# CMU-Quake/hercules

Hardware: AMD Instinct MI355X
Metric: element-updates/sec (whole node) + achieved HBM GB/s, 64M-elem box (higher is better)
Workload: dtype f64

## Files before the change

hercules_amd/capi.py:

```python
import ctypes
import os

import numpy as np

_HERE = os.path.dirname(os.path.abspath(__file__))
_LIBPATH = os.environ.get("HQ_SOLVER_LIB") or os.path.join(_HERE, "csrc", "libhq_solver.so")

HQ_VARIANT_AUTO, HQ_VARIANT_SCATTER, HQ_VARIANT_PATCH = 0, 1, 2
IPC_BLOB_BYTES = 4096

EXPORTS = ["hq_device_count", "hq_last_error", "hq_create", "hq_destroy", "hq_get_info", "hq_get_info_sized", "hq_abi_version", "hq_comm_init_ipc_n",
           "hq_options_init", "hq_create_opts", "hq_get_options", "hq_real_bytes",
           "hq_comm_unique_id", "hq_comm_init", "hq_comm_selftest", "hq_group_link", "hq_group_run", "hq_set_source", "hq_run", "hq_sync", "hq_gather", "hq_gather3",
           "hq_download", "hq_upload", "hq_phase_force", "hq_phase_update", "hq_download_force",
           "hq_run_timed", "hq_dominant_kernel", "hq_plan_check", "hq_stencil_plan_check", "hq_check_finite",
           "hq_stencil_coefficients", "hq_brick_plan_check", "hq_brick_plan_check_n", "hq_comm_init_host",
           "hq_comm_ipc_export", "hq_comm_init_ipc", "hq_comm_init_loopback",
           "hq_record_add", "hq_record_pending", "hq_record_fetch", "hq_record_clear",
           "hq_snapshot_add", "hq_snapshot_pending", "hq_snapshot_fetch", "hq_snapshot_clear"]
HQ_SNAP_TM1, HQ_SNAP_TM2, HQ_SNAP_VEL = 1, 2, 4


class HqError(RuntimeError):
    pass


HOST_EXCHANGE_FN = ctypes.CFUNCTYPE(ctypes.c_int, ctypes.c_void_p, ctypes.c_int32, ctypes.POINTER(ctypes.c_int32),
                                    ctypes.POINTER(ctypes.c_int64), ctypes.POINTER(ctypes.c_void_p), ctypes.c_int32,
                                    ctypes.POINTER(ctypes.c_int32), ctypes.POINTER(ctypes.c_int64),
                                    ctypes.POINTER(ctypes.c_void_p), ctypes.c_int32)


class _Messenger(ctypes.Structure):
    _fields_ = [("procid", ctypes.c_int32), ("nodecount", ctypes.c_int32),
                ("mapping", ctypes.c_void_p)]


class _Schedule(ctypes.Structure):
    _fields_ = [("c_count", ctypes.c_int32), ("first_c", ctypes.POINTER(_Messenger)),
                ("s_count", ctypes.c_int32), ("first_s", ctypes.POINTER(_Messenger))]


class _Desc(ctypes.Structure):
    _fields_ = [("lenum", ctypes.c_int32), ("nharbored", ctypes.c_int32), ("ldnnum", ctypes.c_int32),
                ("lnid", ctypes.c_void_p), ("node_xyz", ctypes.c_void_p),
                ("dn_ldnid", ctypes.c_void_p), ("dn_ptr", ctypes.c_void_p), ("dn_lanid", ctypes.c_void_p),
                ("eTable", ctypes.c_void_p), ("nTable", ctypes.c_void_p),
                ("tm1", ctypes.c_void_p), ("tm2", ctypes.c_void_p),
                ("an_sched", _Schedule), ("dn_sched", _Schedule),
                ("deltaT", ctypes.c_double), ("rank", ctypes.c_int32), ("nranks", ctypes.c_int32),
                ("variant", ctypes.c_int32), ("reserved", ctypes.c_int32), ("node_gnid", ctypes.c_void_p),
                ("edata", ctypes.c_void_p), ("mat_bbase", ctypes.c_double), ("mat_threshold_damping", ctypes.c_double),
                ("mat_threshold_vpvs", ctypes.c_double)]


class _RecorderDesc(ctypes.Structure):
    _fields_ = [("npoints", ctypes.c_int32), ("ids", ctypes.c_void_p), ("phi", ctypes.c_void_p),
                ("rate", ctypes.c_int32), ("derivs", ctypes.c_int32), ("capacity", ctypes.c_int32)]


class _SnapshotDesc(ctypes.Structure):
    _fields_ = [("first", ctypes.c_int32), ("count", ctypes.c_int32), ("rate", ctypes.c_int32),
                ("first_step", ctypes.c_int32), ("fields", ctypes.c_int32), ("slots", ctypes.c_int32)]


class _Info(ctypes.Structure):
    _fields_ = [("variant", ctypes.c_int32), ("npatches", ctypes.c_int32),
                ("patch_pairs", ctypes.c_int64), ("device_bytes", ctypes.c_int64),
                ("step", ctypes.c_int32), ("nranks", ctypes.c_int32),
                ("lattice_patches", ctypes.c_int32), ("stencil_patches", ctypes.c_int32),
                ("ragged_patches", ctypes.c_int32), ("brick_units", ctypes.c_int32),
                ("brick_nodes", ctypes.c_int64), ("brick_units_pernode", ctypes.c_int32),
                ("brick_units_het", ctypes.c_int32), ("pcie_h2d_bytes", ctypes.c_int64),
                ("pcie_d2h_bytes", ctypes.c_int64), ("transport", ctypes.c_int32), ("ipc_arena_coarse", ctypes.c_int32),
                ("ipc_arena_kind", ctypes.c_int32), ("debug_halo", ctypes.c_int32),
                ("brick_units_packed", ctypes.c_int32), ("brick_units_ragged", ctypes.c_int32),
                ("brick_stream", ctypes.c_int32), ("brick_units_ragged_het", ctypes.c_int32), ("timed_steps", ctypes.c_int64),
                ("t_step_us", ctypes.c_double), ("t_shell_us", ctypes.c_double), ("t_interior_us", ctypes.c_double),
                ("t_chain_us", ctypes.c_double), ("t_chain_exposed_us", ctypes.c_double)]


OPTION_FIELDS = ["no_bricks", "brick_cz", "brick_minz", "brick_minnodes", "brick_no_het", "brick_no_ntsame", "brick_by_component",
                 "brick_stream", "brick_no_faces", "brick_half_tiles", "brick_no_pack", "patch_pipe", "patch_threads", "patch_pmax", "patch_pmerge", "patch_psplit", "patch_nlmax",
                 "patch_vmax", "patch_ragged", "patch_no_lattice", "patch_no_stencil", "patch_no_uniform", "patch_no_iso",
                 "patch_no_ntsame", "patch_no_dedup", "patch_wform", "patch_merge_rounds", "overlap", "no_overlap", "reserve_cus",
                 "cu_mask", "no_fused_share", "group_copies", "debug_halo", "ipc_arena"]


class Options(ctypes.Structure):
    _fields_ = ([("size", ctypes.c_uint64)] + [(n, ctypes.c_int32) for n in OPTION_FIELDS] +
                [("ipc_timeout_ms", ctypes.c_double), ("loopback_delay_us", ctypes.c_double),
                 ("verbose", ctypes.c_int32), ("quiet", ctypes.c_int32),
                 ("brick_ragged", ctypes.c_int32), ("brick_ragged_minfill", ctypes.c_int32),
                 ("allow_env", ctypes.c_int32), ("brick_ragged_het", ctypes.c_int32), ("reserved0", ctypes.c_int32),
                 ("phase_timing", ctypes.c_int32)])

    def __init__(self, **kw):
        super().__init__()
        load_library().hq_options_init(ctypes.byref(self), ctypes.c_uint64(ctypes.sizeof(self)))
        for k, v in kw.items():
            if k not in dict(self._fields_):
                raise TypeError("hq_options has no field %r" % k)
            setattr(self, k, v)

    def as_dict(self):
        return {k: getattr(self, k) for k, _ in self._fields_ if k != "size"}


_lib = None
_lib_f32 = None
_LIBPATH_F32 = os.environ.get("HQ_SOLVER_LIB_F32") or os.path.join(_HERE, "csrc", "libhq_solver_f32.so")


def load_library(path=None, precision="f64"):
    global _lib, _lib_f32
    if precision == "f32" and path is None:
        if _lib_f32 is None:
            _lib_f32 = load_library(_LIBPATH_F32)
            if _lib_f32.hq_real_bytes() != 4:
                raise HqError("%s was not built with -DHQ_SINGLE_PRECISION_SOLVER" % _LIBPATH_F32)
        return _lib_f32
    if _lib is not None and path is None:
        return _lib
    p = path or _LIBPATH
    if not os.path.exists(p):
        raise HqError("native library %s is missing: run `python -m hercules_amd.build` "
                      "(there is no Python/CPU fallback)" % p)
    probe = ctypes.CDLL(p, mode=ctypes.RTLD_LOCAL)
    lib = probe if probe.hq_real_bytes() == 4 else ctypes.CDLL(p, mode=ctypes.RTLD_GLOBAL)
    lib.hq_last_error.restype = ctypes.c_char_p
    lib.hq_dominant_kernel.restype = ctypes.c_char_p
    lib.hq_dominant_kernel.argtypes = [ctypes.c_void_p]
    for name in EXPORTS:
        getattr(lib, name)
    if path is None:
        _lib = lib
    return lib


def device_count():
    return int(load_library().hq_device_count())


def _check(rc, lib=None):
    if rc != 0:
        raise HqError("hq error %d: %s" % (rc, (lib or load_library()).hq_last_error().decode()))


# ... 30 lines not shown
        if lib.hq_real_bytes() != np.dtype(self.real).itemsize:
            raise HqError("library and precision %r disagree about sizeof(hq_real)" % precision)
        if isinstance(options, dict):
            options = Options(**options)
        keep = []
        lnid = np.ascontiguousarray(lnid, np.int32)
        etable = np.ascontiguousarray(etable, np.float64)
        ntable = np.ascontiguousarray(ntable, self.real)
        d = _Desc()
        d.lenum, d.nharbored = lnid.shape[0], ntable.shape[0]
        d.lnid, d.eTable, d.nTable = _ptr(lnid), _ptr(etable), _ptr(ntable)
        keep += [lnid, etable, ntable]
        if node_xyz is not None:
            node_xyz = np.ascontiguousarray(node_xyz, np.int32)
            keep.append(node_xyz)
            d.node_xyz = _ptr(node_xyz)
        for name, a in (("tm1", tm1), ("tm2", tm2)):
            if a is not None:
                a = np.ascontiguousarray(a, self.real)
                keep.append(a)
                setattr(d, name, _ptr(a))
        if dangling is not None:
            ids, ptr, anchors = [np.ascontiguousarray(x, np.int32) for x in dangling]
            keep += [ids, ptr, anchors]
            d.ldnnum = len(ids)
            d.dn_ldnid, d.dn_ptr, d.dn_lanid = _ptr(ids), _ptr(ptr), _ptr(anchors)
        if edata is not None:
            edata = np.ascontiguousarray(edata, np.float32)
            assert edata.shape == (lnid.shape[0], 4) and material is not None
            keep.append(edata)
            d.edata = _ptr(edata)
            d.mat_bbase, d.mat_threshold_damping, d.mat_threshold_vpvs = [float(v) for v in material]
        d.an_sched = _schedule(an_sched, keep)
        d.dn_sched = _schedule(dn_sched, keep)
        d.deltaT, d.rank, d.nranks, d.variant = dt, rank, nranks, variant
        self._h = ctypes.c_void_p()
        self.N, self.E = d.nharbored, d.lenum
        self._lib = lib
        if options is None:
            _check(lib.hq_create(ctypes.byref(d), ctypes.c_int(device), ctypes.byref(self._h)), lib)
        else:
            _check(lib.hq_create_opts(ctypes.byref(d), ctypes.c_int(device), ctypes.byref(options), ctypes.byref(self._h)), lib)

    def close(self):
        if getattr(self, "_h", None) and self._h.value:
            self._lib.hq_destroy(self._h)
            self._h = ctypes.c_void_p()

    __del__ = close

    def info(self):
        i = _Info()
        _check(self._lib.hq_get_info_sized(self._h, ctypes.byref(i), ctypes.c_uint64(ctypes.sizeof(i))), self._lib)
        return {k: getattr(i, k) for k, _ in _Info._fields_}

    def options(self):
        o = Options()
        _check(self._lib.hq_get_options(self._h, ctypes.byref(o), ctypes.c_uint64(ctypes.sizeof(o))), self._lib)
        return o.as_dict()

    def set_source(self, loaded_lnid, forces, step0=0):
        ids = np.ascontiguousarray(loaded_lnid, np.int32)
        F = np.ascontiguousarray(forces, np.float64)
        nsteps = F.shape[0] if len(ids) else 0
        _check(self._lib.hq_set_source(self._h, ctypes.c_int32(len(ids)), _ptr(ids),
                                       ctypes.c_int32(step0), ctypes.c_int32(nsteps), _ptr(F)))

    def comm_init(self, id128):
        buf = (ctypes.c_char * 128).from_buffer_copy(bytes(id128))
        _check(self._lib.hq_comm_init(self._h, buf), self._lib)

    def comm_init_host(self, exchange):
        import numpy as np

        def view(ptr, n):
            return np.ctypeslib.as_array(ctypes.cast(ctypes.c_void_p(ptr), ctypes.POINTER(ctypes.c_double)), shape=(int(n),))

        def trampoline(user, nrecv, rpeer, rcount, rbuf, nsend, speer, scount, sbuf, tag):
            try:
                exchange([(rpeer[i], view(rbuf[i], rcount[i])) for i in range(nrecv)],
                         [(speer[i], view(sbuf[i], scount[i])) for i in range(nsend)], tag)
                return 0
            except Exception:
                import traceback
                traceback.print_exc()
                return 1
        self._host_exchange = HOST_EXCHANGE_FN(trampoline)
        _check(self._lib.hq_comm_init_host(self._h, self._host_exchange, None), self._lib)

    def comm_ipc_export(self):
        buf = (ctypes.c_char * IPC_BLOB_BYTES)()
        _check(self._lib.hq_comm_ipc_export(self._h, buf), self._lib)
        return bytes(buf)

    def comm_init_ipc(self, blobs):
        raw = blobs if isinstance(blobs, (bytes, bytearray)) else b"".join(blobs)
        if len(raw) % IPC_BLOB_BYTES:
            raise HqError("comm_init_ipc: %d bytes is not a whole number of %d-byte blobs" % (len(raw), IPC_BLOB_BYTES))
        buf = (ctypes.c_char * len(raw)).from_buffer_copy(bytes(raw))
        _check(self._lib.hq_comm_init_ipc_n(self._h, buf, ctypes.c_int32(len(raw) // IPC_BLOB_BYTES)), self._lib)

    def comm_init_loopback(self):
        _check(self._lib.hq_comm_init_loopback(self._h), self._lib)

    def comm_selftest(self, count=1024):
        _check(self._lib.hq_comm_selftest(self._h, ctypes.c_int32(count)), self._lib)

# ... 97 lines not shown
        vel = np.empty((count, 3), np.float64) if fields & HQ_SNAP_VEL else None
        step = ctypes.c_int32(-1)
        _check(self._lib.hq_snapshot_fetch(self._h, ctypes.c_int32(handle), _ptr(tm1), _ptr(tm2), _ptr(vel),
                                           ctypes.byref(step)), self._lib)
        if step.value < 0:
            return -1, None, None, None
        return step.value, tm1, tm2, vel

    def snapshot_clear(self):
        _check(self._lib.hq_snapshot_clear(self._h), self._lib)
        self._snapshots = {}

    def phase_force(self):
        _check(self._lib.hq_phase_force(self._h), self._lib)

    def phase_update(self):
        _check(self._lib.hq_phase_update(self._h), self._lib)

    def download_force(self):
        f = np.empty((self.N, 3))
        _check(self._lib.hq_download_force(self._h, _ptr(f)), self._lib)
        return f


PLAN_REPORT = ("patches", "lattice_patches", "pairs", "distinct_row_blocks", "gather_passes", "gather_instructions",
               "lattice_gather_passes", "faults")


def plan_check(desc):
    rep = (ctypes.c_int64 * 8)()
    _check(load_library().hq_plan_check(ctypes.byref(desc), rep))
    return dict(zip(PLAN_REPORT, [int(v) for v in rep]))


STENCIL_PLAN_REPORT = ("patches", "tables", "full_lattices", "boundary_nodes", "corners_checked", "faults")


def stencil_plan_check(desc):
    rep = (ctypes.c_int64 * 6)()
    _check(load_library().hq_stencil_plan_check(ctypes.byref(desc), rep))
    return dict(zip(STENCIL_PLAN_REPORT, [int(v) for v in rep]))


BRICK_PLAN_REPORT = ("brick_nodes", "columns", "units", "units_one_nt_row", "het_units", "neighbours_checked",
                     "patch_nodes", "faults", "ragged_units", "ragged_nodes", "ragged_het_units", "ragged_het_nodes", "packed_units")


def brick_plan_check(desc):
    rep = (ctypes.c_int64 * len(BRICK_PLAN_REPORT))()
    _check(load_library().hq_brick_plan_check_n(ctypes.byref(desc), rep, ctypes.c_int32(len(BRICK_PLAN_REPORT))))
    return dict(zip(BRICK_PLAN_REPORT, [int(v) for v in rep]))


def comm_unique_id():
    buf = (ctypes.c_char * 128)()
    _check(load_library().hq_comm_unique_id(buf))
    return bytes(buf)


def group_link(solvers):
    arr = (ctypes.c_void_p * len(solvers))(*[s._h for s in solvers])
    lib = solvers[0]._lib
    _check(lib.hq_group_link(arr, ctypes.c_int32(len(solvers))), lib)


def group_run(solvers, nsteps):
    arr = (ctypes.c_void_p * len(solvers))(*[s._h for s in solvers])
    lib = solvers[0]._lib
    _check(lib.hq_group_run(arr, ctypes.c_int32(len(solvers)), ctypes.c_int32(nsteps)), lib)
    for s in solvers:
        s.sync()
```

hercules_amd/csrc/hq_brick.h:

```cpp
#ifndef HQ_BRICK_H
#define HQ_BRICK_H

#include <chrono>
#include <map>

#include "hq_patch.h"

#define HQ_BK_TX 64
#ifndef HQ_BK_TY
#define HQ_BK_TY 8
#endif
#define HQ_BK_THREADS (HQ_BK_TX * HQ_BK_TY)
#define HQ_BK_PY (HQ_BK_TX + 2)
#define HQ_BK_PLANE ((HQ_BK_TX + 2) * (HQ_BK_TY + 2))
#ifndef HQ_BK_ATTR
#define HQ_BK_ATTR
#endif
#define HQ_BK_NTSAME 1
#define HQ_BK_HET 2
#define HQ_BK_TOPFACE 8
#define HQ_BK_BOTFACE 16
#define HQ_BK_RAGGED 32
#define HQ_BK_PACKED 4
#ifndef HQ_BH_WAVES
#define HQ_BH_WAVES 8
#endif
#define HQ_BH_THREADS (64 * HQ_BH_WAVES)
#define HQ_BH_NRT (64 + 2 * (HQ_BH_WAVES - 1))
#define HQ_BH_TX 62
#define HQ_BH_TY (HQ_BH_WAVES - 1)
#define HQ_BH_PY 65
#define HQ_BH_CS HQ_BH_THREADS
#define HQ_BH_ROWS (65 * (HQ_BH_WAVES + 1))

struct hq_brick_unit {
    int64_t base;
    int64_t tab;
    int32_t nx, ny, np, flags;
    double  c1, c2, beta;
    double  m0, m2, m1;
    double  ft[7], fb[7];
    int64_t coef;
};

struct hq_brick_cfg {
    int cz = 32;
    int minz = 4;
    int minnodes = 512;
    int ragged = 1;
    int minfill = 128;
    int ragged_het = 1;
};

static hq_brick_cfg hq_brick_cfg_of(const hq_options& o)
{
    hq_brick_cfg c;
    c.cz = std::max(2, hq_value_or(o.brick_cz, c.cz));
    c.minz = std::max(1, hq_value_or(o.brick_minz, c.minz));
    c.minnodes = std::max(1, hq_value_or(o.brick_minnodes, c.minnodes));
    c.ragged = hq_value_or(o.brick_ragged, c.ragged) != 0;
    c.minfill = std::min(HQ_BK_THREADS, std::max(1, hq_value_or(o.brick_ragged_minfill, c.minfill)));
    c.ragged_het = hq_value_or(o.brick_ragged_het, c.ragged_het) != 0;
    return c;
}

struct hq_brick_host {
    int64_t nb = 0;
    std::vector<int32_t> perm;
    std::vector<hq_brick_unit> units;
    int32_t nsame = 0;
    int32_t nrag = 0;
    std::vector<int32_t> tab;
    std::vector<double> coef;
    std::vector<float> coef32;
    std::vector<double> nt2;
    int32_t nhet = 0;
    int32_t npacked = 0;
    int32_t nrhet = 0, nrpacked = 0;
    int32_t ncolumns = 0, nlevels = 0;
};

struct hq_brick_plan {
    int64_t nb = 0;
    int32_t nunits = 0, nsame = 0, nrag = 0, nhet = 0, npacked = 0, nrhet = 0, nrpacked = 0;
    hq_brick_unit* d_units = nullptr;
    int32_t* d_tab = nullptr;
    double* d_coef = nullptr;
    float* d_coef32 = nullptr;
    double* d_nt2 = nullptr;
    hq_mat_const mat = { 0, 0, 0, 0, 0, 0 };
    int32_t* d_src_ptr = nullptr;
    int32_t* d_src_ent = nullptr;
    std::vector<int64_t> h_base;
    std::vector<int32_t> h_slot;
    std::vector<int64_t> h_size;
    std::vector<int64_t> h_first;
};

struct hq_mat_src {
    const float* edata = nullptr;
    double dt = 0, bbase = 0, thr_damp = 0, thr_vpvs = 0;
};

static int hq_brick_plan_host(const hq_options& o, int64_t E, int64_t N, const int32_t* lnid, const int32_t* xyz, const double* c1,
                              const double* c2, const double* beta, const double* ntab, const char* excl,
                              hq_brick_host* B, const hq_mat_src* MS = nullptr)
{
    *B = hq_brick_host();
    if (!xyz || E <= 0 || N <= 0) return 0;
    const hq_brick_cfg cfg = hq_brick_cfg_of(o);
    const bool verbose = o.verbose > 1;
    auto t_lap = std::chrono::steady_clock::now();
    auto lap = [&](const char* what) {
        if (!verbose) return;
        const auto now = std::chrono::steady_clock::now();
        fprintf(stderr, "  brick plan: %-36s %6.2f s\n", what, std::chrono::duration<double>(now - t_lap).count());
        t_lap = now;
    };
    const int TX = HQ_BK_TX, TY = HQ_BK_TY;
    const bool want_het = !hq_set(o.brick_no_het);
    const bool stencil_ok = hq_stencil().ok;

    std::vector<int32_t> hs((size_t)E);
    std::map<int32_t, int64_t> cnt;
    {
        bool bad_order = false;
#pragma omp parallel
        {
            std::map<int32_t, int64_t> mine;
#pragma omp for schedule(static) reduction(|| : bad_order)
            for (int64_t e = 0; e < E; e++) {
                const int32_t* id = lnid + 8 * e;
                const int64_t h = (int64_t)xyz[3 * (int64_t)id[1]] - xyz[3 * (int64_t)id[0]];
                if (h <= 0 || h > 0x7fffffff) { bad_order = true; hs[(size_t)e] = 0; continue; }
                hs[(size_t)e] = (int32_t)h;
                mine[(int32_t)h]++;
            }
#pragma omp critical
            for (auto& kv : mine) cnt[kv.first] += kv.second;
        }
        if (bad_order) return 0;
    }
    lap("edge lengths");

    const bool want_faces = stencil_ok && hq_stencil().face_ok && !hq_set(o.brick_no_faces) && !hq_set(o.brick_no_ntsame);
    std::vector<uint8_t> touch;
    if (want_faces) {
        touch.assign((size_t)N, 0);
#pragma omp parallel for schedule(static)
        for (int64_t i = 0; i < E * 8; i++) {
            uint8_t& t8 = touch[(size_t)lnid[i]];
#pragma omp atomic
            t8++;
        }
    }

    struct level_t {
        int32_t h;
        int64_t O[3];
        int64_t D[3];
        std::vector<int32_t> Ng;
        std::vector<int32_t> Eg;
    };
    struct column_t { int lvl; int32_t x0, y0, nx, ny, z0, nz, ti, tj; int64_t base; int het; int top, bot; int rag; };
    struct ragged_t { std::vector<uint8_t> own; std::vector<int32_t> pfx; double c[3], m[3]; };
    std::vector<level_t> levels;
    std::vector<column_t> cols;
    std::vector<ragged_t> rags;
    std::vector<int32_t> ntx_of_level;

    for (auto& kv : cnt) {
        const int32_t h = kv.first;
        if (kv.second < (int64_t)cfg.minnodes) continue;
        level_t L;
        L.h = h;
        int64_t mn[3] = { INT64_MAX, INT64_MAX, INT64_MAX }, mx[3] = { INT64_MIN, INT64_MIN, INT64_MIN };
        {
            int64_t mn0 = INT64_MAX, mn1 = INT64_MAX, mn2 = INT64_MAX, mx0 = INT64_MIN, mx1 = INT64_MIN, mx2 = INT64_MIN;
#pragma omp parallel for schedule(static) reduction(min : mn0, mn1, mn2) reduction(max : mx0, mx1, mx2)
            for (int64_t e = 0; e < E; e++) {
                if (hs[(size_t)e] != h) continue;
                const int32_t* p = xyz + 3 * (int64_t)lnid[8 * e];
                mn0 = std::min<int64_t>(mn0, p[0]); mn1 = std::min<int64_t>(mn1, p[1]); mn2 = std::min<int64_t>(mn2, p[2]);
                mx0 = std::max<int64_t>(mx0, p[0]); mx1 = std::max<int64_t>(mx1, p[1]); mx2 = std::max<int64_t>(mx2, p[2]);
            }
            mn[0] = mn0; mn[1] = mn1; mn[2] = mn2; mx[0] = mx0; mx[1] = mx1; mx[2] = mx2;
        }
        bool ok = true;
        for (int d = 0; d < 3; d++) {
            L.O[d] = mn[d];
            if ((mx[d] - mn[d]) % h) ok = false;
            L.D[d] = (mx[d] - mn[d]) / h + 1;
        }
        if (!ok) continue;
        const int64_t NX = L.D[0] + 1, NY = L.D[1] + 1, NZ = L.D[2] + 1;
        const double vol = (double)NX * (double)NY * (double)NZ;
        if (vol > 8.0 * (double)kv.second + 65536.0 || vol > 2.0e9) continue;
        std::vector<int32_t>& Eg = L.Eg;
        Eg.assign((size_t)(L.D[0] * L.D[1] * L.D[2]), -1);
        L.Ng.assign((size_t)(NX * NY * NZ), -1);
        for (int pass = 0; pass < 2 && ok; pass++) {
            bool bad = false;
#pragma omp parallel for schedule(static) reduction(|| : bad)
            for (int64_t e = 0; e < E; e++) {
                if (hs[(size_t)e] != h) continue;
                const int32_t* id = lnid + 8 * e;
                int64_t q[3];
                bool good = true;
                for (int d = 0; d < 3; d++) {
                    const int64_t v = (int64_t)xyz[3 * (int64_t)id[0] + d] - L.O[d];
                    if (v % h) good = false;
                    q[d] = v / h;
                }
                if (!good) { bad = true; continue; }
                int32_t& cell = Eg[(size_t)((q[2] * L.D[1] + q[1]) * L.D[0] + q[0])];
// ... 9 lines not shown
            if (bad) ok = false;
        }
        if (!ok) continue;
        lap("level grids");
        std::vector<char> S((size_t)(NX * NY * NZ), 0);
        int64_t sx0 = INT64_MAX, sx1 = -1, sy0 = INT64_MAX, sy1 = -1;
        int64_t nsimple = 0;
#pragma omp parallel for schedule(static) reduction(min : sx0, sy0) reduction(max : sx1, sy1) reduction(+ : nsimple)
        for (int64_t Z = 1; Z < L.D[2]; Z++)
            for (int64_t Y = 1; Y < L.D[1]; Y++)
                for (int64_t X = 1; X < L.D[0]; X++) {
                    const int32_t n = L.Ng[(size_t)((Z * NY + Y) * NX + X)];
                    if (n < 0 || (excl && excl[n])) continue;
                    const double* q = ntab + 7 * (int64_t)n;
                    if (!((q[1] == q[2]) && (q[1] == q[3]) && (q[4] == q[5]) && (q[4] == q[6]))) continue;
                    int32_t e0 = -1;
                    bool s = true, uni = true;
                    for (int o = 0; o < 8 && s; o++) {
                        const int64_t cx = X - (o & 1), cy = Y - ((o >> 1) & 1), cz = Z - ((o >> 2) & 1);
                        const int32_t e = Eg[(size_t)((cz * L.D[1] + cy) * L.D[0] + cx)];
                        if (e < 0) { s = false; break; }
                        if (e0 < 0) e0 = e;
                        else uni = uni && c1[e] == c1[e0] && c2[e] == c2[e0] && beta[e] == beta[e0];
                    }
                    if (!s) continue;
                    if (!stencil_ok) uni = false;
                    if (!uni && !want_het) continue;
                    S[(size_t)((Z * NY + Y) * NX + X)] = uni ? 2 : 1;
                    nsimple++;
                    sx0 = std::min(sx0, X); sx1 = std::max(sx1, X); sy0 = std::min(sy0, Y); sy1 = std::max(sy1, Y);
                }
        if (nsimple < cfg.minnodes) continue;
        if (want_faces && L.D[2] >= 2) {
#pragma omp parallel for schedule(static) collapse(2)
            for (int side = 0; side < 2; side++)
                for (int64_t Y = 1; Y < L.D[1]; Y++)
                    for (int64_t X = 1; X < L.D[0]; X++) {
                        const int64_t Z = side ? L.D[2] : 0, cz = side ? L.D[2] - 1 : 0;
                        const int32_t n = L.Ng[(size_t)((Z * NY + Y) * NX + X)];
                        if (n < 0 || (excl && excl[n]) || touch[(size_t)n] != 4) continue;
                        int32_t e0 = -1;
                        bool s4 = true;
                        for (int o = 0; o < 4 && s4; o++) {
                            const int32_t e = Eg[(size_t)((cz * L.D[1] + (Y - ((o >> 1) & 1))) * L.D[0] + (X - (o & 1)))];
                            if (e < 0) { s4 = false; break; }
                            if (e0 < 0) e0 = e;
                            else s4 = c1[e] == c1[e0] && c2[e] == c2[e0] && beta[e] == beta[e0];
                        }
                        if (s4 && c1[e0] + c2[e0] != 0.0) S[(size_t)((Z * NY + Y) * NX + X)] = side ? 4 : 3;
                    }
        }
        lap("simple nodes");
        const int lvl = (int)levels.size();
        std::vector<std::vector<column_t>> found;
        int32_t ntx_lvl = 1;
        const int rag = cfg.ragged && stencil_ok && !hq_set(o.brick_no_ntsame) ? 1 : 0;
        const int half = rag || hq_value_or(o.brick_half_tiles, 1) != 0 ? 1 : 0;
        const int rag_het = cfg.ragged && want_het && cfg.ragged_het ? 1 : 0;
        for (int round = 0; round < 2 + half + rag_het; round++) {
            const bool rh_round = rag_het && round == 2 + half;
            const int pass = (round == 1 + half || rh_round) ? 1 : 0;
            const bool rag_round = rag && round == 1;
            const int PTX = pass == 1 ? HQ_BH_TX : (round == 0 || rag_round ? TX : TX / 2), PTY = pass == 0 ? TY : HQ_BH_TY;
            auto in_run = [pass](char v) { return pass == 0 ? v == 2 : (v == 1 || v == 2); };
            if (round >= 1) {
                sx0 = INT64_MAX; sx1 = -1; sy0 = INT64_MAX; sy1 = -1;
                for (int64_t Z = 0; Z < NZ; Z++)
                    for (int64_t Y = 0; Y < NY; Y++)
                        for (int64_t X = 0; X < NX; X++)
                            if (in_run(S[(size_t)((Z * NY + Y) * NX + X)])) { sx0 = std::min(sx0, X); sx1 = std::max(sx1, X); sy0 = std::min(sy0, Y); sy1 = std::max(sy1, Y); }
                if (sx1 < 0) { if (pass == 1) break; else continue; }
            }
            const int32_t ntx = (int32_t)((sx1 - sx0) / PTX + 1), nty = (int32_t)((sy1 - sy0) / PTY + 1);
            if (round == 0) ntx_lvl = ntx;
            const size_t f0 = found.size();
            found.resize(f0 + (size_t)nty);
            std::vector<std::vector<ragged_t>> found_r(rag_round || rh_round ? (size_t)nty : 0);
            const int32_t minfill = rh_round ? std::max(1, cfg.minfill * (HQ_BH_TX * HQ_BH_TY) / HQ_BK_THREADS) : cfg.minfill;
#pragma omp parallel for schedule(dynamic, 1)
            for (int32_t tj = 0; tj < nty; tj++) {
                const int64_t y0 = sy0 + (int64_t)tj * PTY;
                const int32_t ny = (int32_t)std::min<int64_t>(PTY, sy1 - y0 + 1);
                std::vector<int32_t> cntz;
                for (int32_t ti = 0; ti < ntx; ti++) {
                    const int64_t x0 = sx0 + (int64_t)ti * PTX;
                    const int32_t nx = (int32_t)std::min<int64_t>(PTX, sx1 - x0 + 1);
                    if (rag_round || rh_round) {
                        cntz.assign((size_t)NZ, 0);
                        for (int iter = 0; iter < (rh_round ? 1 : 4); iter++) {
                            int32_t n0 = -1;
                            int64_t Z0 = 0, X0 = 0, Y0 = 0;
                            auto cand = [&](char v) { return rh_round ? (v == 1 || v == 2) : v == 2; };
                            for (int64_t Z = 1; Z < L.D[2] && n0 < 0; Z++)
                                for (int64_t y = y0; y < y0 + ny && n0 < 0; y++) {
                                    const char* row = &S[(size_t)((Z * NY + y) * NX + x0)];
                                    for (int32_t x = 0; x < nx; x++)
                                        if (cand(row[x])) { n0 = L.Ng[(size_t)((Z * NY + y) * NX + x0 + x)]; Z0 = Z; Y0 = y; X0 = x0 + x; break; }
                                }
                            if (n0 < 0) break;
                            const int32_t e0 = L.Eg[(size_t)(((Z0 - 1) * L.D[1] + (Y0 - 1)) * L.D[0] + (X0 - 1))];
                            const double rc[3] = { c1[e0], c2[e0], beta[e0] };
                            const double* q0 = ntab + 7 * (int64_t)n0;
                            auto match = [&](int64_t X, int64_t Y, int64_t Z) -> bool {
                                if (rh_round) return true;
                                const double* q = ntab + 7 * (int64_t)L.Ng[(size_t)((Z * NY + Y) * NX + X)];
                                if (q[0] != q0[0] || q[1] != q0[1] || q[4] != q0[4]) return false;
                                const int32_t e = L.Eg[(size_t)(((Z - 1) * L.D[1] + (Y - 1)) * L.D[0] + (X - 1))];
                                return c1[e] == rc[0] && c2[e] == rc[1] && beta[e] == rc[2];
                            };
                            for (int64_t Z = Z0; Z < L.D[2]; Z++) {
                                int32_t cnt = 0;
                                for (int64_t y = y0; y < y0 + ny; y++) {
                                    const char* row = &S[(size_t)((Z * NY + y) * NX + x0)];
                                    for (int32_t x = 0; x < nx; x++) cnt += cand(row[x]) && match(x0 + x, y, Z);
                                }
                                cntz[(size_t)Z] = cnt;
                            }
                            int64_t ra = -1;
                            for (int64_t Z = Z0; Z <= L.D[2]; Z++) {
                                const bool in = Z < L.D[2] && cntz[(size_t)Z] >= minfill;
                                if (in) { if (ra < 0) ra = Z; continue; }
                                if (ra < 0) continue;
                                const int64_t nz = Z - ra;
                                int64_t total = 0;
                                for (int64_t z = ra; z < Z; z++) total += cntz[(size_t)z];
                                if (nz >= cfg.minz && total >= cfg.minnodes) {
                                    ragged_t R;
                                    R.own.assign((size_t)(nz * nx * ny), 0);
                                    R.pfx.assign((size_t)nz + 1, 0);
                                    for (int d = 0; d < 3; d++) R.c[d] = rc[d];
                                    R.m[0] = q0[0]; R.m[1] = q0[1]; R.m[2] = q0[4];
                                    for (int64_t z = ra; z < Z; z++) {
                                        int32_t k = 0;
                                        for (int64_t y = y0; y < y0 + ny; y++) {
                                            char* row = &S[(size_t)((z * NY + y) * NX + x0)];
                                            for (int32_t x = 0; x < nx; x++)
                                                if (cand(row[x]) && match(x0 + x, y, z)) { R.own[(size_t)(((z - ra) * ny + (y - y0)) * nx + x)] = 1; row[x] = 0; k++; }
                                        }
                                        R.pfx[(size_t)(z - ra) + 1] = R.pfx[(size_t)(z - ra)] + k;
// ... 114 lines not shown
    }
    {
        int nth = 1;
#pragma omp parallel
        {
#pragma omp single
            nth = omp_get_num_threads();
        }
        std::vector<int64_t> first((size_t)nth + 1, 0);
#pragma omp parallel for schedule(static, 1)
        for (int t = 0; t < nth; t++) {
            const int64_t lo = N * t / nth, hi = N * (t + 1) / nth;
            int64_t cnt = 0;
            for (int64_t n = lo; n < hi; n++) cnt += B->perm[(size_t)n] < 0;
            first[(size_t)t + 1] = cnt;
        }
        for (int i = 0; i < nth; i++) first[(size_t)i + 1] += first[(size_t)i];
#pragma omp parallel for schedule(static, 1)
        for (int t = 0; t < nth; t++) {
            const int64_t lo = N * t / nth, hi = N * (t + 1) / nth;
            int64_t k = nb + first[(size_t)t];
            for (int64_t n = lo; n < hi; n++) if (B->perm[(size_t)n] < 0) B->perm[(size_t)n] = (int32_t)k++;
        }
        if (nb + first[(size_t)nth] != N) { g_patch_err = "brick plan: numbering is not a permutation"; return -1; }
    }
    lap("numbering");
    B->nb = nb;
    B->ncolumns = (int32_t)cols.size();
    B->nlevels = (int32_t)levels.size();

    struct unit_t { int col; int32_t za, np; int64_t key; };
    std::vector<unit_t> us;
    int cz = cfg.cz;
    if (!hq_given(o.brick_cz)) {
        for (cz = 32; cz > 8; cz /= 2) {
            int64_t n = 0;
            for (auto& c : cols) n += (c.nz + cz - 1) / cz;
            if (n >= 512) break;
        }
    }
    for (size_t ci = 0; ci < cols.size(); ci++) {
        const column_t& c = cols[ci];
        const int32_t nch = (c.nz + cz - 1) / cz;
        const int32_t G = std::max(1, 64 / std::max(1, ntx_of_level[(size_t)c.lvl]));
        for (int32_t k = 0; k < nch; k++) {
            const int32_t za = (int32_t)((int64_t)c.nz * k / nch), zb = (int32_t)((int64_t)c.nz * (k + 1) / nch);
            const int64_t key = ((int64_t)c.lvl << 56) | ((int64_t)(c.tj / G) << 42) | ((int64_t)((c.z0 + za) / cz) << 28) |
                                ((int64_t)(c.tj % G) << 20) | (int64_t)c.ti;
            us.push_back({ (int)ci, c.z0 + za, zb - za, key });
        }
    }
    std::stable_sort(us.begin(), us.end(), [](const unit_t& a, const unit_t& b) { return a.key < b.key; });
    B->units.resize(us.size());
    std::vector<int64_t> toff(us.size() + 1, 0);
    for (size_t u = 0; u < us.size(); u++) {
        const column_t& c = cols[(size_t)us[u].col];
        const int64_t nr = 2 * (c.nx + 2) + 2 * c.ny;
        toff[u + 1] = toff[u] + ((int64_t)(us[u].np + 2) * nr + (c.rag ? us[u].np + 2 : 2) * (int64_t)c.nx * c.ny + 3) / 4 * 4;
    }
    B->tab.assign((size_t)toff[us.size()] + 64, 0);
    std::vector<int64_t> coff(us.size() + 1, 0);
    for (size_t u = 0; u < us.size(); u++)
        coff[u + 1] = coff[u] + (cols[(size_t)us[u].col].het ? (int64_t)(us[u].np + 1) * HQ_BH_THREADS * 3 : 0);
    B->coef.assign((size_t)coff[us.size()] + 8, 0.0);
    const bool try_pack = MS && MS->edata && MS->dt > 0 && !hq_set(o.brick_no_pack);
    if (try_pack) { B->coef32.assign((size_t)coff[us.size()] + 8, 0.0f); B->nt2.assign(2 * (size_t)N, 0.0); }
    int fault = 0;
    auto set_fault = [&]() {
#pragma omp atomic write
        fault = 1;
    };
    std::vector<char> same(us.size(), 0);
#pragma omp parallel for schedule(dynamic, 16)
    for (int64_t u = 0; u < (int64_t)us.size(); u++) {
        const column_t& c = cols[(size_t)us[(size_t)u].col];
        const level_t& L = levels[(size_t)c.lvl];
        const int64_t NX = L.D[0] + 1, NY = L.D[1] + 1;
        const int32_t za = us[(size_t)u].za, np = us[(size_t)u].np, nx = c.nx, ny = c.ny, nr = 2 * (nx + 2) + 2 * ny;
        auto dev = [&](int64_t X, int64_t Y, int64_t Z) -> int32_t {
            if (X < 0 || Y < 0 || Z < 0 || X > L.D[0] || Y > L.D[1] || Z > L.D[2]) { set_fault(); return 0; }
            const int32_t n = L.Ng[(size_t)((Z * NY + Y) * NX + X)];
            if (n < 0) { set_fault(); return 0; }
            return B->perm[(size_t)n];
        };
        int32_t* t = B->tab.data() + toff[(size_t)u];
        hq_brick_unit& U = B->units[(size_t)u];
        if (c.rag) {
            const ragged_t& R = rags[(size_t)c.rag - 1];
            auto any = [&](int64_t X, int64_t Y, int64_t Z) -> int32_t {
                if (X < 0 || Y < 0 || Z < 0 || X > L.D[0] || Y > L.D[1] || Z > L.D[2]) return -1;
                const int32_t n = L.Ng[(size_t)((Z * NY + Y) * NX + X)];
                return n < 0 ? -1 : B->perm[(size_t)n];
            };
            auto owns = [&](int32_t i, int32_t j, int32_t k) -> bool {
                return i >= 0 && i < nx && j >= 0 && j < ny && k >= 1 && k <= np && R.own[(size_t)((((int64_t)za - 1 + k - c.z0) * ny + j) * nx + i)];
            };
            auto wanted = [&](int32_t i, int32_t j, int32_t k) -> bool {
                for (int32_t dk = -1; dk <= 1; dk++)
                    for (int32_t dj = -1; dj <= 1; dj++)
                        for (int32_t di = -1; di <= 1; di++)
                            if (owns(i + di, j + dj, k + dk)) return true;
                return false;
            };
            for (int32_t k = 0; k < np + 2; k++) {
                const int64_t Z = (int64_t)za - 1 + k;
                int32_t* r = t + (int64_t)k * nr;
                for (int32_t i = 0; i < nx + 2; i++) {
                    r[i] = wanted(i - 1, -1, k) ? any(c.x0 - 1 + i, c.y0 - 1, Z) : -1;
                    r[nx + 2 + i] = wanted(i - 1, ny, k) ? any(c.x0 - 1 + i, c.y0 + ny, Z) : -1;
                }
                for (int32_t j = 0; j < ny; j++) {
                    r[2 * (nx + 2) + j] = wanted(-1, j, k) ? any(c.x0 - 1, c.y0 + j, Z) : -1;
                    r[2 * (nx + 2) + ny + j] = wanted(nx, j, k) ? any(c.x0 + nx, c.y0 + j, Z) : -1;
                }
                int32_t* pl = t + (int64_t)(np + 2) * nr + (int64_t)k * nx * ny;
                for (int32_t j = 0; j < ny; j++)
                    for (int32_t i = 0; i < nx; i++) {
                        const bool own = owns(i, j, k);
                        const int32_t q = own || wanted(i, j, k) ? any(c.x0 + i, c.y0 + j, Z) : -1;
                        if (own && q < 0) set_fault();
                        pl[j * nx + i] = own ? q : (q < 0 ? -1 : -q - 2);
                    }
            }
            U.base = c.base + R.pfx[(size_t)(za - c.z0)];
            U.tab = toff[(size_t)u];
            U.nx = nx; U.ny = ny; U.np = np; U.flags = HQ_BK_NTSAME | HQ_BK_RAGGED;
            memset(U.ft, 0, sizeof U.ft); memset(U.fb, 0, sizeof U.fb);
            U.coef = 0;
            if (!c.het) {
                U.c1 = R.c[0]; U.c2 = R.c[1]; U.beta = R.c[2];
                U.m0 = R.m[0]; U.m2 = R.m[1]; U.m1 = R.m[2];
                same[(size_t)u] = 4;
                continue;
            }
            U.flags = HQ_BK_RAGGED;
            U.c1 = U.c2 = U.beta = 0.0; U.m0 = 1.0; U.m2 = U.m1 = 0.0;
        }
        if (!c.rag) {
        for (int32_t k = 0; k < np + 2; k++) {
            const int64_t Z = (int64_t)za - 1 + k;
            int32_t* r = t + (int64_t)k * nr;
            for (int32_t i = 0; i < nx + 2; i++) { r[i] = dev(c.x0 - 1 + i, c.y0 - 1, Z); r[nx + 2 + i] = dev(c.x0 - 1 + i, c.y0 + ny, Z); }
            for (int32_t j = 0; j < ny; j++) { r[2 * (nx + 2) + j] = dev(c.x0 - 1, c.y0 + j, Z); r[2 * (nx + 2) + ny + j] = dev(c.x0 + nx, c.y0 + j, Z); }
        }
        int32_t* cap = t + (int64_t)(np + 2) * nr;
        for (int32_t j = 0; j < ny; j++)
            for (int32_t i = 0; i < nx; i++) {
                cap[j * nx + i] = dev(c.x0 + i, c.y0 + j, (int64_t)za - 1);
                cap[nx * ny + j * nx + i] = dev(c.x0 + i, c.y0 + j, (int64_t)za + np);
            }
        U.base = c.base + (int64_t)(za - c.z0 + c.top) * nx * ny;
        U.tab = toff[(size_t)u];
        U.nx = nx; U.ny = ny; U.np = np; U.flags = 0;
        memset(U.ft, 0, sizeof U.ft); memset(U.fb, 0, sizeof U.fb);
        if (c.top && za == c.z0) {
            U.flags |= HQ_BK_TOPFACE;
            memcpy(U.ft, ntab + 7 * (int64_t)L.Ng[(size_t)((((int64_t)za - 1) * NY + c.y0) * NX + c.x0)], sizeof U.ft);
        }
        if (c.bot && za + np == c.z0 + c.nz) {
            U.flags |= HQ_BK_BOTFACE;
            memcpy(U.fb, ntab + 7 * (int64_t)L.Ng[(size_t)((((int64_t)za + np) * NY + c.y0) * NX + c.x0)], sizeof U.fb);
        }
        const int32_t n0 = L.Ng[(size_t)(((int64_t)za * NY + c.y0) * NX + c.x0)];
        {
            const int32_t e0 = L.Eg[(size_t)((((int64_t)za - 1) * L.D[1] + (c.y0 - 1)) * L.D[0] + (c.x0 - 1))];
            if (e0 < 0) { set_fault(); continue; }
            U.c1 = c1[e0]; U.c2 = c2[e0]; U.beta = beta[e0];
        }
        bool sm = true;
        const double* q0 = ntab + 7 * (int64_t)n0;
        for (int32_t z = 0; z < np && sm; z++)
            for (int32_t y = 0; y < ny && sm; y++)
                for (int32_t x = 0; x < nx; x++) {
                    const int32_t n = L.Ng[(size_t)((((int64_t)za + z) * NY + (c.y0 + y)) * NX + (c.x0 + x))];
                    const double* q = ntab + 7 * (int64_t)n;
                    if (q[0] != q0[0] || q[1] != q0[1] || q[4] != q0[4]) { sm = false; break; }
                }
        if (sm && !c.het && !hq_set(o.brick_no_ntsame)) { U.flags |= HQ_BK_NTSAME; same[(size_t)u] = 1; }
        U.m0 = q0[0]; U.m2 = q0[1]; U.m1 = q0[4];
        U.coef = 0;
        }
        if (c.het) {
            U.flags |= HQ_BK_HET;
            same[(size_t)u] = c.rag ? 5 : 2;
            U.coef = coff[(size_t)u];
            double* cf = B->coef.data() + coff[(size_t)u];
            for (int32_t l = 0; l <= np; l++)
                for (int32_t j = 0; j < HQ_BH_WAVES; j++)
                    for (int32_t i = 0; i < 64; i++) {
                        const int64_t cx = (int64_t)c.x0 - 1 + i, cy = (int64_t)c.y0 - 1 + j, cz = (int64_t)za - 1 + l;
                        double* o = cf + (int64_t)l * (3 * HQ_BH_THREADS) + (j * 64 + i);
                        int32_t e = -1;
                        if (cx >= 0 && cy >= 0 && cz >= 0 && cx < L.D[0] && cy < L.D[1] && cz < L.D[2])
                            e = L.Eg[(size_t)((cz * L.D[1] + cy) * L.D[0] + cx)];
                        if (e >= 0) { o[0] = c1[e]; o[HQ_BH_CS] = c2[e]; o[2 * HQ_BH_CS] = beta[e]; }
                        else if (!c.rag && i <= nx && j <= ny) set_fault();
                    }
            if (try_pack) {
                bool ok = true;
                int32_t e0 = L.Eg[(size_t)(((int64_t)za * L.D[1] + c.y0) * L.D[0] + c.x0)];
                if (c.rag) {
                    e0 = -1;
                    for (int32_t l = 0; l <= np && e0 < 0; l++)
                        for (int32_t j = 0; j < HQ_BH_WAVES && e0 < 0; j++)
                            for (int32_t i = 0; i < 64 && e0 < 0; i++) {
                                const int64_t cx = (int64_t)c.x0 - 1 + i, cy = (int64_t)c.y0 - 1 + j, cz = (int64_t)za - 1 + l;
                                if (cx >= 0 && cy >= 0 && cz >= 0 && cx < L.D[0] && cy < L.D[1] && cz < L.D[2]) e0 = L.Eg[(size_t)((cz * L.D[1] + cy) * L.D[0] + cx)];
                            }
                }
                const float hf = e0 >= 0 ? MS->edata[4 * (int64_t)e0] : 0.0f;
                hq_mat_const K = { (MS->dt * MS->dt) * (double)hf, (double)hf, MS->dt, MS->bbase, MS->thr_damp, MS->thr_vpvs };
                float* cq = B->coef32.data() + coff[(size_t)u];
                for (int32_t l = 0; l <= np && ok; l++)
                    for (int32_t j = 0; j < HQ_BH_WAVES && ok; j++)
                        for (int32_t i = 0; i < 64; i++) {
                            const int64_t cx = (int64_t)c.x0 - 1 + i, cy = (int64_t)c.y0 - 1 + j, cz = (int64_t)za - 1 + l;
                            int32_t e = -1;
                            if (cx >= 0 && cy >= 0 && cz >= 0 && cx < L.D[0] && cy < L.D[1] && cz < L.D[2])
                                e = L.Eg[(size_t)((cz * L.D[1] + cy) * L.D[0] + cx)];
                            float* o = cq + (int64_t)l * (3 * HQ_BH_THREADS) + (j * 64 + i);
                            o[0] = o[HQ_BH_CS] = o[2 * HQ_BH_CS] = 0.0f;
                            if (e < 0) continue;
                            const float* ed = MS->edata + 4 * (int64_t)e;
                            if (ed[0] != hf || !(ed[3] > 0.0f)) { ok = false; break; }
                            bool hit = false;
                            for (int fixed = 0; fixed < 2 && !hit; fixed++) {
                                double k1, k2, kb;
                                hq_material_coef(fixed ? -ed[3] : ed[3], ed[2], ed[1], K, &k1, &k2, &kb);
                                if (k1 == c1[e] && k2 == c2[e] && kb == beta[e]) { o[0] = fixed ? -ed[3] : ed[3]; o[HQ_BH_CS] = ed[2]; o[2 * HQ_BH_CS] = ed[1]; hit = true; }
                            }
                            if (!hit) { ok = false; break; }
                        }
                const int32_t* own_ids = c.rag ? t + (int64_t)(np + 2) * nr + (int64_t)nx * ny : nullptr;
                for (int32_t z = 0; z < np && ok; z++)
                    for (int32_t y = 0; y < ny && ok; y++)
                        for (int32_t x = 0; x < nx; x++) {
                            if (own_ids && own_ids[((int64_t)z * ny + y) * nx + x] < 0) continue;
                            const int32_t n = L.Ng[(size_t)((((int64_t)za + z) * NY + (c.y0 + y)) * NX + (c.x0 + x))];
                            const double* q = ntab + 7 * (int64_t)n;
                            const double sdiff = q[0] - q[4];
                            if (q[0] - sdiff != q[4] || fabs((2.0 * q[0] - sdiff) - q[1]) > 1e-15 * fabs(q[1])) { ok = false; break; }
                            double* o2 = B->nt2.data() + 2 * (own_ids ? (int64_t)own_ids[((int64_t)z * ny + y) * nx + x] : U.base + ((int64_t)z * ny + y) * nx + x);
                            o2[0] = q[0]; o2[1] = sdiff;
                        }
                if (ok) { U.flags |= HQ_BK_PACKED; same[(size_t)u] = c.rag ? 6 : 3; U.c1 = K.A; U.c2 = K.h; }
            }
        }
    }
    lap("unit tables");
    if (fault) { g_patch_err = "brick plan: a neighbour of a simple node is missing"; return -1; }
    {
        std::vector<hq_brick_unit> a, r, b, h, hp, rh, rhp;
        for (size_t u = 0; u < us.size(); u++)
            (same[u] == 1 ? a : (same[u] == 4 ? r : (same[u] == 2 ? h : (same[u] == 3 ? hp : (same[u] == 5 ? rh : (same[u] == 6 ? rhp : b)))))).push_back(B->units[u]);
        B->nsame = (int32_t)(a.size() + r.size());
        B->nrag = (int32_t)r.size();
        B->nhet = (int32_t)(h.size() + hp.size());
        B->npacked = (int32_t)hp.size();
        B->nrhet = (int32_t)(rh.size() + rhp.size());
        B->nrpacked = (int32_t)rhp.size();
        a.insert(a.end(), r.begin(), r.end());
        a.insert(a.end(), b.begin(), b.end());
        a.insert(a.end(), h.begin(), h.end());
        a.insert(a.end(), hp.begin(), hp.end());
        a.insert(a.end(), rh.begin(), rh.end());
        a.insert(a.end(), rhp.begin(), rhp.end());
        B->units.swap(a);
        if (B->npacked + B->nrpacked == 0) { std::vector<float>().swap(B->coef32); std::vector<double>().swap(B->nt2); }
        if (verbose) fprintf(stderr, "  brick plan: %d units: %d with one n_t row of which %d ragged, %d per-element coefficients of which %d packed, %d ragged per-element of which %d packed\n",
                             (int)B->units.size(), B->nsame, B->nrag, B->nhet, B->npacked, B->nrhet, B->nrpacked);
        if (verbose && B->nrag) {
            int64_t pos = 0, own = 0, other = 0;
            for (const hq_brick_unit& U : B->units) {
                if (!(U.flags & HQ_BK_RAGGED)) continue;
                const int32_t* pl = B->tab.data() + U.tab + (int64_t)(U.np + 2) * (2 * (U.nx + 2) + 2 * U.ny);
                for (int64_t i = 0; i < (int64_t)U.nx * U.ny * (U.np + 2); i++) { pos++; own += pl[i] >= 0; other += pl[i] <= -2; }
            }
            fprintf(stderr, "  brick plan: ragged units: %lld positions, %lld owned, %lld loaded for their neighbours' sake\n", (long long)pos, (long long)own, (long long)other);
        }
    }
    return 0;
}


static __device__ __forceinline__ double hq_uniform(double v)
{
    const int lo = __builtin_amdgcn_readfirstlane(__double2loint(v)), hi = __builtin_amdgcn_readfirstlane(__double2hiint(v));
    return __hiloint2double(hi, lo);
}

template <bool PERNODE, bool BYCOMP, bool RAGGED = false>
__global__ void HQ_BK_ATTR __launch_bounds__(HQ_BK_THREADS, 4)
hq_k_brick(int32_t count, int32_t per_xcd, const hq_brick_unit* __restrict__ units, const int32_t* __restrict__ tab,
           const hq_real* __restrict__ u1g, const hq_real* __restrict__ u2g, hq_real* __restrict__ ung,
           const double* __restrict__ nt3, const int32_t* __restrict__ src_ptr, const int32_t* __restrict__ src_ent,
           const double* __restrict__ F, double dt2, hq_stencil_coef sc)
{
    __shared__ __align__(16) double s_w[2 * 3 * HQ_BK_PLANE];
    const int slot = (int)(blockIdx.x & 7) * per_xcd + (int)(blockIdx.x >> 3);
    if (slot >= count) return;
    const hq_brick_unit U = units[slot];
    const int nx = U.nx, ny = U.ny, np = U.np, nxy = nx * ny, nr = 2 * (nx + 2) + 2 * ny;
    const int t = threadIdx.x, lx = t & (HQ_BK_TX - 1), ly = t >> 6;
    const bool active = lx < nx && ly < ny;
    const int sidx = active ? ly * nx + lx : 0;
    const int myrow = (ly + 1) * HQ_BK_PY + lx + 1;
    const bool ring = t < nr;
    int rrow;
    {
        int rx, ry;
        if (t < nx + 2) { rx = t - 1; ry = -1; }
        else if (t < 2 * (nx + 2)) { rx = t - (nx + 2) - 1; ry = ny; }
        else if (t < 2 * (nx + 2) + ny) { rx = -1; ry = t - 2 * (nx + 2); }
        else { rx = nx; ry = t - 2 * (nx + 2) - ny; }
        rrow = (ry + 1) * HQ_BK_PY + rx + 1;
    }
    const int32_t* __restrict__ utab = tab + U.tab;
    const int rofs = ring ? t : 0;
    const int32_t* __restrict__ cap = utab + (int64_t)(np + 2) * nr;
    int32_t vOut = -1, vMid = RAGGED ? cap[sidx] : 0, vCur = RAGGED ? cap[nxy + sidx] : 0, vNext = 0;
    const int32_t id_lo = RAGGED ? (vMid >= 0 ? vMid : -vMid - 2) : cap[sidx];
    const double beta = U.beta;
    double P[6], Q[2];
#pragma unroll
    for (int i = 0; i < 6; i++) P[i] = hq_uniform(U.c1 * sc.p1[i] + U.c2 * sc.p2[i]);
#pragma unroll
    for (int i = 0; i < 2; i++) Q[i] = hq_uniform(U.c1 * sc.q1[i] + U.c2 * sc.q2[i]);
    const bool has_src = F && src_ptr[slot + 1] > src_ptr[slot];

    hq_real x1[3] = { 0, 0, 0 }, x2[3] = { 0, 0, 0 }, y1[3] = { 0, 0, 0 }, y2[3] = { 0, 0, 0 };
    double mn[3] = { U.m0, U.m2, U.m1 };
    double m0A = hq_uniform(1.0 / U.m0), m0B = m0A;
    double fA[3] = { 0.0, 0.0, 0.0 }, fB[3] = { 0.0, 0.0, 0.0 };
    int32_t rid = utab[rofs];

#define HQ_BK_LOAD(node_)                                                                             \
    {                                                                                                 \
        const int64_t a_ = (node_);                                                                   \
        if (active && (!RAGGED || a_ >= 0)) {                                                         \
            _Pragma("unroll") for (int d = 0; d < 3; d++) { x1[d] = u1g[3 * a_ + d]; x2[d] = u2g[3 * a_ + d]; } \
            if (PERNODE) { _Pragma("unroll") for (int d = 0; d < 3; d++) mn[d] = nt3[3 * a_ + d]; }    \
        }                                                                                             \
        if (ring && (!RAGGED || rid >= 0)) {                                                          \
            const int64_t b_ = (int64_t)rid;                                                          \
            _Pragma("unroll") for (int d = 0; d < 3; d++) { y1[d] = u1g[3 * b_ + d]; y2[d] = u2g[3 * b_ + d]; } \
        }                                                                                             \
    }
#define HQ_BK_PUT(s_, acc_, M2_, M1_)                                                                 \
    {                                                                                                 \
        hq_lds_double* img_ = (hq_lds_double*)s_w + 3 * HQ_BK_PLANE * (s_);                            \
        if (active) {                                                                                 \
            _Pragma("unroll") for (int d = 0; d < 3; d++) {                                           \
                const double a1_ = x1[d], a2_ = x2[d];                                                \
// ... 77 lines not shown
            g[0] = fma(P[2], C[0], fma(P[3], sx[0], fma(P[4], sy[0], fma(P[5], dg[0], Q[1] * A_y))));
            g[1] = fma(P[2], C[1], fma(P[3], sy[1], fma(P[4], sx[1], fma(P[5], dg[1], Q[1] * A_x))));
            g[2] = fma(P[1], C[2], fma(P[3], sxy_z, P[5] * dg[2]));
            Uo[0] = fma(Q[0], Bx0_z, Q[1] * Bx1_z);
            Uo[1] = fma(Q[0], By0_z, Q[1] * By1_z);
            Uo[2] = fma(Q[0], Bx0_x, fma(Q[1], Bx1_x, fma(Q[0], By0_y, Q[1] * By1_y)));
        }
        if (k == 0 && topf) {
            m[0] = fma(rho, Uo[0], 0.5 * m[0]); m[1] = fma(rho, Uo[1], 0.5 * m[1]); m[2] = fma(-rho, Uo[2], 0.5 * m[2]);
        }
        if (k == np + 1 && botf && active) {
            double f[3];
            f[0] = fB[0] + fma(-rho, Uo[0], 0.5 * m[0]); f[1] = fB[1] + fma(-rho, Uo[1], 0.5 * m[1]); f[2] = fB[2] + fma(rho, Uo[2], 0.5 * m[2]);
            const int local = np * nxy + sidx;
            if (has_src) {
                for (int i = src_ptr[slot]; i < src_ptr[slot + 1]; i++)
                    if (src_ent[2 * i] == local) {
                        const int li = src_ent[2 * i + 1];
                        for (int d = 0; d < 3; d++) f[d] += F[3 * li + d] * dt2;
                    }
            }
            hq_real* out = ung + 3 * (int64_t)cap[nxy + sidx];
            const double rm = 1.0 / U.fb[0];
#pragma unroll
            for (int d = 0; d < 3; d++) out[d] = f[d] * rm;
        }
        const bool outface = k == 1 && topf;
        if ((k >= 2 || outface) && active && (!RAGGED || vOut >= 0)) {
            double f[3];
#pragma unroll
            for (int d = 0; d < 3; d++) f[d] = fA[d] + (g[d] + Uo[d]);
            const int local = RAGGED ? (int)(vOut - U.base) : (k - 2) * nxy + sidx;
            if (has_src) {
                for (int i = src_ptr[slot]; i < src_ptr[slot + 1]; i++)
                    if (src_ent[2 * i] == local) {
                        const int li = src_ent[2 * i + 1];
                        for (int d = 0; d < 3; d++) f[d] += F[3 * li + d] * dt2;
                    }
            }
            hq_real* out = ung + 3 * (RAGGED ? (int64_t)vOut : (outface ? (int64_t)cap[sidx] : U.base + (int64_t)local));
            const double rm = outface ? 1.0 / U.ft[0] : m0A;
#pragma unroll
            for (int d = 0; d < 3; d++) out[d] = f[d] * rm;
        }
#pragma unroll
        for (int d = 0; d < 3; d++) { fA[d] = fB[d] + m[d]; fB[d] = g[d] - Uo[d]; }
        if (RAGGED) { vOut = vMid; vMid = vCur; vCur = vNext; }
        if (PERNODE) { m0A = m0B; m0B = 1.0 / mn[0]; }
        if (k < np || (k == np && !botf)) HQ_BK_PUT((k + 1) & 1, fB, mn[1], mn[2])
        else if (k == np) HQ_BK_PUT((k + 1) & 1, fB, U.fb[1 + d], U.fb[4 + d])
    }
#undef HQ_BK_LOAD
#undef HQ_BK_PUT
}


#define HQ_BH_LDS (8 * (2 * 2 * 3 * HQ_BH_ROWS + 6 * HQ_BH_THREADS))
#ifndef HQ_BH_ABL
#define HQ_BH_ABL 0
#endif

static __device__ __forceinline__ double hq_dpp_from_next_lane(double v)
{
    int lo = __double2loint(v), hi = __double2hiint(v);
    lo = __builtin_amdgcn_update_dpp(0, lo, 0x130, 0xf, 0xf, true);
    hi = __builtin_amdgcn_update_dpp(0, hi, 0x130, 0xf, 0xf, true);
    return __hiloint2double(hi, lo);
}

static __device__ __forceinline__ int64_t hq_rag_node(int32_t v) { return v >= 0 ? (int64_t)v : (v <= -2 ? (int64_t)(-v - 2) : (int64_t)0); }

template <bool PACKED, bool RAGGED = false>
__global__ void __launch_bounds__(HQ_BH_THREADS, HQ_BH_WAVES == 12 ? 3 : 4)
hq_k_brick_het(int32_t count, int32_t per_xcd, const hq_brick_unit* __restrict__ units, const int32_t* __restrict__ tab,
               const void* __restrict__ coef_any, const hq_real* __restrict__ u1g, const hq_real* __restrict__ u2g,
               hq_real* __restrict__ ung, const double* __restrict__ nt3, const int32_t* __restrict__ src_ptr,
               const int32_t* __restrict__ src_ent, const double* __restrict__ F, double dt2, hq_mat_const mat)
{
    extern __shared__ __align__(16) double s_het[];
    hq_lds_double* const img = (hq_lds_double*)s_het;
    hq_lds_double* const xch = img + 2 * 2 * 3 * HQ_BH_ROWS;
    const int slot = (int)(blockIdx.x & 7) * per_xcd + (int)(blockIdx.x >> 3);
    if (slot >= count) return;
    const hq_brick_unit U = units[slot];
    const int nx = U.nx, ny = U.ny, np = U.np, nxy = nx * ny, nr = 2 * (nx + 2) + 2 * ny;
    const int t = threadIdx.x, lx = t & 63, ly = t >> 6;
    const bool owner = lx < nx && ly < ny;
    const int sidx = owner ? ly * nx + lx : 0;
    const int myrow = (ly + 1) * HQ_BH_PY + lx + 1;
    const int row0 = ly * HQ_BH_PY + lx;
    const int rq = ly == HQ_BH_WAVES - 1 ? lx : (lx >= 62 ? 64 + 2 * ly + (lx - 62) : -1);
    const bool ringA = rq >= 0 && rq < nr, ringB = rq >= 0 && rq + HQ_BH_NRT < nr;
    auto ring_row = [&](int r) {
        int rx, ry;
        if (r < nx + 2) { rx = r - 1; ry = -1; }
        else if (r < 2 * (nx + 2)) { rx = r - (nx + 2) - 1; ry = ny; }
        else if (r < 2 * (nx + 2) + ny) { rx = -1; ry = r - 2 * (nx + 2); }
        else { rx = nx; ry = r - 2 * (nx + 2) - ny; }
        return (ry + 1) * HQ_BH_PY + rx + 1;
    };
    const int rrowA = ringA ? ring_row(rq) : 0, rrowB = ringB ? ring_row(rq + HQ_BH_NRT) : 0;
    const int32_t* __restrict__ rtabA = tab + U.tab + (ringA ? rq : 0);
    const int32_t* __restrict__ rtabB = tab + U.tab + (ringB ? rq + HQ_BH_NRT : 0);
    const int32_t* __restrict__ cap = tab + U.tab + (int64_t)(np + 2) * nr;
    const int64_t id_lo = RAGGED ? 0 : cap[sidx], id_hi = RAGGED ? 0 : cap[nxy + sidx];
    int32_t vload = RAGGED ? cap[sidx] : 0, vnext = RAGGED ? cap[nxy + sidx] : 0, idA = -1, idB = -1;
// ... 87 lines not shown
                    G[yb][zb][2] = Z[m1] + hq_dpp_from_next_lane(Z[m0]);
                }
#pragma unroll
            for (int zb = 0; zb < 2; zb++)
#pragma unroll
                for (int d = 0; d < 3; d++) xch[(3 * zb + d) * HQ_BH_THREADS + t] = G[0][zb][d];
            __syncthreads();
            if (owner) {
                double H0[3], H1[3];
#pragma unroll
                for (int d = 0; d < 3; d++) {
                    H0[d] = G[1][0][d] + xch[d * HQ_BH_THREADS + t + 64];
                    H1[d] = G[1][1][d] + xch[(3 + d) * HQ_BH_THREADS + t + 64];
                }
                if (l >= 1 && (!RAGGED || idA >= 0)) {
                    double f[3];
#pragma unroll
                    for (int d = 0; d < 3; d++) f[d] = accA[d] + (H0[d] - H1[d]);
                    const int local = RAGGED ? (int)((int64_t)idA - U.base) : (l - 1) * nxy + sidx;
                    if (has_src) {
                        for (int i = src_ptr[slot]; i < src_ptr[slot + 1]; i++)
                            if (src_ent[2 * i] == local) {
                                const int li = src_ent[2 * i + 1];
                                for (int d = 0; d < 3; d++) f[d] += F[3 * li + d] * dt2;
                            }
                    }
                    hq_real* out = ung + 3 * (U.base + (int64_t)local);
#pragma unroll
                    for (int d = 0; d < 3; d++) out[d] = f[d] * m0A;
                }
#pragma unroll
                for (int d = 0; d < 3; d++) accA[d] = accB[d] + (H0[d] + H1[d]);
                m0A = m0B;
                if (RAGGED) idA = idB;
            }
        }
        if (l < np) HQ_BH_PUT(l & 1, accB, m0B)
        if (PACKED) hq_material_coef(nrho, nvs, nvp, K, &c1, &c2, &beta);
        else { c1 = nc1; c2 = nc2; beta = nbeta; }
        asm volatile("" : "+v"(c1), "+v"(c2), "+v"(beta), "+v"(ridA), "+v"(ridB));
        if (RAGGED) { asm volatile("" : "+v"(vnext)); ridA = ridA < 0 ? 0 : ridA; ridB = ridB < 0 ? 0 : ridB; }
        if (l + 1 < np) HQ_BH_REQUEST(l + 3)
        __syncthreads();
    }
#undef HQ_BH_REQUEST
#undef HQ_BH_LOAD
#undef HQ_BH_LOAD_B
#undef HQ_BH_PUT
}


static void hq_brick_free(hq_brick_plan* P)
{
    void* ptrs[] = { P->d_units, P->d_tab, P->d_coef, P->d_coef32, P->d_nt2, P->d_src_ptr, P->d_src_ent };
    for (void* p : ptrs) if (p) hipFree(p);
    *P = hq_brick_plan();
}

static int hq_brick_upload(hq_brick_plan* P, const hq_brick_host& B, int64_t* bytes)
{
    P->nb = B.nb;
    P->nunits = (int32_t)B.units.size();
    P->nsame = B.nsame;
    P->nrag = B.nrag;
    P->nhet = B.nhet;
    P->npacked = B.npacked;
    P->nrhet = B.nrhet;
    P->nrpacked = B.nrpacked;
    if (P->nunits == 0) return 0;
    if (P->nhet + P->nrhet > 0) {
        if (P->nhet > P->npacked || P->nrhet > P->nrpacked) {
            if (hipMalloc((void**)&P->d_coef, 8 * B.coef.size()) != hipSuccess) { g_patch_err = "hipMalloc failed"; return -2; }
            *bytes += (int64_t)(8 * B.coef.size());
            if (hipMemcpy(P->d_coef, B.coef.data(), 8 * B.coef.size(), hipMemcpyHostToDevice) != hipSuccess) { g_patch_err = "brick coefficient upload failed"; return -3; }
        }
        if (P->npacked + P->nrpacked > 0) {
            if (hipMalloc((void**)&P->d_coef32, 4 * B.coef32.size()) != hipSuccess || hipMalloc((void**)&P->d_nt2, 8 * B.nt2.size()) != hipSuccess) { g_patch_err = "hipMalloc failed"; return -2; }
            *bytes += (int64_t)(4 * B.coef32.size() + 8 * B.nt2.size());
            if (hipMemcpy(P->d_coef32, B.coef32.data(), 4 * B.coef32.size(), hipMemcpyHostToDevice) != hipSuccess ||
                hipMemcpy(P->d_nt2, B.nt2.data(), 8 * B.nt2.size(), hipMemcpyHostToDevice) != hipSuccess) { g_patch_err = "brick coefficient upload failed"; return -3; }
        }
        static bool attr_set = false;
        if (!attr_set) {
            if (hipFuncSetAttribute((const void*)hq_k_brick_het<false>, hipFuncAttributeMaxDynamicSharedMemorySize, HQ_BH_LDS) != hipSuccess ||
                hipFuncSetAttribute((const void*)hq_k_brick_het<true>, hipFuncAttributeMaxDynamicSharedMemorySize, HQ_BH_LDS) != hipSuccess ||
                hipFuncSetAttribute((const void*)hq_k_brick_het<false, true>, hipFuncAttributeMaxDynamicSharedMemorySize, HQ_BH_LDS) != hipSuccess ||
                hipFuncSetAttribute((const void*)hq_k_brick_het<true, true>, hipFuncAttributeMaxDynamicSharedMemorySize, HQ_BH_LDS) != hipSuccess) { g_patch_err = "hq_k_brick_het: LDS attribute"; return -3; }
            attr_set = true;
        }
    }
    if (hipMalloc((void**)&P->d_units, sizeof(hq_brick_unit) * B.units.size()) != hipSuccess ||
        hipMalloc((void**)&P->d_tab, 4 * B.tab.size()) != hipSuccess) { g_patch_err = "hipMalloc failed"; return -2; }
    *bytes += (int64_t)(sizeof(hq_brick_unit) * B.units.size() + 4 * B.tab.size());
    if (hipMemcpy(P->d_units, B.units.data(), sizeof(hq_brick_unit) * B.units.size(), hipMemcpyHostToDevice) != hipSuccess ||
        hipMemcpy(P->d_tab, B.tab.data(), 4 * B.tab.size(), hipMemcpyHostToDevice) != hipSuccess) { g_patch_err = "brick table upload failed"; return -3; }
    std::vector<std::pair<int64_t, int32_t>> by_base;
    for (int32_t u = 0; u < P->nunits; u++) by_base.push_back({ B.units[(size_t)u].base, u });
    std::sort(by_base.begin(), by_base.end());
    for (auto& pr : by_base) {
        const hq_brick_unit& U = B.units[(size_t)pr.second];
        const int64_t nxy = (int64_t)U.nx * U.ny;
        const int top = (U.flags & HQ_BK_TOPFACE) != 0, bot = (U.flags & HQ_BK_BOTFACE) != 0;
        int64_t size = nxy * (U.np + top + bot);
        if (U.flags & HQ_BK_RAGGED) {
            const int32_t* pl = B.tab.data() + U.tab + (int64_t)(U.np + 2) * (2 * (U.nx + 2) + 2 * U.ny);
            size = 0;
            for (int64_t i = nxy; i < nxy * (U.np + 1); i++) size += pl[i] >= 0;
        }
        P->h_base.push_back(pr.first - top * nxy); P->h_slot.push_back(pr.second); P->h_size.push_back(size);
        P->h_first.push_back(pr.first);
    }
    return 0;
}

static int hq_brick_set_source(hq_brick_plan* P, int32_t nloaded, const int32_t* loaded, int64_t* bytes)
{
    if (P->d_src_ptr) { hipFree(P->d_src_ptr); P->d_src_ptr = nullptr; }
    if (P->d_src_ent) { hipFree(P->d_src_ent); P->d_src_ent = nullptr; }
    if (nloaded <= 0 || P->nunits == 0) return 0;
    std::vector<std::array<int32_t, 3>> rec;
    for (int32_t i = 0; i < nloaded; i++) {
        if (loaded[i] >= P->nb) continue;
        const size_t k = (size_t)(std::upper_bound(P->h_base.begin(), P->h_base.end(), (int64_t)loaded[i]) - P->h_base.begin()) - 1;
        rec.push_back({ P->h_slot[k], (int32_t)(loaded[i] - P->h_first[k]), i });
    }
    if (rec.empty()) return 0;
    std::sort(rec.begin(), rec.end());
    std::vector<int32_t> ptr((size_t)P->nunits + 1, 0), ent(rec.size() * 2);
    for (auto& r : rec) ptr[(size_t)r[0] + 1]++;
    for (int32_t u = 0; u < P->nunits; u++) ptr[(size_t)u + 1] += ptr[(size_t)u];
    for (size_t k = 0; k < rec.size(); k++) { ent[2 * k] = rec[k][1]; ent[2 * k + 1] = rec[k][2]; }
    if (hipMalloc((void**)&P->d_src_ptr, 4 * ptr.size()) != hipSuccess) { P->d_src_ptr = nullptr; return -2; }
    if (hipMalloc((void**)&P->d_src_ent, 4 * ent.size()) != hipSuccess) {
        hipFree(P->d_src_ptr); P->d_src_ptr = nullptr; P->d_src_ent = nullptr;
        return -2;
    }
    if (hipMemcpy(P->d_src_ptr, ptr.data(), 4 * ptr.size(), hipMemcpyHostToDevice) != hipSuccess ||
        hipMemcpy(P->d_src_ent, ent.data(), 4 * ent.size(), hipMemcpyHostToDevice) != hipSuccess) {
        hipFree(P->d_src_ptr); hipFree(P->d_src_ent); P->d_src_ptr = nullptr; P->d_src_ent = nullptr;
        return -3;
    }
    *bytes += (int64_t)(4 * ptr.size() + 4 * ent.size());
    return 0;
}

static void hq_brick_launch(const hq_brick_plan* P, const hq_real* u1, const hq_real* u2, hq_real* un, const double* nt3,
                            const double* F, double dt2, hipStream_t stream, bool light = false)
{
    const int32_t cnt[7] = { P->nsame - P->nrag, P->nunits - P->nsame - P->nhet - P->nrhet, P->nhet - P->npacked, P->npacked, P->nrag,
                             P->nrhet - P->nrpacked, P->nrpacked };
    int32_t first = 0;
    for (int k4 = 0; k4 < 7; k4++) {
        const int k = k4 == 0 ? 0 : (k4 == 1 ? 4 : (k4 < 5 ? k4 - 1 : k4));
        const int32_t count = cnt[k];
        if (count <= 0) continue;
        const int per_xcd = (count + 7) / 8;
        const int32_t* sp = P->d_src_ptr ? P->d_src_ptr + first : nullptr;
#define HQ_BK_ARGS count, per_xcd, P->d_units + first, P->d_tab, u1, u2, un, nt3, sp, P->d_src_ent, (sp ? F : nullptr), dt2, hq_stencil().c
#ifdef HQ_EXPERIMENT
        const unsigned xpad = getenv("HQ_X_BRICK_LDS_PAD") ? (unsigned)atoi(getenv("HQ_X_BRICK_LDS_PAD")) : 0u;
        if (xpad && k == 0) {
            static bool once = false;
            if (!once) {
                once = true;
                hipFuncSetAttribute((const void*)hq_k_brick<false, true>, hipFuncAttributeMaxDynamicSharedMemorySize, (int)xpad);
                hipFuncSetAttribute((const void*)hq_k_brick<false, false>, hipFuncAttributeMaxDynamicSharedMemorySize, (int)xpad);
            }
            if (light) hq_k_brick<false, true><<<per_xcd * 8, HQ_BK_THREADS, xpad, stream>>>(HQ_BK_ARGS);
            else hq_k_brick<false, false><<<per_xcd * 8, HQ_BK_THREADS, xpad, stream>>>(HQ_BK_ARGS);
        } else
#endif
        if (k == 0 && light) hq_k_brick<false, true><<<per_xcd * 8, HQ_BK_THREADS, 0, stream>>>(HQ_BK_ARGS);
        else if (k == 0) hq_k_brick<false, false><<<per_xcd * 8, HQ_BK_THREADS, 0, stream>>>(HQ_BK_ARGS);
        else if (k == 1 && light) hq_k_brick<true, true><<<per_xcd * 8, HQ_BK_THREADS, 0, stream>>>(HQ_BK_ARGS);
        else if (k == 1) hq_k_brick<true, false><<<per_xcd * 8, HQ_BK_THREADS, 0, stream>>>(HQ_BK_ARGS);
        else if (k == 4 && light) hq_k_brick<false, true, true><<<per_xcd * 8, HQ_BK_THREADS, 0, stream>>>(HQ_BK_ARGS);
        else if (k == 4) hq_k_brick<false, false, true><<<per_xcd * 8, HQ_BK_THREADS, 0, stream>>>(HQ_BK_ARGS);
        else if (k == 2) hq_k_brick_het<false><<<per_xcd * 8, HQ_BH_THREADS, HQ_BH_LDS, stream>>>(count, per_xcd, P->d_units + first, P->d_tab, P->d_coef, u1, u2, un, nt3, sp,
                                                                                               P->d_src_ent, (sp ? F : nullptr), dt2, P->mat);
        else if (k == 3) hq_k_brick_het<true><<<per_xcd * 8, HQ_BH_THREADS, HQ_BH_LDS, stream>>>(count, per_xcd, P->d_units + first, P->d_tab, P->d_coef32, u1, u2, un, P->d_nt2, sp,
                                                                                   P->d_src_ent, (sp ? F : nullptr), dt2, P->mat);
        else if (k == 5) hq_k_brick_het<false, true><<<per_xcd * 8, HQ_BH_THREADS, HQ_BH_LDS, stream>>>(count, per_xcd, P->d_units + first, P->d_tab, P->d_coef, u1, u2, un, nt3, sp,
                                                                                                     P->d_src_ent, (sp ? F : nullptr), dt2, P->mat);
        else hq_k_brick_het<true, true><<<per_xcd * 8, HQ_BH_THREADS, HQ_BH_LDS, stream>>>(count, per_xcd, P->d_units + first, P->d_tab, P->d_coef32, u1, u2, un, P->d_nt2, sp,
                                                                                          P->d_src_ent, (sp ? F : nullptr), dt2, P->mat);
#undef HQ_BK_ARGS
        first += count;
    }
}

#endif
```

hercules_amd/csrc/hq_engine.hip:

```cpp
#include <hip/hip_runtime.h>
#include <dlfcn.h>
#include <stdint.h>
#include <stdio.h>
#include <stdlib.h>
#include <string.h>
#include <unistd.h>

#include <algorithm>
#include <chrono>
#include <vector>

#define HQ_SOLVER_IMPLEMENTATION 1
#include "../../include/hq_solver.h"
#include "hq_kernels.h"
#include "hq_opts.h"
#include "hq_patch.h"
#include "hq_brick.h"


static thread_local char g_err[512] = "";

static int hq_fail(int code, const char* fmt, const char* a = "", const char* b = "")
{
    snprintf(g_err, sizeof g_err, fmt, a, b);
// ... 62 lines not shown
    int32_t procid, nodecount;
    int32_t offset;
};

struct hq_dev_schedule {
    std::vector<hq_dev_messenger> c, s;
    int32_t* d_cmap = nullptr;
    int32_t* d_smap = nullptr;
    int32_t* d_cmap_f = nullptr;
    int32_t* d_smap_f = nullptr;
    double*  d_c_out = nullptr;
    double*  d_c_in = nullptr;
    double*  d_s_out = nullptr;
    double*  d_s_in = nullptr;
    int32_t  ctotal = 0, stotal = 0;
    int64_t* d_c_out_id = nullptr;
    int64_t* d_c_in_id = nullptr;
    int64_t* d_s_out_id = nullptr;
    int64_t* d_s_in_id = nullptr;
    double** d_c_dst = nullptr;
    double** d_s_dst = nullptr;
    double*  h_c_out = nullptr;
    double*  h_c_in = nullptr;
    double*  h_s_out = nullptr;
    double*  h_s_in = nullptr;
    int64_t* h_c_out_id = nullptr;
    int64_t* h_c_in_id = nullptr;
    int64_t* h_s_out_id = nullptr;
    int64_t* h_s_in_id = nullptr;
};

struct hq_ctx {
    hq_options opts;
    int device = 0;
    hipStream_t stream = nullptr;
    int32_t E = 0, N = 0, ldnnum = 0;
    int32_t variant = HQ_VARIANT_SCATTER;
    int32_t step = 0;
    int32_t rank = 0, nranks = 1;
    double dt = 0, dt2 = 0;
    int64_t bytes = 0;
    int64_t h2d_bytes = 0, d2h_bytes = 0;
    int32_t* d_gather_ids = nullptr;
    hq_real* d_gather_out = nullptr;
    int32_t gather_cap = 0;

    int32_t Epad = 0;
    int32_t* d_lnid = nullptr;
    double* d_c1 = nullptr;
    double* d_c2 = nullptr;
    double* d_beta = nullptr;
    double* d_nt = nullptr;
    double* d_nt_rows = nullptr;
    hq_real* d_u[3] = { nullptr, nullptr, nullptr };
    int now = 0, prev = 1, spare = 2;
    double* d_force = nullptr;
    int32_t nloaded = 0, src_step0 = 0, src_nsteps = 0;
    int32_t* d_loaded = nullptr;
    double* d_F = nullptr;
    std::vector<int32_t> h_loaded;
    size_t F_capacity = 0;
    int32_t* d_dn_id = nullptr;
    int32_t* d_dn_ptr = nullptr;
    int32_t* d_dn_anchor = nullptr;
    hq_dev_schedule an, dn;
    hq_nccl_comm comm = nullptr;
    hq_host_exchange_fn host_xchg = nullptr;
    void* host_user = nullptr;
    std::vector<hq_ctx*>* group = nullptr;
    bool group_owner = false;
    bool share_packed = false;
    struct hq_ipc_state* ipc = nullptr;
    hipEvent_t ev_sent = nullptr;
    hipStream_t cstream = nullptr;
    hipEvent_t ev_bnd = nullptr, ev_shared = nullptr, ev_an_shared = nullptr, ev_assigned = nullptr;
    hipStream_t bstream = nullptr;
    hipEvent_t ev_patches = nullptr, ev_bricks = nullptr;
    bool overlap = false;
    bool stream_masked = false;
    bool can_overlap = false;
    int reserve_cus = 8;
    int32_t nI = 0, nOI = 0;
    double* d_iforce = nullptr;
    int32_t* d_oi_node = nullptr;
    int32_t* d_oi_slot = nullptr;
    int32_t* d_oi_ptr = nullptr;
    int32_t* d_oi_pos = nullptr;
    int32_t* d_oi_fc = nullptr;
    int32_t  nSD = 0;
    int32_t* d_sd_dst = nullptr;
    int32_t* d_sd_ptr = nullptr;
    int32_t* d_sd_src = nullptr;
    int32_t* d_sd_deps = nullptr;
    hq_patch_plan plan;
    hq_brick_plan bricks;
    std::vector<int32_t> perm;
    bool debug_halo = false;
    unsigned long long dbg_send_epoch[4] = { 0, 0, 0, 0 }, dbg_recv_epoch[4] = { 0, 0, 0, 0 };
    int64_t* d_gkey = nullptr;
    int32_t* d_halo_err = nullptr;
    enum { HQ_CLK_STEP0 = 0, HQ_CLK_SHELL1, HQ_CLK_INT0, HQ_CLK_INT1, HQ_CLK_CHAIN0, HQ_CLK_CHAIN1, HQ_CLK_N, HQ_CLK_SLOTS = 64 };
    struct hq_clock_slot { hipEvent_t e[HQ_CLK_N] = {}; bool used[HQ_CLK_N] = {}; bool pending = false; };
    bool clock_skip = false;
    std::vector<hq_clock_slot> clock;
    size_t clock_at = 0;
    double clk_us[5] = { 0, 0, 0, 0, 0 };
    int64_t clk_steps = 0;
    struct hq_recorder {
// ... 978 lines not shown
    for (auto& sn : c->snaps) {
        if (!hq_snapshot_due(sn, c->step)) continue;
        if (sn.npending >= sn.slots) return hq_fail(HQ_ERR_STATE, "a snapshot's slots are all pending%s", "");
        const int32_t slot = (sn.head + sn.npending) % sn.slots;
        sn.steps[(size_t)slot] = c->step;
        sn.npending++;
        char* d = sn.d_stage + (size_t)slot * sn.slot_bytes;
        constexpr int32_t tile_rows = 256 * (16 / (int32_t)sizeof(hq_real));
        const int64_t ntiles = ((int64_t)sn.count + tile_rows - 1) / tile_rows;
        hq_k_snapshot<hq_real><<<(unsigned)std::min<int64_t>(ntiles, 8192), 256, 0, c->stream>>>(
            sn.first, sn.count, sn.d_map, c->d_u[c->now], c->d_u[c->prev], c->dt,
            (sn.fields & HQ_SNAP_TM1) ? (hq_real*)(d + sn.off[0]) : nullptr,
            (sn.fields & HQ_SNAP_TM2) ? (hq_real*)(d + sn.off[1]) : nullptr,
            (sn.fields & HQ_SNAP_VEL) ? (double*)(d + sn.off[2]) : nullptr);
        HQ_HIP(hipEventRecord(c->ev_snapped, c->stream));
        HQ_HIP(hipStreamWaitEvent(c->sstream, c->ev_snapped, 0));
        HQ_HIP(hipMemcpyAsync(sn.h_stage + (size_t)slot * sn.slot_bytes, d, sn.slot_bytes, hipMemcpyDeviceToHost, c->sstream));
        HQ_HIP(hipEventRecord(sn.done[(size_t)slot], c->sstream));
        c->d2h_bytes += (int64_t)sn.slot_bytes;
        any = true;
    }
    if (any && c->variant == HQ_VARIANT_PATCH) {
        if (brick_stream && c->bstream) HQ_HIP(hipStreamWaitEvent(c->bstream, c->ev_snapped, 0));
        if (c->overlap && c->cstream) HQ_HIP(hipStreamWaitEvent(c->cstream, c->ev_snapped, 0));
    }
    return HQ_OK;
}

static int hq_phase(hq_ctx* c, int ph)
{
    const bool patch = (c->variant == HQ_VARIANT_PATCH);
    double* ftab = patch ? c->d_iforce : c->d_force;
    hq_real* unew = patch ? c->d_u[c->spare] : c->d_u[c->prev];
    switch (ph) {
    case 0:
        if (patch) {
            int32_t k = c->step - c->src_step0;
            const double* F = (c->nloaded > 0 && k >= 0 && k < c->src_nsteps)
                                  ? c->d_F + (int64_t)k * c->nloaded * 3 : nullptr;
            int32_t nb = c->plan.nb, ne = c->plan.ne;
            if (c->overlap && !hq_patch_uses_pers(&c->plan) && nb > 0 && nb + ne <= 2 * hq_value_or(c->opts.patch_merge_rounds, 2) * c->plan.grid_cus) { nb += ne; ne = 0; }
            const bool bs = hq_use_brick_stream(c);
            if (c->overlap) HQ_HIP(hipStreamWaitEvent(c->stream, c->ev_shared, 0));
            if (bs) {
                HQ_HIP(hipStreamWaitEvent(c->stream, c->ev_bricks, 0));
                if (c->ev_shared) HQ_HIP(hipStreamWaitEvent(c->bstream, c->ev_shared, 0));
                HQ_HIP(hipStreamWaitEvent(c->bstream, c->ev_patches, 0));
            }
            if (!c->snaps.empty()) HQ_TRY(hq_snapshot_enqueue(c, bs));
            if (!c->recs.empty()) HQ_TRY(hq_record_enqueue(c, bs));
            auto launch_bricks = [&]() {
                if (c->bricks.nunits > 0)
                    hq_brick_launch(&c->bricks, c->d_u[c->now], c->d_u[c->prev], c->d_u[c->spare], c->plan.d_nt3, F, c->dt2,
                                    bs ? c->bstream : c->stream, hq_given(c->opts.brick_by_component) ? c->opts.brick_by_component != 0 : c->overlap);
                if (bs) hipEventRecord(c->ev_bricks, c->bstream);
            };
            hq_mark(c);
            hq_clock_begin(c);
            hq_clock(c, hq_ctx::HQ_CLK_STEP0, c->stream);
            if (bs) hq_clock(c, hq_ctx::HQ_CLK_INT0, c->bstream);
            bool chain_marked = false;
            auto chain_released = [&]() {
                if (!chain_marked && c->overlap) hq_clock(c, hq_ctx::HQ_CLK_CHAIN0, c->cstream);
                chain_marked = true;
            };
            if (c->plan.ns > 0 || c->plan.nr > 0) {
                const int32_t head = c->overlap ? nb : nb + ne;
                hq_patch_launch(&c->plan, 0, head, c->d_u[c->now], c->d_u[c->prev], c->d_u[c->spare], c->d_nt, F, c->dt2,
                                c->d_iforce, c->stream);
                hq_patch_launch_stencil(&c->plan, 0, c->d_u[c->now], c->d_u[c->prev], c->d_u[c->spare], c->d_nt, F, c->dt2,
                                        c->d_iforce, c->stream);
                if (c->overlap) {
                    HQ_HIP(hipEventRecord(c->ev_bnd, c->stream));
                    HQ_HIP(hipStreamWaitEvent(c->cstream, c->ev_bnd, 0));
                    chain_released();
                    hq_patch_launch(&c->plan, nb, ne, c->d_u[c->now], c->d_u[c->prev], c->d_u[c->spare], c->d_nt, F, c->dt2,
                                    c->d_iforce, c->stream, c->reserve_cus);
                }
                hq_patch_launch_stencil(&c->plan, 1, c->d_u[c->now], c->d_u[c->prev], c->d_u[c->spare], c->d_nt, F, c->dt2,
                                        c->d_iforce, c->stream);
            } else {
                if (c->overlap) {
                    hq_patch_launch(&c->plan, 0, nb, c->d_u[c->now], c->d_u[c->prev], c->d_u[c->spare], c->d_nt, F, c->dt2,
                                    c->d_iforce, c->stream);
                    HQ_HIP(hipEventRecord(c->ev_bnd, c->stream));
                    HQ_HIP(hipStreamWaitEvent(c->cstream, c->ev_bnd, 0));
                    chain_released();
                    hq_patch_launch(&c->plan, nb, ne, c->d_u[c->now], c->d_u[c->prev], c->d_u[c->spare], c->d_nt, F,
                                    c->dt2, c->d_iforce, c->stream, c->reserve_cus);
                } else {
                    hq_patch_launch(&c->plan, 0, nb + ne, c->d_u[c->now], c->d_u[c->prev], c->d_u[c->spare], c->d_nt, F,
                                    c->dt2, c->d_iforce, c->stream);
                }
            }
            if (bs) HQ_HIP(hipEventRecord(c->ev_patches, c->stream));
            hq_clock(c, hq_ctx::HQ_CLK_SHELL1, c->stream);
            if (!bs) hq_clock(c, hq_ctx::HQ_CLK_INT0, c->stream);
            launch_bricks();
            hq_clock(c, hq_ctx::HQ_CLK_INT1, bs ? c->bstream : c->stream);
            if (!c->overlap && hq_has_transport(c)) hq_clock(c, hq_ctx::HQ_CLK_CHAIN0, c->stream);
            hq_mark(c);
        } else {
            if (!c->snaps.empty()) HQ_TRY(hq_snapshot_enqueue(c, false));
            if (!c->recs.empty()) HQ_TRY(hq_record_enqueue(c, false));
            HQ_TRY(hq_launch_source(c));
            HQ_TRY(hq_launch_element_scatter(c));
        }
// ... 51 lines not shown
                }
                hq_k_interface_update<0><<<hq_blocks(c->nOI * 3, 256), 256, 0, xs>>>(
                    c->nOI, c->d_oi_node, c->d_oi_slot, c->d_oi_ptr, c->d_oi_pos, c->d_oi_fc, c->d_iforce, c->an.d_s_in,
                    c->d_nt, c->d_u[c->now], c->d_u[c->prev], unew, s_dst ? nullptr : s_out, s_dst, ia);
                c->share_packed = fuse;
            } else if (hq_ipc_ready(c) && !ipc_dbg) {
                hq_ipc_wait(c, &c->an, true, xs);
            }
        } else {
            HQ_TRY(hq_xchg_recv(c, &c->an, ftab, true, true));
            HQ_TRY(hq_launch_update(c));
        }
        return HQ_OK;
    case 5: return hq_xchg_send(c, &c->an, unew, false, false);
    case 6:
        HQ_TRY(hq_xchg_recv(c, &c->an, unew, false, false));
        if (c->ldnnum) {
            if (c->overlap) {
                HQ_HIP(hipEventRecord(c->ev_an_shared, c->cstream));
                HQ_HIP(hipStreamWaitEvent(c->stream, c->ev_an_shared, 0));
            }
            hq_k_adjust_assign<<<hq_blocks(c->ldnnum * 3, 256), 256, 0, c->stream>>>(
                c->ldnnum, c->d_dn_id, c->d_dn_ptr, c->d_dn_anchor, unew);
            if (c->overlap) {
                HQ_HIP(hipEventRecord(c->ev_assigned, c->stream));
                HQ_HIP(hipStreamWaitEvent(c->cstream, c->ev_assigned, 0));
            }
            if (c->bstream) HQ_HIP(hipEventRecord(c->ev_patches, c->stream));
        }
        return HQ_OK;
    case 7: return hq_xchg_send(c, &c->dn, unew, false, false);
    case 8:
        HQ_TRY(hq_xchg_recv(c, &c->dn, unew, false, false));
        if (patch) {
            if (c->overlap) HQ_HIP(hipEventRecord(c->ev_shared, c->cstream));
            if (hq_has_transport(c)) hq_clock(c, hq_ctx::HQ_CLK_CHAIN1, c->overlap ? c->cstream : c->stream);
            int n = c->now, p = c->prev, sp = c->spare;
            c->now = sp; c->prev = n; c->spare = p;
        } else {
            std::swap(c->now, c->prev);
        }
        c->step++;
        return HQ_OK;
    }
    return HQ_OK;
}

static int hq_step(hq_ctx* c)
{
    for (int ph = 0; ph < HQ_NPHASE; ph++) HQ_TRY(hq_phase(c, ph));
    return HQ_OK;
}


static int hq_build_distribution(hq_ctx* c, const std::vector<int32_t>& sd)
{
    const size_t n = sd.size() / 3;
    c->nSD = 0;
    if (!n) return HQ_OK;
    std::vector<int32_t> order(n);
    for (size_t i = 0; i < n; i++) order[i] = (int32_t)i;
    std::stable_sort(order.begin(), order.end(), [&](int32_t a, int32_t b) { return sd[3 * (size_t)a + 1] < sd[3 * (size_t)b + 1]; });
    std::vector<int32_t> dst, ptr(1, 0), src, deps;
    for (size_t k = 0; k < n; k++) {
        const size_t i = (size_t)order[k];
        if (dst.empty() || dst.back() != sd[3 * i + 1]) { if (!dst.empty()) ptr.push_back((int32_t)src.size()); dst.push_back(sd[3 * i + 1]); }
        src.push_back(sd[3 * i]); deps.push_back(sd[3 * i + 2]);
    }
    ptr.push_back((int32_t)src.size());
    auto up = [&](const std::vector<int32_t>& v, int32_t** p) -> int {
        HQ_TRY(hq_dev_alloc(c, p, v.size()));
        HQ_HIP(hipMemcpy(*p, v.data(), 4 * v.size(), hipMemcpyHostToDevice));
        return HQ_OK;
    };
    HQ_TRY(up(dst, &c->d_sd_dst)); HQ_TRY(up(ptr, &c->d_sd_ptr)); HQ_TRY(up(src, &c->d_sd_src)); HQ_TRY(up(deps, &c->d_sd_deps));
    c->nSD = (int32_t)dst.size();
    return HQ_OK;
}

static int hq_setup_interface(hq_ctx* c, const hq_desc* d)
{
    if (c->an.ctotal == 0 && c->an.stotal == 0 && c->dn.ctotal == 0 && c->dn.stotal == 0) return HQ_OK;
    std::vector<int32_t> slot((size_t)c->N, -1);
    std::vector<char> nonowned((size_t)c->N, 0), dn_shared((size_t)c->N, 0);
    int32_t nI = 0;
    auto slot_of = [&](int32_t n) { if (slot[n] < 0) slot[n] = nI++; return slot[n]; };
    auto translate = [&](int32_t count, const hq_messenger* list, std::vector<int32_t>& out, char* mark) {
        for (int32_t i = 0; i < count; i++)
            for (int32_t k = 0; k < list[i].nodecount; k++) {
                out.push_back(slot_of(list[i].mapping[k]));
                if (mark) mark[list[i].mapping[k]] = 1;
            }
    };
    std::vector<int32_t> an_ss, an_cs, dn_ss, dn_cs;
    translate(d->an_sched.s_count, d->an_sched.first_s, an_ss, nullptr);
    translate(d->an_sched.c_count, d->an_sched.first_c, an_cs, nonowned.data());
    translate(d->dn_sched.s_count, d->dn_sched.first_s, dn_ss, dn_shared.data());
    translate(d->dn_sched.c_count, d->dn_sched.first_c, dn_cs, nonowned.data());
    std::vector<int32_t> sd;
    for (int32_t k = 0; k < c->ldnnum; k++) {
        int32_t dnode = d->dn_ldnid[k];
        if (!dn_shared[dnode]) continue;
        int32_t deps = d->dn_ptr[k + 1] - d->dn_ptr[k];
        for (int32_t a = d->dn_ptr[k]; a < d->dn_ptr[k + 1]; a++) {
            sd.push_back(slot_of(dnode));
            sd.push_back(slot_of(d->dn_lanid[a]));
// ... 240 lines not shown
    if (hipMemset(c->d_halo_err, 0, 4 * sizeof(int32_t)) != hipSuccess) return bail(hq_fail(HQ_ERR_DEVICE, "memset%s", ""));
    if (hq_set(opts.debug_halo) && c->nranks > 1) {
        if (!d->node_gnid && !d->node_xyz)
            return bail(hq_fail(HQ_ERR_ARG, "HQ_DEBUG_HALO needs hq_desc.node_gnid or node_xyz%s", ""));
        std::vector<int64_t> key((size_t)c->N);
        for (int64_t n = 0; n < c->N; n++) {
            if (d->node_gnid) { key[(size_t)n] = d->node_gnid[n]; continue; }
            uint64_t h = 0x9E3779B97F4A7C15ull;
            for (int k = 0; k < 3; k++) {
                h ^= (uint64_t)(uint32_t)d->node_xyz[3 * n + k];
                h *= 0xBF58476D1CE4E5B9ull; h ^= h >> 29;
            }
            key[(size_t)n] = (int64_t)h;
        }
        if ((rc = hq_dev_alloc(c, &c->d_gkey, (size_t)c->N)) != HQ_OK) return bail(rc);
        if (hipMemcpy(c->d_gkey, key.data(), sizeof(int64_t) * (size_t)c->N, hipMemcpyHostToDevice) != hipSuccess)
            return bail(hq_fail(HQ_ERR_DEVICE, "node identity upload failed%s", ""));
        c->debug_halo = true;
    }

    if (variant == HQ_VARIANT_SCATTER) {
        if ((rc = hq_dev_alloc(c, &c->d_force, n3)) != HQ_OK) return bail(rc);
        if (hipMemset(c->d_force, 0, sizeof(double) * n3) != hipSuccess) return bail(hq_fail(HQ_ERR_DEVICE, "memset%s", ""));
        c->Epad = (c->E + 63) & ~63;
        std::vector<int32_t> soa((size_t)8 * c->Epad, 0);
        for (int64_t e = 0; e < c->E; e++)
            for (int n = 0; n < 8; n++) soa[(size_t)n * c->Epad + e] = d->lnid[8 * e + n];
        if ((rc = hq_dev_alloc(c, &c->d_lnid, soa.size())) != HQ_OK) return bail(rc);
        if ((rc = hq_dev_alloc(c, &c->d_c1, (size_t)c->E)) != HQ_OK) return bail(rc);
        if ((rc = hq_dev_alloc(c, &c->d_c2, (size_t)c->E)) != HQ_OK) return bail(rc);
        if ((rc = hq_dev_alloc(c, &c->d_beta, (size_t)c->E)) != HQ_OK) return bail(rc);
        if (hipMemcpy(c->d_lnid, soa.data(), sizeof(int32_t) * soa.size(), hipMemcpyHostToDevice) != hipSuccess ||
            hipMemcpy(c->d_c1, prep.c1.data(), sizeof(double) * c->E, hipMemcpyHostToDevice) != hipSuccess ||
            hipMemcpy(c->d_c2, prep.c2.data(), sizeof(double) * c->E, hipMemcpyHostToDevice) != hipSuccess ||
            hipMemcpy(c->d_beta, prep.beta.data(), sizeof(double) * c->E, hipMemcpyHostToDevice) != hipSuccess)
            return bail(hq_fail(HQ_ERR_DEVICE, "element table upload failed%s", ""));
        if ((rc = hq_build_schedule(c, &d->an_sched, &c->an)) != HQ_OK) return bail(rc);
        if ((rc = hq_build_schedule(c, &d->dn_sched, &c->dn)) != HQ_OK) return bail(rc);
        if (c->ldnnum) {
            std::vector<int32_t> sd;
            for (int32_t k = 0; k < c->ldnnum; k++)
                for (int32_t a = d->dn_ptr[k]; a < d->dn_ptr[k + 1]; a++) {
                    sd.push_back(d->dn_ldnid[k]); sd.push_back(d->dn_lanid[a]); sd.push_back(d->dn_ptr[k + 1] - d->dn_ptr[k]);
                }
            if ((rc = hq_build_distribution(c, sd)) != HQ_OK) return bail(rc);
        }
    } else {
        int64_t pb = 0;
        c->plan.ragged_default = true;
        rc = hq_patch_build(opts, &c->plan, c->E, c->N, d->lnid, d->node_xyz, prep.c1.data(), prep.c2.data(), prep.beta.data(), ntab,
                            prep.dn, prep.seed0.data(), &pb, BH.nb);
        lap("patch plan");
        if (rc == 0 && BH.nb > 0) rc = hq_brick_upload(&c->bricks, BH, &pb);
        c->bricks.mat = { 0.0, 0.0, d->deltaT, d->mat_bbase, d->mat_threshold_damping, d->mat_threshold_vpvs };
        lap("brick upload");
        if (rc != 0)
            return bail(hq_fail(rc == -1 ? HQ_ERR_ARG : (rc == -2 ? HQ_ERR_NOMEM : HQ_ERR_DEVICE), "patch plan: %s",
                                hq_patch_error()));
        c->bytes += pb;
        c->plan.grid_cus = std::max(8, prop.multiProcessorCount & ~7);
        if ((rc = hq_build_schedule(c, &d->an_sched, &c->an)) != HQ_OK) return bail(rc);
        if ((rc = hq_build_schedule(c, &d->dn_sched, &c->dn)) != HQ_OK) return bail(rc);
        if ((rc = hq_setup_interface(c, d)) != HQ_OK) return bail(rc);
        lap("schedules, interface");
    }
    if (hipDeviceSynchronize() != hipSuccess) return bail(hq_fail(HQ_ERR_DEVICE, "upload failed%s", ""));
    c->h2d_bytes = c->d2h_bytes = 0;
    *out = c;
    return HQ_OK;
}

#include "hq_plan_check.h"

extern "C" int hq_destroy(hq_ctx* c)
{
    if (!c) return HQ_OK;
    hipSetDevice(c->device);
    if (c->stream) hq_quiesce(c);
    if (c->sstream) hipStreamSynchronize(c->sstream);
    if (c->comm && g_rccl.handle) g_rccl.CommDestroy(c->comm);
    if (c->ipc) {
        hq_ipc_state* I = c->ipc;
        for (int x = 0; x < 4; x++) {
            hq_dev_schedule* sc = x < 2 ? &c->an : &c->dn;
            if (x & 1) sc->d_c_in = nullptr; else sc->d_s_in = nullptr;
            if (I->d_dst[x]) hipFree(I->d_dst[x]);
            if (I->d_sig[x]) hipFree(I->d_sig[x]);
            if (I->d_dst_id[x]) hipFree(I->d_dst_id[x]);
        }
        for (void* p : I->opened) hipIpcCloseMemHandle(p);
        if (I->d_done) hipFree(I->d_done);
        if (I->arena) hipFree(I->arena);
        delete I;
        c->ipc = nullptr;
    }
    void* ptrs[] = { c->d_gather_ids, c->d_gather_out, c->d_lnid, c->d_c1, c->d_c2, c->d_beta, c->d_nt_rows, c->d_u[0], c->d_u[1], c->d_u[2],
                     c->d_force, c->d_loaded, c->d_F, c->d_dn_id, c->d_dn_ptr, c->d_dn_anchor,
                     c->an.d_cmap, c->an.d_smap, c->an.d_c_out, c->an.d_c_in, c->an.d_s_out, c->an.d_s_in,
                     c->dn.d_cmap, c->dn.d_smap, c->dn.d_c_out, c->dn.d_c_in, c->dn.d_s_out, c->dn.d_s_in,
                     c->d_iforce, c->d_oi_node, c->d_oi_slot, c->d_oi_ptr, c->d_oi_pos, c->d_oi_fc, c->d_sd_dst, c->d_sd_ptr, c->d_sd_src, c->d_sd_deps,
                     c->d_gkey, c->d_halo_err, c->an.d_c_out_id, c->an.d_c_in_id, c->an.d_s_out_id, c->an.d_s_in_id,
                     c->dn.d_c_out_id, c->dn.d_c_in_id, c->dn.d_s_out_id, c->dn.d_s_in_id };
    for (void* p : ptrs) if (p) hipFree(p);
    hq_record_drop_all(c);
    hq_snapshot_drop_all(c);
    if (c->an.d_cmap_f && c->an.d_cmap_f != c->an.d_cmap) hipFree(c->an.d_cmap_f);
    if (c->an.d_smap_f && c->an.d_smap_f != c->an.d_smap) hipFree(c->an.d_smap_f);
    if (c->dn.d_cmap_f && c->dn.d_cmap_f != c->dn.d_cmap) hipFree(c->dn.d_cmap_f);
    if (c->dn.d_smap_f && c->dn.d_smap_f != c->dn.d_smap) hipFree(c->dn.d_smap_f);
    for (hq_dev_schedule* sc : { &c->an, &c->dn }) {
        for (double* hp : { sc->h_c_out, sc->h_c_in, sc->h_s_out, sc->h_s_in })
            if (hp) hipHostFree(hp);
        for (int64_t* hp : { sc->h_c_out_id, sc->h_c_in_id, sc->h_s_out_id, sc->h_s_in_id })
            if (hp) hipHostFree(hp);
        if (sc->d_c_dst) hipFree(sc->d_c_dst);
        if (sc->d_s_dst) hipFree(sc->d_s_dst);
    }
    if (c->ev_sent) hipEventDestroy(c->ev_sent);
    if (c->cstream) { hipStreamSynchronize(c->cstream); hipStreamDestroy(c->cstream); }
    if (c->bstream) { hipStreamSynchronize(c->bstream); hipStreamDestroy(c->bstream); }
    for (auto& sl : c->clock) for (hipEvent_t e : sl.e) if (e) hipEventDestroy(e);
    if (c->ev_patches) hipEventDestroy(c->ev_patches);
    if (c->ev_bricks) hipEventDestroy(c->ev_bricks);
    if (c->ev_bnd) hipEventDestroy(c->ev_bnd);
    if (c->ev_shared) hipEventDestroy(c->ev_shared);
    if (c->ev_an_shared) hipEventDestroy(c->ev_an_shared);
    if (c->ev_assigned) hipEventDestroy(c->ev_assigned);
    if (c->group) {
        std::vector<hq_ctx*>* g = c->group;
        bool any = false;
        for (auto& m : *g) { if (m == c) m = nullptr; any |= (m != nullptr); }
        if (!any) delete g;
    }
    hq_patch_free(&c->plan);
    hq_brick_free(&c->bricks);
    for (hipEvent_t e : c->ev) hipEventDestroy(e);
    for (int k = 0; k < 2; k++) if (c->ev_span[k]) hipEventDestroy(c->ev_span[k]);
    if (c->stream) hipStreamDestroy(c->stream);
    delete c;
    return HQ_OK;
}

extern "C" int hq_real_bytes(void) { return (int)sizeof(hq_real); }

extern "C" int hq_abi_version(void) { return HQ_ABI_VERSION; }

extern "C" int hq_get_info_sized(hq_ctx* c, hq_info* info, uint64_t size)
{
    if (!c || !info) return hq_fail(HQ_ERR_ARG, "null argument%s", "");
// ... 459 lines not shown
                             int32_t nsteps, const double* F)
{
    if (!c || nloaded < 0 || nsteps < 0 || (nloaded && nsteps && (!loaded || !F)))
        return hq_fail(HQ_ERR_ARG, "bad source description%s", "");
    HQ_HIP(hipSetDevice(c->device));
    HQ_HIP(hq_quiesce(c));
    for (int32_t i = 0; i < nloaded; i++)
        if (loaded[i] < 0 || loaded[i] >= c->N) return hq_fail(HQ_ERR_ARG, "loaded node id out of range%s", "");
    std::vector<int32_t> dev_ids;
    if (!c->perm.empty() && nloaded > 0) {
        dev_ids.resize((size_t)nloaded);
        for (int32_t i = 0; i < nloaded; i++) dev_ids[(size_t)i] = c->perm[(size_t)loaded[i]];
        loaded = dev_ids.data();
    }
    const bool same_nodes = nloaded > 0 && nsteps > 0 && c->d_loaded && (int32_t)c->h_loaded.size() == nloaded &&
                            memcmp(c->h_loaded.data(), loaded, sizeof(int32_t) * (size_t)nloaded) == 0 &&
                            (size_t)nloaded * 3 * (size_t)nsteps <= c->F_capacity;
    if (same_nodes) {
        c->src_step0 = step0; c->src_nsteps = nsteps;
        HQ_HIP(hipMemcpy(c->d_F, F, sizeof(double) * 3 * nloaded * (size_t)nsteps, hipMemcpyHostToDevice));
        HQ_HIP(hipStreamSynchronize(nullptr));
        c->h2d_bytes += 24 * (int64_t)nloaded * nsteps;
        return HQ_OK;
    }
    if (c->d_loaded) { hipFree(c->d_loaded); c->d_loaded = nullptr; }
    if (c->d_F) { hipFree(c->d_F); c->d_F = nullptr; }
    c->nloaded = nloaded; c->src_step0 = step0; c->src_nsteps = nsteps;
    c->h_loaded.clear(); c->F_capacity = 0;
    if (nloaded && nsteps) {
        HQ_TRY(hq_dev_alloc(c, &c->d_loaded, (size_t)nloaded));
        HQ_TRY(hq_dev_alloc(c, &c->d_F, (size_t)nloaded * 3 * nsteps));
        HQ_HIP(hipMemcpy(c->d_loaded, loaded, sizeof(int32_t) * nloaded, hipMemcpyHostToDevice));
        HQ_HIP(hipMemcpy(c->d_F, F, sizeof(double) * 3 * nloaded * (size_t)nsteps, hipMemcpyHostToDevice));
        c->h2d_bytes += 4 * (int64_t)nloaded + 24 * (int64_t)nloaded * nsteps;
        c->h_loaded.assign(loaded, loaded + nloaded);
        c->F_capacity = (size_t)nloaded * 3 * (size_t)nsteps;
    }
    if (c->variant == HQ_VARIANT_PATCH) {
        int r = hq_patch_set_source(&c->plan, (nloaded && nsteps) ? nloaded : 0, loaded, &c->bytes);
        if (r == 0) r = hq_brick_set_source(&c->bricks, (nloaded && nsteps) ? nloaded : 0, loaded, &c->bytes);
        if (r != 0) return hq_fail(HQ_ERR_NOMEM, "source table allocation failed%s", "");
    }
    HQ_HIP(hipStreamSynchronize(nullptr));
    return HQ_OK;
}

extern "C" int hq_run(hq_ctx* c, int32_t nsteps)
{
    if (!c || nsteps < 0) return hq_fail(HQ_ERR_ARG, "bad argument%s", "");
    if (c->group && c->group->size() > 1)
        return hq_fail(HQ_ERR_STATE, "linked contexts are stepped with hq_group_run%s", "");
    HQ_TRY(hq_output_check_room(c, nsteps));
    HQ_HIP(hipSetDevice(c->device));
    for (int32_t s = 0; s < nsteps; s++) HQ_TRY(hq_step(c));
    HQ_HIP(hipGetLastError());
    return HQ_OK;
}

extern "C" int hq_sync(hq_ctx* c)
{
    if (!c) return hq_fail(HQ_ERR_ARG, "null argument%s", "");
    HQ_HIP(hipSetDevice(c->device));
    HQ_HIP(hq_quiesce(c));
    if (c->sstream) HQ_HIP(hipStreamSynchronize(c->sstream));
    hq_clock_harvest_all(c, true);
    if (c->ipc) {
        int32_t late = 0;
        HQ_HIP(hipMemcpy(&late, c->d_halo_err + 2, sizeof late, hipMemcpyDeviceToHost));
        if (late) {
            char n[32];
            snprintf(n, sizeof n, "%d", late);
            HQ_HIP(hipMemsetAsync(c->d_halo_err + 2, 0, sizeof(int32_t), c->stream));
            HQ_HIP(hipStreamSynchronize(c->stream));
            return hq_fail(HQ_ERR_COMM, "IPC transport: %s waits for a neighbour's halo records timed out (HQ_IPC_TIMEOUT_MS)", n);
        }
    }
    if (c->debug_halo) {
        int32_t bad = 0;
        HQ_HIP(hipMemcpy(&bad, c->d_halo_err, sizeof bad, hipMemcpyDeviceToHost));
        if (bad) {
            char n[32];
            snprintf(n, sizeof n, "%d", bad);
            HQ_HIP(hipMemsetAsync(c->d_halo_err, 0, sizeof(int32_t), c->stream));
            HQ_HIP(hipStreamSynchronize(c->stream));
            return hq_fail(HQ_ERR_COMM, "HQ_DEBUG_HALO: %s halo records arrived for another node than the schedule names "
                                        "(global node ids do not match, psolve.c:5058-5069)", n);
        }
    }
    return HQ_OK;
}

extern "C" int hq_check_finite(hq_ctx* c, int64_t* nonfinite)
{
    if (!c || !nonfinite) return hq_fail(HQ_ERR_ARG, "null argument%s", "");
    HQ_HIP(hipSetDevice(c->device));
    HQ_HIP(hq_quiesce(c));
    HQ_HIP(hipMemsetAsync(c->d_halo_err + 1, 0, sizeof(int32_t), c->stream));
    const int64_t n3 = 3 * (int64_t)c->N;
    const hq_real* arr[2] = { c->d_u[c->now], c->d_u[c->prev] };
    for (const hq_real* a : arr)
        if (a) hq_k_count_nonfinite<<<2048, 256, 0, c->stream>>>(n3, a, c->d_halo_err + 1);
    if (c->d_force) hq_k_count_nonfinite<<<2048, 256, 0, c->stream>>>(n3, (const double*)c->d_force, c->d_halo_err + 1);
    int32_t bad = 0;
    HQ_HIP(hipMemcpyAsync(&bad, c->d_halo_err + 1, sizeof bad, hipMemcpyDeviceToHost, c->stream));
    HQ_HIP(hipStreamSynchronize(c->stream));
    *nonfinite = bad;
    return HQ_OK;
}

extern "C" int hq_run_timed(hq_ctx* c, int32_t nsteps, double* total_ms, double* kernel_ms_avg)
{
    if (!c || nsteps <= 0) return hq_fail(HQ_ERR_ARG, "bad argument%s", "");
    HQ_TRY(hq_output_check_room(c, nsteps));
    HQ_HIP(hipSetDevice(c->device));
    size_t need = 2 * (size_t)nsteps;
    while (c->ev.size() < need) {
        hipEvent_t e;
        HQ_HIP(hipEventCreate(&e));
        c->ev.push_back(e);
    }
    for (int k = 0; k < 2; k++)
        if (!c->ev_span[k]) HQ_HIP(hipEventCreate(&c->ev_span[k]));
    HQ_HIP(hq_quiesce(c));
    hq_clock_harvest_all(c, true);
    const double clk_us0 = c->clk_us[0];
    const int64_t clk_n0 = c->clk_steps;
    c->ev_used = 0;
    HQ_HIP(hipEventRecord(c->ev_span[0], c->stream));
    c->timing = true;
    int rc = HQ_OK;
    for (int32_t s = 0; s < nsteps && rc == HQ_OK; s++) rc = hq_step(c);
    c->timing = false;
    if (c->overlap) hipStreamWaitEvent(c->stream, c->ev_shared, 0);
    if (c->bstream) hipStreamWaitEvent(c->stream, c->ev_bricks, 0);
    hipEventRecord(c->ev_span[1], c->stream);
    hipError_t he = hq_quiesce(c);
    if (he == hipSuccess) hq_clock_harvest_all(c, true);
    double tot = 0, ker = 0;
    if (rc == HQ_OK && he == hipSuccess) {
        float ms = 0;
        hipEventElapsedTime(&ms, c->ev_span[0], c->ev_span[1]);
        tot = ms;
        for (size_t i = 0; i + 1 < c->ev_used; i += 2) {
            hipEventElapsedTime(&ms, c->ev[i], c->ev[i + 1]);
            ker += ms;
        }
        if (c->ev_used >= 2) ker /= (double)(c->ev_used / 2);
        if (c->bstream && c->clk_steps > clk_n0) ker = (c->clk_us[0] - clk_us0) / (double)(c->clk_steps - clk_n0) * 1e-3;
    }
    if (rc != HQ_OK) return rc;
    if (he != hipSuccess) return hq_fail(HQ_ERR_DEVICE, "timed run failed: %s", hipGetErrorString(he));
    if (total_ms) *total_ms = tot;
    if (kernel_ms_avg) *kernel_ms_avg = ker;
    return HQ_OK;
}

extern "C" const char* hq_dominant_kernel(hq_ctx* c)
{
    if (!c || c->variant != HQ_VARIANT_PATCH) return "hq_k_element_scatter";
    if (2 * c->bricks.nb > (int64_t)c->N) return "hq_k_brick";
    if (2 * c->plan.nstencil > c->plan.npatches) return "hq_k_patch_stencil";
    if (!hq_patch_uses_pers(&c->plan)) return "hq_k_patch_step";
    return c->plan.seeded ? "hq_k_patch_seed" : "hq_k_patch_pers";
}

static int hq_gather_impl(hq_ctx* c, int32_t n, const int32_t* lnid, hq_real* o1, hq_real* o2, hq_real* o3);

extern "C" int hq_gather(hq_ctx* c, int32_t n, const int32_t* lnid, hq_real* o1, hq_real* o2)
{
    return hq_gather_impl(c, n, lnid, o1, o2, nullptr);
}

extern "C" int hq_gather3(hq_ctx* c, int32_t n, const int32_t* lnid, hq_real* o1, hq_real* o2, hq_real* o3)
{
    if (c && o3 && c->variant != HQ_VARIANT_PATCH)
        return hq_fail(HQ_ERR_STATE, "u(t - 2 dt) is kept by the patch variant only%s", "");
    return hq_gather_impl(c, n, lnid, o1, o2, o3);
}

static int hq_gather_impl(hq_ctx* c, int32_t n, const int32_t* lnid, hq_real* o1, hq_real* o2, hq_real* o3)
{
    if (!c || n < 0 || (n && !lnid)) return hq_fail(HQ_ERR_ARG, "bad argument%s", "");
    if (n == 0) return HQ_OK;
    HQ_HIP(hipSetDevice(c->device));
    HQ_HIP(hq_quiesce(c));
    for (int32_t i = 0; i < n; i++)
        if (lnid[i] < 0 || lnid[i] >= c->N) return hq_fail(HQ_ERR_ARG, "node id out of range%s", "");
    if (n > c->gather_cap) {
        if (c->d_gather_ids) { hipFree(c->d_gather_ids); c->d_gather_ids = nullptr; }
        if (c->d_gather_out) { hipFree(c->d_gather_out); c->d_gather_out = nullptr; }
        c->gather_cap = 0;
        const int32_t cap = std::max(n, 1024);
        HQ_HIP(hipMalloc((void**)&c->d_gather_ids, sizeof(int32_t) * (size_t)cap));
        if (hipMalloc((void**)&c->d_gather_out, sizeof(hq_real) * 9 * (size_t)cap) != hipSuccess) {
            hipFree(c->d_gather_ids); c->d_gather_ids = nullptr;
            return hq_fail(HQ_ERR_NOMEM, "hipMalloc failed%s", "");
        }
        c->gather_cap = cap;
    }
    int32_t* d_ids = c->d_gather_ids;
    hq_real* d_o = c->d_gather_out;
    hipError_t e;
    c->h2d_bytes += 4 * (int64_t)n;
    c->d2h_bytes += 3 * (int64_t)sizeof(hq_real) * (int64_t)n * ((o1 ? 1 : 0) + (o2 ? 1 : 0) + (o3 ? 1 : 0));
    std::vector<int32_t> dev_ids;
    if (!c->perm.empty()) {
// ... 214 lines not shown

extern "C" int hq_snapshot_fetch(hq_ctx* c, int32_t handle, hq_real* tm1, hq_real* tm2, double* vel, int32_t* step)
{
    if (!c || !step) return hq_fail(HQ_ERR_ARG, "null argument%s", "");
    hq_ctx::hq_snapshot* sn = hq_snapshot_find(c, handle);
    if (!sn) return hq_fail(HQ_ERR_ARG, "unknown snapshot handle%s", "");
    if ((tm1 && !(sn->fields & HQ_SNAP_TM1)) || (tm2 && !(sn->fields & HQ_SNAP_TM2)) || (vel && !(sn->fields & HQ_SNAP_VEL)))
        return hq_fail(HQ_ERR_ARG, "the snapshot does not hold a field that an output pointer was given for%s", "");
    *step = -1;
    if (sn->npending == 0) return HQ_OK;
    HQ_HIP(hipSetDevice(c->device));
    HQ_HIP(hipEventSynchronize(sn->done[(size_t)sn->head]));
    const char* h = sn->h_stage + (size_t)sn->head * sn->slot_bytes;
    const size_t n3 = 3 * (size_t)sn->count;
    if (tm1) hq_host_copy(tm1, h + sn->off[0], sizeof(hq_real) * n3);
    if (tm2) hq_host_copy(tm2, h + sn->off[1], sizeof(hq_real) * n3);
    if (vel) hq_host_copy(vel, h + sn->off[2], sizeof(double) * n3);
    *step = sn->steps[(size_t)sn->head];
    sn->head = (sn->head + 1) % sn->slots;
    sn->npending--;
    return HQ_OK;
}

extern "C" int hq_snapshot_clear(hq_ctx* c)
{
    if (!c) return hq_fail(HQ_ERR_ARG, "null argument%s", "");
    if (c->snaps.empty()) return HQ_OK;
    HQ_HIP(hipSetDevice(c->device));
    HQ_HIP(hq_quiesce(c));
    if (c->sstream) HQ_HIP(hipStreamSynchronize(c->sstream));
    hq_snapshot_drop_all(c);
    return HQ_OK;
}

extern "C" int hq_download(hq_ctx* c, hq_real* tm1, hq_real* tm2)
{
    if (!c) return hq_fail(HQ_ERR_ARG, "null argument%s", "");
    HQ_HIP(hipSetDevice(c->device));
    HQ_HIP(hq_quiesce(c));
    if (tm1) HQ_TRY(hq_field_to_host(c, c->d_u[c->now], tm1));
    if (tm2) HQ_TRY(hq_field_to_host(c, c->d_u[c->prev], tm2));
    return HQ_OK;
}

extern "C" int hq_upload(hq_ctx* c, const hq_real* tm1, const hq_real* tm2, int32_t step)
{
    if (!c || !tm1 || !tm2) return hq_fail(HQ_ERR_ARG, "null argument%s", "");
    HQ_HIP(hipSetDevice(c->device));
    HQ_HIP(hq_quiesce(c));
    size_t bytes = sizeof(hq_real) * 3 * (size_t)c->N;
    HQ_TRY(hq_field_to_device(c, tm1, c->d_u[c->now]));
    HQ_TRY(hq_field_to_device(c, tm2, c->d_u[c->prev]));
    if (c->d_u[2]) {
        HQ_HIP(hipMemsetAsync(c->d_u[c->spare], 0, bytes, c->stream));
        HQ_HIP(hipStreamSynchronize(c->stream));
    }
    HQ_HIP(hipStreamSynchronize(nullptr));
    c->step = step;
    return HQ_OK;
}

extern "C" int hq_phase_force(hq_ctx* c)
{
    if (!c) return hq_fail(HQ_ERR_ARG, "null argument%s", "");
    if (c->variant != HQ_VARIANT_SCATTER) return hq_fail(HQ_ERR_STATE, "phases exist in the scatter variant only%s", "");
    HQ_HIP(hipSetDevice(c->device));
    HQ_TRY(hq_launch_source(c));
    HQ_TRY(hq_launch_element_scatter(c));
    HQ_HIP(hipGetLastError());
    return HQ_OK;
}

extern "C" int hq_phase_update(hq_ctx* c)
{
    if (!c) return hq_fail(HQ_ERR_ARG, "null argument%s", "");
    if (c->variant != HQ_VARIANT_SCATTER) return hq_fail(HQ_ERR_STATE, "phases exist in the scatter variant only%s", "");
    HQ_HIP(hipSetDevice(c->device));
    HQ_TRY(hq_launch_update(c));
    std::swap(c->now, c->prev);
    c->step++;
    HQ_HIP(hipGetLastError());
    return HQ_OK;
}

extern "C" int hq_download_force(hq_ctx* c, double* force)
{
    if (!c || !force) return hq_fail(HQ_ERR_ARG, "null argument%s", "");
    if (c->variant != HQ_VARIANT_SCATTER) return hq_fail(HQ_ERR_STATE, "no force array in the patch variant%s", "");
    HQ_HIP(hipSetDevice(c->device));
    HQ_HIP(hq_quiesce(c));
    HQ_HIP(hipMemcpy(force, c->d_force, sizeof(double) * 3 * (size_t)c->N, hipMemcpyDeviceToHost));
    return HQ_OK;
}
```

hercules_amd/csrc/hq_opts.h:

```cpp
#ifndef HQ_OPTS_H
#define HQ_OPTS_H

#include <cstddef>
#include <cstdlib>
#include <cstring>

struct hq_opt_entry { const char* env; size_t off; int kind; };

#define HQ_OPT_I(env_, field_) { env_, offsetof(hq_options, field_), 0 }
#define HQ_OPT_D(env_, field_) { env_, offsetof(hq_options, field_), 1 }
static const hq_opt_entry g_opt_table[] = {
    HQ_OPT_I("HQ_NO_BRICKS", no_bricks), HQ_OPT_I("HQ_BRICK_CZ", brick_cz), HQ_OPT_I("HQ_BRICK_MINZ", brick_minz),
    HQ_OPT_I("HQ_BRICK_MINNODES", brick_minnodes), HQ_OPT_I("HQ_BRICK_NO_HET", brick_no_het),
    HQ_OPT_I("HQ_BRICK_NO_NTSAME", brick_no_ntsame), HQ_OPT_I("HQ_BRICK_BY_COMPONENT", brick_by_component),
    HQ_OPT_I("HQ_BRICK_STREAM", brick_stream), HQ_OPT_I("HQ_BRICK_NO_FACES", brick_no_faces), HQ_OPT_I("HQ_BRICK_HALF_TILES", brick_half_tiles), HQ_OPT_I("HQ_BRICK_NO_PACK", brick_no_pack), HQ_OPT_I("HQ_PATCH_PIPE", patch_pipe), HQ_OPT_I("HQ_PATCH_THREADS", patch_threads),
    HQ_OPT_I("HQ_PATCH_PMAX", patch_pmax), HQ_OPT_I("HQ_PATCH_PMERGE", patch_pmerge), HQ_OPT_I("HQ_PATCH_PSPLIT", patch_psplit),
    HQ_OPT_I("HQ_PATCH_NLMAX", patch_nlmax), HQ_OPT_I("HQ_PATCH_VMAX", patch_vmax), HQ_OPT_I("HQ_PATCH_RAGGED", patch_ragged),
    HQ_OPT_I("HQ_PATCH_NO_LATTICE", patch_no_lattice), HQ_OPT_I("HQ_PATCH_NO_STENCIL", patch_no_stencil),
    HQ_OPT_I("HQ_PATCH_NO_UNIFORM", patch_no_uniform), HQ_OPT_I("HQ_PATCH_NO_ISO", patch_no_iso),
    HQ_OPT_I("HQ_PATCH_NO_NTSAME", patch_no_ntsame), HQ_OPT_I("HQ_PATCH_NO_DEDUP", patch_no_dedup),
    HQ_OPT_I("HQ_PATCH_WFORM", patch_wform), HQ_OPT_I("HQ_PATCH_MERGE_ROUNDS", patch_merge_rounds),
    HQ_OPT_I("HQ_OVERLAP", overlap), HQ_OPT_I("HQ_NO_OVERLAP", no_overlap), HQ_OPT_I("HQ_RESERVE_CUS", reserve_cus),
    HQ_OPT_I("HQ_CU_MASK", cu_mask), HQ_OPT_I("HQ_NO_FUSED_SHARE", no_fused_share), HQ_OPT_I("HQ_GROUP_COPIES", group_copies),
    HQ_OPT_I("HQ_DEBUG_HALO", debug_halo), HQ_OPT_I("HQ_IPC_ARENA", ipc_arena), HQ_OPT_D("HQ_IPC_TIMEOUT_MS", ipc_timeout_ms),
    HQ_OPT_D("HQ_LOOPBACK_DELAY_US", loopback_delay_us), HQ_OPT_I("HQ_PATCH_VERBOSE", verbose), HQ_OPT_I("HQ_QUIET", quiet),
    HQ_OPT_I("HQ_BRICK_RAGGED", brick_ragged), HQ_OPT_I("HQ_BRICK_RAGGED_MINFILL", brick_ragged_minfill),
    HQ_OPT_I("HQ_PHASE_TIMING", phase_timing), HQ_OPT_I("HQ_BRICK_RAGGED_HET", brick_ragged_het),
};
#undef HQ_OPT_I
#undef HQ_OPT_D

static void hq_options_defaults(hq_options* o)
{
    o->size = sizeof(hq_options);
    for (const hq_opt_entry& e : g_opt_table) {
        if (e.kind == 0) *(int32_t*)((char*)o + e.off) = -1;
        else *(double*)((char*)o + e.off) = -1.0;
    }
    o->allow_env = -1;
    o->reserved0 = -1;
}

static void hq_options_adopt(hq_options* dst, const hq_options* src)
{
    hq_options_defaults(dst);
    if (!src) return;
    const size_t n = (size_t)(src->size < sizeof(hq_options) ? src->size : sizeof(hq_options));
    if (n > sizeof(uint64_t)) memcpy((char*)dst + sizeof(uint64_t), (const char*)src + sizeof(uint64_t), n - sizeof(uint64_t));
    dst->size = sizeof(hq_options);
}

static int hq_opt_env_int(const char* env, const char* v)
{
    if (!strcmp(env, "HQ_IPC_ARENA")) return !strcmp(v, "fine") ? 0 : (!strcmp(v, "uncached") ? 1 : (!strcmp(v, "coarse") ? 2 : atoi(v)));
    if (!*v) return 1;
    return atoi(v);
}

static void hq_options_resolve(hq_options* out, const hq_options* caller)
{
    hq_options_adopt(out, caller);
    const char* master = getenv("HQ_ALLOW_ENV");
    const bool allow = out->allow_env >= 0 ? out->allow_env != 0 : (master && *master && strcmp(master, "0") != 0);
    out->allow_env = allow ? 1 : 0;
    if (!allow) return;
    for (const hq_opt_entry& e : g_opt_table) {
        const char* v = getenv(e.env);
        if (!v) continue;
        if (e.kind == 0) *(int32_t*)((char*)out + e.off) = hq_opt_env_int(e.env, v);
        else if (*v) *(double*)((char*)out + e.off) = atof(v);
    }
}

template <typename T> static inline bool hq_given(T f) { return f >= 0; }
template <typename T> static inline T hq_value_or(T f, T def) { return f >= 0 ? f : def; }
template <typename T> static inline bool hq_set(T f) { return f > 0; }

static inline const char* hq_opt_env_only(const hq_options& o, const char* env)
{
    return o.allow_env == 1 ? getenv(env) : nullptr;
}

#endif
```

hercules_amd/csrc/hq_plan_check.h:

```cpp
#ifndef HQ_PLAN_CHECK_H
#define HQ_PLAN_CHECK_H

extern "C" int hq_plan_check(const hq_desc* d, int64_t report[8])
{
    hq_options opts;
    hq_options_resolve(&opts, nullptr);
    if (!report) return hq_fail(HQ_ERR_ARG, "inconsistent mesh description%s", "");
    hq_prep prep;
    HQ_TRY(hq_prepare(d, opts, 0, &prep));
    const int64_t E = d->lenum, N = d->nharbored;
    const hq_dangling& dn = prep.dn;
    bool want_lattice = false;
    const hq_patch_cfg cfg = hq_patch_cfg_of(opts, dn.n > 0, d->node_xyz != nullptr, &want_lattice);
    hq_patch_host H;
    if (hq_patch_plan_host(opts, cfg, E, N, d->lnid, d->node_xyz, dn, want_lattice, &H) != 0)
        return hq_fail(HQ_ERR_ARG, "patch plan: %s", hq_patch_error());
    const hq_lattice_tab& T = hq_lattice();
    int64_t nlat = 0, passes = 0, lpasses = 0, instr = 0, bad = 0;
    std::vector<int32_t> covered((size_t)N, 0);
#pragma omp parallel for schedule(dynamic, 64) reduction(+ : nlat, passes, lpasses, instr, bad)
    for (int64_t p = 0; p < (int64_t)H.desc.size(); p++) {
        const hq_patch_desc& D = H.desc[(size_t)p];
        const bool lat = H.lattice[(size_t)p] != 0;
        nlat += lat;
// ... 336 lines not shown
        std::vector<int32_t> all((size_t)E);
        for (int64_t e = 0; e < E; e++) all[(size_t)e] = (int32_t)e;
        if (hq_patch_plan_host(opts, cfg, E, N, p_lnid, p_xyz, dn, false, &Ha, B.nb) != 0 ||
            hq_patch_plan_host(opts, cfg, E, N, p_lnid, p_xyz, dn, false, &Hb, B.nb, &all) != 0)
            return hq_fail(HQ_ERR_ARG, "patch plan: %s", hq_patch_error());
        if (Ha.pelem != Hb.pelem || Ha.halo != Hb.halo || Ha.pidx != Hb.pidx || Ha.desc.size() != Hb.desc.size() || Ha.ds_ent != Hb.ds_ent) bad++;
        for (size_t q = 0; q < Ha.desc.size() && q < Hb.desc.size(); q++)
            if (Ha.desc[q].base != Hb.desc[q].base || Ha.desc[q].nown != Hb.desc[q].nown || Ha.desc[q].npairs != Hb.desc[q].npairs ||
                Ha.desc[q].nhalo != Hb.desc[q].nhalo || Ha.desc[q].pair_off != Hb.desc[q].pair_off) bad++;
        std::vector<int32_t> patch_of((size_t)N, -1);
        for (size_t q = 0; q < Ha.desc.size(); q++)
            for (int32_t n = Ha.desc[q].base; n < Ha.desc[q].base + Ha.desc[q].nown; n++) patch_of[(size_t)n] = (int32_t)q;
        for (int64_t n = B.nb; n < N; n++) if (patch_of[(size_t)n] < 0) bad++;
        int64_t need = 0, have = 0;
        for (int64_t e = 0; e < E; e++) {
            int32_t seen[8]; int ns = 0;
            for (int c8 = 0; c8 < 8; c8++) {
                const int32_t q = patch_of[(size_t)p_lnid[8 * e + c8]];
                bool dup = q < 0;
                for (int t = 0; t < ns; t++) dup |= seen[t] == q;
                if (!dup) seen[ns++] = q;
            }
            for (int t = 0; t < ns; t++) {
                need++;
                const hq_patch_desc& D = Ha.desc[(size_t)seen[t]];
                have += std::binary_search(Ha.pelem.begin() + D.pair_off, Ha.pelem.begin() + D.pair_off + D.npairs, (int32_t)e);
            }
        }
        if (have != need) bad++;
    }
    report[0] = B.nb; report[1] = B.ncolumns; report[2] = (int64_t)B.units.size(); report[3] = nsame;
    report[4] = B.nhet + B.nrhet; report[5] = nchecked; report[6] = N - B.nb; report[7] = bad;
    report[8] = B.nrag; report[10] = B.nrhet; report[12] = B.npacked + B.nrpacked;
    for (const hq_brick_unit& U : B.units) {
        if (!(U.flags & HQ_BK_RAGGED)) continue;
        const int32_t* pl = B.tab.data() + U.tab + (int64_t)(U.np + 2) * (2 * (U.nx + 2) + 2 * U.ny);
        for (int64_t i = (int64_t)U.nx * U.ny; i < (int64_t)U.nx * U.ny * (U.np + 1); i++) report[(U.flags & HQ_BK_HET) ? 11 : 9] += pl[i] >= 0;
    }
    if (bad) return hq_fail(HQ_ERR_STATE, "brick plan self-check failed%s", "");
    return HQ_OK;
}

extern "C" int hq_brick_plan_check(const hq_desc* d, int64_t report[8]) { return hq_brick_plan_check_n(d, report, 8); }

extern "C" int hq_brick_plan_check_n(const hq_desc* d, int64_t* report, int32_t n)
{
    int64_t r13[13];
    if (!report || n < 8) return hq_fail(HQ_ERR_ARG, "hq_brick_plan_check_n: a report of at least 8 entries%s", "");
    const int rc = hq_brick_plan_check_impl(d, r13);
    for (int k = 0; k < n; k++) report[k] = k < 13 ? r13[k] : 0;
    return rc;
}

#endif
```

hercules_amd/csrc/hq_prepare.h:

```cpp
#ifndef HQ_PREPARE_H
#define HQ_PREPARE_H

template <typename F>
static void hq_for_each_sched_node(const hq_desc* d, F&& f)
{
    const hq_schedule* sched[2] = { &d->an_sched, &d->dn_sched };
    for (int s = 0; s < 2; s++)
        for (int side = 0; side < 2; side++) {
            const int32_t cnt = side ? sched[s]->s_count : sched[s]->c_count;
            const hq_messenger* list = side ? sched[s]->first_s : sched[s]->first_c;
            for (int32_t i = 0; i < cnt; i++)
                for (int32_t k = 0; k < list[i].nodecount; k++) f(s, side, list[i].mapping ? list[i].mapping[k] : -1);
        }
}

enum { HQ_PREP_COEF = 1, HQ_PREP_NT = 2, HQ_PREP_BRICKS = 4 };

struct hq_prep {
    std::vector<double> c1, c2, beta;
    const double* ntab = nullptr;
    std::vector<char> excl;
    hq_brick_host bricks;
    std::vector<int32_t> perm;
    hq_desc desc;
// ... 28 lines not shown
    const int64_t E = d->lenum, N = d->nharbored;
    const int32_t ndn = d->ldnnum;

    for (int64_t i = 0; i < E * 8; i++)
        if (d->lnid[i] < 0 || d->lnid[i] >= N) return hq_fail(HQ_ERR_ARG, "lnid out of range%s", "");
    if (ndn && (!d->dn_ldnid || !d->dn_ptr || !d->dn_lanid)) return hq_fail(HQ_ERR_ARG, "dangling-node tables missing%s", "");
    for (int32_t k = 0; k < ndn; k++) {
        if (d->dn_ldnid[k] < 0 || d->dn_ldnid[k] >= N || d->dn_ptr[k + 1] <= d->dn_ptr[k])
            return hq_fail(HQ_ERR_ARG, "bad dangling-node table%s", "");
        for (int32_t a = d->dn_ptr[k]; a < d->dn_ptr[k + 1]; a++)
            if (d->dn_lanid[a] < 0 || d->dn_lanid[a] >= N) return hq_fail(HQ_ERR_ARG, "bad anchor id%s", "");
    }
    if (ndn) {
        std::vector<char> is_dn((size_t)N, 0);
        for (int32_t k = 0; k < ndn; k++) is_dn[d->dn_ldnid[k]] = 1;
        for (int32_t a = 0; a < d->dn_ptr[ndn]; a++)
            if (is_dn[d->dn_lanid[a]]) return hq_fail(HQ_ERR_ARG, "an anchor is itself a hanging node%s", "");
    }
    bool ids_ok = true;
    hq_for_each_sched_node(d, [&](int, int, int32_t n) { ids_ok = ids_ok && n >= 0 && n < N; });
    if (!ids_ok) return hq_fail(HQ_ERR_ARG, "messenger node id out of range%s", "");

    if (what & HQ_PREP_COEF) {
        out->c1.resize((size_t)E); out->c2.resize((size_t)E); out->beta.resize((size_t)E);
        for (int64_t e = 0; e < E; e++) {
            const double* ep = d->eTable + 4 * e;
            out->c1[(size_t)e] = ep[0]; out->c2[(size_t)e] = ep[1];
            out->beta[(size_t)e] = (ep[0] != 0.0) ? ep[2] / ep[0] : ((ep[1] != 0.0) ? ep[3] / ep[1] : 0.0);
            const double lhs = ep[2] * ep[1], rhs = ep[3] * ep[0];
            if (fabs(lhs - rhs) > 1e-12 * std::max(fabs(lhs), fabs(rhs)))
                return hq_fail(HQ_ERR_ARG, "eTable is not Rayleigh-proportional (c3/c1 != c4/c2): not the table solver_init builds%s", "");
        }
    }
    auto t_last = std::chrono::steady_clock::now();
    auto lap = [&](double* s) {
        *s = std::chrono::duration<double>(std::chrono::steady_clock::now() - t_last).count();
        t_last = std::chrono::steady_clock::now();
    };
    if (what & HQ_PREP_NT) out->ntab = hq_ntable64(d, out->nt64);

    out->excl.assign((size_t)N, 0);
    for (int32_t k = 0; k < ndn; k++) {
        out->excl[d->dn_ldnid[k]] = 1;
        for (int32_t a = d->dn_ptr[k]; a < d->dn_ptr[k + 1]; a++) out->excl[d->dn_lanid[a]] = 1;
    }
    hq_for_each_sched_node(d, [&](int, int, int32_t n) { out->excl[n] = 1; });

    hq_desc& dd = out->desc;
    dd = *d;
    hq_brick_host& BH = out->bricks;
    if ((what & HQ_PREP_BRICKS) && d->node_xyz && !hq_set(o.no_bricks)) {
        hq_mat_src ms;
        ms.edata = d->edata; ms.dt = d->deltaT; ms.bbase = d->mat_bbase; ms.thr_damp = d->mat_threshold_damping; ms.thr_vpvs = d->mat_threshold_vpvs;
        if (hq_brick_plan_host(o, E, N, d->lnid, d->node_xyz, out->c1.data(), out->c2.data(), out->beta.data(), out->ntab,
                               out->excl.data(), &BH, &ms) != 0)
            return hq_fail(HQ_ERR_ARG, "brick plan: %s", hq_patch_error());
        lap(&out->brick_plan_s);
    }
    if (BH.nb > 0) {
        const std::vector<int32_t>& pm = BH.perm;
        bool in_range = (int64_t)pm.size() == N;
#pragma omp parallel for schedule(static) reduction(&& : in_range)
        for (int64_t n = 0; n < (int64_t)pm.size(); n++) in_range = in_range && pm[(size_t)n] >= 0 && pm[(size_t)n] < N;
        if (!in_range) return hq_fail(HQ_ERR_STATE, "brick plan: the numbering leaves the mesh%s", "");
        out->p_lnid.resize((size_t)E * 8);
#pragma omp parallel for schedule(static)
        for (int64_t i = 0; i < E * 8; i++) out->p_lnid[(size_t)i] = pm[(size_t)d->lnid[i]];
        out->p_xyz.resize((size_t)N * 3);
        out->p_nt.resize((size_t)N * 7);
        int32_t* p_xyz = out->p_xyz.data();
        double* p_nt = out->p_nt.data();
        const double* ntab = out->ntab;
#pragma omp parallel for schedule(static)
        for (int64_t n = 0; n < N; n++) {
            const int64_t q = pm[(size_t)n];
            for (int k = 0; k < 3; k++) p_xyz[3 * q + k] = d->node_xyz[3 * n + k];
            for (int k = 0; k < 7; k++) p_nt[7 * q + k] = ntab[7 * n + k];
        }
        dd.lnid = out->p_lnid.data(); dd.node_xyz = p_xyz; dd.nTable = nullptr; out->ntab = p_nt;
        std::vector<double>().swap(out->nt64);
        if (d->node_gnid) {
            out->p_gnid.resize((size_t)N);
            for (int64_t n = 0; n < N; n++) out->p_gnid[(size_t)pm[(size_t)n]] = d->node_gnid[n];
            dd.node_gnid = out->p_gnid.data();
        }
        if (ndn) {
            const int32_t na = d->dn_ptr[ndn];
            out->p_dn_id.resize((size_t)ndn); out->p_dn_anchor.resize((size_t)na);
            for (int32_t k = 0; k < ndn; k++) out->p_dn_id[(size_t)k] = pm[(size_t)d->dn_ldnid[k]];
            for (int32_t a = 0; a < na; a++) out->p_dn_anchor[(size_t)a] = pm[(size_t)d->dn_lanid[a]];
            dd.dn_ldnid = out->p_dn_id.data(); dd.dn_lanid = out->p_dn_anchor.data();
        }
        {
            const hq_schedule* in[2] = { &d->an_sched, &d->dn_sched };
            hq_schedule* to[2] = { &dd.an_sched, &dd.dn_sched };
            size_t nm = 0;
            for (int s2 = 0; s2 < 2; s2++) nm += (size_t)in[s2]->c_count + (size_t)in[s2]->s_count;
            out->p_maps.reserve(nm);
            for (int s2 = 0; s2 < 2; s2++)
                for (int side = 0; side < 2; side++) {
                    const int32_t cnt = side ? in[s2]->s_count : in[s2]->c_count;
                    const hq_messenger* list = side ? in[s2]->first_s : in[s2]->first_c;
                    std::vector<hq_messenger>& v = out->p_msg[2 * s2 + side];
                    for (int32_t i = 0; i < cnt; i++) {
                        out->p_maps.emplace_back((size_t)list[i].nodecount);
                        for (int32_t k = 0; k < list[i].nodecount; k++) out->p_maps.back()[(size_t)k] = pm[(size_t)list[i].mapping[k]];
                        v.push_back({ list[i].procid, list[i].nodecount, out->p_maps.back().data() });
                    }
// ... 31 lines not shown
```

include/hq_solver.h:

```cpp
#ifndef HQ_SOLVER_H
#define HQ_SOLVER_H

#include <stdint.h>

#ifdef __cplusplus
extern "C" {
#endif

#define HQ_API __attribute__((visibility("default")))

typedef struct hq_ctx hq_ctx;

typedef enum {
    HQ_OK            =  0,
    HQ_ERR_ARG       = -1,
    HQ_ERR_NOMEM     = -2,
    HQ_ERR_DEVICE    = -3,
    HQ_ERR_NODEVICE  = -4,
    HQ_ERR_COMM      = -5,
    HQ_ERR_STATE     = -6
} hq_status;

enum {
    HQ_VARIANT_AUTO    = 0,
// ... 81 lines not shown
HQ_API int hq_device_count(void);

HQ_API const char* hq_last_error(void);

HQ_API int hq_create(const hq_desc* desc, int device, hq_ctx** out);

typedef struct {
    uint64_t size;
    int32_t no_bricks;
    int32_t brick_cz;
    int32_t brick_minz;
    int32_t brick_minnodes;
    int32_t brick_no_het;
    int32_t brick_no_ntsame;
    int32_t brick_by_component;
    int32_t brick_stream;
    int32_t brick_no_faces;
    int32_t brick_half_tiles;
    int32_t brick_no_pack;
    int32_t patch_pipe;
    int32_t patch_threads;
    int32_t patch_pmax;
    int32_t patch_pmerge;
    int32_t patch_psplit;
    int32_t patch_nlmax;
    int32_t patch_vmax;
    int32_t patch_ragged;
    int32_t patch_no_lattice;
    int32_t patch_no_stencil;
    int32_t patch_no_uniform;
    int32_t patch_no_iso;
    int32_t patch_no_ntsame;
    int32_t patch_no_dedup;
    int32_t patch_wform;
    int32_t patch_merge_rounds;
    int32_t overlap;
    int32_t no_overlap;
    int32_t reserve_cus;
    int32_t cu_mask;
    int32_t no_fused_share;
    int32_t group_copies;
    int32_t debug_halo;
    int32_t ipc_arena;
    double  ipc_timeout_ms;
    double  loopback_delay_us;
    int32_t verbose;
    int32_t quiet;
    int32_t brick_ragged;
    int32_t brick_ragged_minfill;
    int32_t allow_env;
    int32_t brick_ragged_het;
    int32_t reserved0;
    int32_t phase_timing;
} hq_options;

HQ_API void hq_options_init(hq_options* opts, uint64_t size);
HQ_API int  hq_create_opts(const hq_desc* desc, int device, const hq_options* opts, hq_ctx** out);
HQ_API int  hq_get_options(hq_ctx* ctx, hq_options* out, uint64_t size);

HQ_API int hq_destroy(hq_ctx* ctx);

#define HQ_ABI_VERSION 6
HQ_API int hq_abi_version(void);
HQ_API int hq_real_bytes(void);
HQ_API int hq_get_info_sized(hq_ctx* ctx, hq_info* info, uint64_t size);
HQ_API int hq_get_info(hq_ctx* ctx, hq_info* info);
#ifndef HQ_SOLVER_IMPLEMENTATION
#define hq_get_info(ctx, info) hq_get_info_sized((ctx), (info), (uint64_t)sizeof(hq_info))
#endif

HQ_API int hq_comm_unique_id(void* id128);
HQ_API int hq_comm_init(hq_ctx* ctx, const void* id128);
HQ_API int hq_comm_selftest(hq_ctx* ctx, int32_t count);

typedef int (*hq_host_exchange_fn)(void* user, int32_t nrecv, const int32_t* recv_peer, const int64_t* recv_count,
                                   double* const* recv_buf, int32_t nsend, const int32_t* send_peer,
                                   const int64_t* send_count, const double* const* send_buf, int32_t tag);
HQ_API int hq_comm_init_host(hq_ctx* ctx, hq_host_exchange_fn fn, void* user);

#define HQ_IPC_BLOB_BYTES 4096
HQ_API int hq_comm_ipc_export(hq_ctx* ctx, void* blob);
HQ_API int hq_comm_init_ipc(hq_ctx* ctx, const void* all_blobs);
HQ_API int hq_comm_init_ipc_n(hq_ctx* ctx, const void* all_blobs, int32_t nblobs);
HQ_API int hq_comm_init_loopback(hq_ctx* ctx);

HQ_API int hq_group_link(hq_ctx** ctxs, int32_t n);
HQ_API int hq_group_run(hq_ctx** ctxs, int32_t n, int32_t nsteps);

HQ_API int hq_set_source(hq_ctx* ctx, int32_t nloaded, const int32_t* loaded_lnid,
                         int32_t step0, int32_t nsteps, const double* F);

HQ_API int hq_run(hq_ctx* ctx, int32_t nsteps);

HQ_API int hq_sync(hq_ctx* ctx);

HQ_API int hq_check_finite(hq_ctx* ctx, int64_t* nonfinite);

HQ_API int hq_gather(hq_ctx* ctx, int32_t n, const int32_t* lnid, hq_real* tm1_out, hq_real* tm2_out);
HQ_API int hq_gather3(hq_ctx* ctx, int32_t n, const int32_t* lnid, hq_real* tm1_out, hq_real* tm2_out,
                      hq_real* tm3_out);
HQ_API int hq_download(hq_ctx* ctx, hq_real* tm1, hq_real* tm2);
HQ_API int hq_upload(hq_ctx* ctx, const hq_real* tm1, const hq_real* tm2, int32_t step);

typedef struct {
    int32_t        npoints;
    const int32_t* ids;
    const double*  phi;
    int32_t        rate;
    int32_t        derivs;
    int32_t        capacity;
} hq_recorder_desc;
HQ_API int hq_record_add(hq_ctx* ctx, const hq_recorder_desc* desc, int32_t* handle);
HQ_API int hq_record_pending(hq_ctx* ctx, int32_t handle, int32_t* nsamples, int32_t* first_step);
HQ_API int hq_record_fetch(hq_ctx* ctx, int32_t handle, int32_t max_samples, double* out, int32_t* steps,
                           int32_t* nfetched);
HQ_API int hq_record_clear(hq_ctx* ctx);

enum { HQ_SNAP_TM1 = 1, HQ_SNAP_TM2 = 2, HQ_SNAP_VEL = 4 };
typedef struct {
    int32_t first, count;
    int32_t rate;
    int32_t first_step;
    int32_t fields;
    int32_t slots;
} hq_snapshot_desc;
HQ_API int hq_snapshot_add(hq_ctx* ctx, const hq_snapshot_desc* desc, int32_t* handle);
HQ_API int hq_snapshot_pending(hq_ctx* ctx, int32_t handle, int32_t* npending, int32_t* nready, int32_t* first_step);
HQ_API int hq_snapshot_fetch(hq_ctx* ctx, int32_t handle, hq_real* tm1, hq_real* tm2, double* vel, int32_t* step);
HQ_API int hq_snapshot_clear(hq_ctx* ctx);

HQ_API int hq_phase_force(hq_ctx* ctx);
HQ_API int hq_phase_update(hq_ctx* ctx);
HQ_API int hq_download_force(hq_ctx* ctx, double* force);

HQ_API int hq_run_timed(hq_ctx* ctx, int32_t nsteps, double* total_ms, double* kernel_ms_avg);

HQ_API int hq_plan_check(const hq_desc* desc, int64_t report[8]);

HQ_API int hq_stencil_plan_check(const hq_desc* desc, int64_t report[6]);

HQ_API int hq_brick_plan_check(const hq_desc* desc, int64_t report[8]);
HQ_API int hq_brick_plan_check_n(const hq_desc* desc, int64_t* report, int32_t n);

HQ_API int hq_stencil_coefficients(double out[16]);

HQ_API const char* hq_dominant_kernel(hq_ctx* ctx);

#ifdef __cplusplus
}
#endif
#endif
```

Before: 61.74 billion.

## Add two-step temporal blocking for uniform brick units on single-rank runs

Adds a two-step brick mode in which uniform interior units (same material, single n_t row, not ragged or heterogeneous) advance two time steps per pass. Each unit keeps a widened halo of two cells, with extra index tables, and the tiles are cut to a smaller 62x6 footprint so the overlapping halo fits the block. Units near loaded source nodes are demoted back to single-step. The goal is to roughly halve HBM traffic per element update for the bulk of a box mesh, at the cost of redundant halo computation, larger tables and more planning complexity. It is enabled by default only for f64 single-rank runs with no scheduled communication.

```diff
diff --git a/hercules_amd/capi.py b/hercules_amd/capi.py
--- a/hercules_amd/capi.py
+++ b/hercules_amd/capi.py
@@ -9,7 +9,7 @@
 HQ_VARIANT_AUTO, HQ_VARIANT_SCATTER, HQ_VARIANT_PATCH = 0, 1, 2
 IPC_BLOB_BYTES = 4096
 
-EXPORTS = ["hq_device_count", "hq_last_error", "hq_create", "hq_destroy", "hq_get_info", "hq_get_info_sized", "hq_abi_version", "hq_comm_init_ipc_n",
+EXPORTS = ["hq_brick_twostep_check", "hq_get_pair_info", "hq_device_count", "hq_last_error", "hq_create", "hq_destroy", "hq_get_info", "hq_get_info_sized", "hq_abi_version", "hq_comm_init_ipc_n",
            "hq_options_init", "hq_create_opts", "hq_get_options", "hq_real_bytes",
            "hq_comm_unique_id", "hq_comm_init", "hq_comm_selftest", "hq_group_link", "hq_group_run", "hq_set_source", "hq_run", "hq_sync", "hq_gather", "hq_gather3",
            "hq_download", "hq_upload", "hq_phase_force", "hq_phase_update", "hq_download_force",
@@ -93,7 +93,7 @@
                  ("verbose", ctypes.c_int32), ("quiet", ctypes.c_int32),
                  ("brick_ragged", ctypes.c_int32), ("brick_ragged_minfill", ctypes.c_int32),
                  ("allow_env", ctypes.c_int32), ("brick_ragged_het", ctypes.c_int32), ("reserved0", ctypes.c_int32),
-                 ("phase_timing", ctypes.c_int32)])
+                 ("phase_timing", ctypes.c_int32), ("brick_twostep", ctypes.c_int32), ("reserved1", ctypes.c_int32)])
 
     def __init__(self, **kw):
         super().__init__()
@@ -230,7 +230,11 @@
     def info(self):
         i = _Info()
         _check(self._lib.hq_get_info_sized(self._h, ctypes.byref(i), ctypes.c_uint64(ctypes.sizeof(i))), self._lib)
-        return {k: getattr(i, k) for k, _ in _Info._fields_}
+        out = {k: getattr(i, k) for k, _ in _Info._fields_}
+        pair = (ctypes.c_int64 * 4)()
+        _check(self._lib.hq_get_pair_info(self._h, pair), self._lib)
+        out.update(brick_units_twostep=int(pair[0]), brick_units_demoted=int(pair[1]), steps_paired=int(pair[2]))
+        return out
 
     def options(self):
         o = Options()
@@ -434,6 +438,17 @@
     return dict(zip(BRICK_PLAN_REPORT, [int(v) for v in rep]))
 
 
+TWOSTEP_REPORT = ("twostep_units", "twostep_nodes", "region_nodes_checked", "neighbours_checked", "demoted_units", "units",
+                  "reserved", "faults")
+
+
+def brick_twostep_check(desc, loaded=()):
+    ids = np.ascontiguousarray(loaded, np.int32)
+    rep = (ctypes.c_int64 * 8)()
+    _check(load_library().hq_brick_twostep_check(ctypes.byref(desc), ctypes.c_int32(len(ids)), _ptr(ids) if len(ids) else None, rep))
+    return dict(zip(TWOSTEP_REPORT, [int(v) for v in rep]))
+
+
 def comm_unique_id():
     buf = (ctypes.c_char * 128)()
     _check(load_library().hq_comm_unique_id(buf))
diff --git a/hercules_amd/csrc/hq_brick.h b/hercules_amd/csrc/hq_brick.h
--- a/hercules_amd/csrc/hq_brick.h
+++ b/hercules_amd/csrc/hq_brick.h
@@ -22,6 +22,10 @@
 #define HQ_BK_BOTFACE 16
 #define HQ_BK_RAGGED 32
 #define HQ_BK_PACKED 4
+#define HQ_BK_TWOSTEP 64
+#define HQ_B2_TX (HQ_BK_TX - 2)
+#define HQ_B2_TY (HQ_BK_TY - 2)
+#define HQ_B2_THREADS (HQ_BK_THREADS + HQ_BK_TX * HQ_B2_TY)
 #ifndef HQ_BH_WAVES
 #define HQ_BH_WAVES 8
 #endif
@@ -41,6 +45,7 @@
     double  m0, m2, m1;
     double  ft[7], fb[7];
     int64_t coef;
+    int64_t tab2;
 };
 
 struct hq_brick_cfg {
@@ -50,6 +55,7 @@
     int ragged = 1;
     int minfill = 128;
     int ragged_het = 1;
+    int twostep = 1;
 };
 
 static hq_brick_cfg hq_brick_cfg_of(const hq_options& o)
@@ -61,6 +67,7 @@
     c.ragged = hq_value_or(o.brick_ragged, c.ragged) != 0;
     c.minfill = std::min(HQ_BK_THREADS, std::max(1, hq_value_or(o.brick_ragged_minfill, c.minfill)));
     c.ragged_het = hq_value_or(o.brick_ragged_het, c.ragged_het) != 0;
+    c.twostep = hq_value_or(o.brick_twostep, c.twostep) != 0 && sizeof(hq_real) == sizeof(double);
     return c;
 }
 
@@ -70,6 +77,7 @@
     std::vector<hq_brick_unit> units;
     int32_t nsame = 0;
     int32_t nrag = 0;
+    int32_t ntwo = 0;
     std::vector<int32_t> tab;
     std::vector<double> coef;
     std::vector<float> coef32;
@@ -82,6 +90,8 @@
 
 struct hq_brick_plan {
     int64_t nb = 0;
+    int32_t ntwo = 0, ndemoted = 0;
+    uint8_t* d_demoted = nullptr;
     int32_t nunits = 0, nsame = 0, nrag = 0, nhet = 0, npacked = 0, nrhet = 0, nrpacked = 0;
     hq_brick_unit* d_units = nullptr;
     int32_t* d_tab = nullptr;
@@ -104,7 +114,7 @@
 
 static int hq_brick_plan_host(const hq_options& o, int64_t E, int64_t N, const int32_t* lnid, const int32_t* xyz, const double* c1,
                               const double* c2, const double* beta, const double* ntab, const char* excl,
-                              hq_brick_host* B, const hq_mat_src* MS = nullptr)
+                              hq_brick_host* B, const hq_mat_src* MS = nullptr, bool alone = false)
 {
     *B = hq_brick_host();
     if (!xyz || E <= 0 || N <= 0) return 0;
@@ -161,6 +171,7 @@
         int64_t D[3];
         std::vector<int32_t> Ng;
         std::vector<int32_t> Eg;
+        std::vector<char> S0;
     };
     struct column_t { int lvl; int32_t x0, y0, nx, ny, z0, nz, ti, tj; int64_t base; int het; int top, bot; int rag; };
     struct ragged_t { std::vector<uint8_t> own; std::vector<int32_t> pfx; double c[3], m[3]; };
@@ -276,6 +287,25 @@
         }
         lap("simple nodes");
         const int lvl = (int)levels.size();
+        std::vector<int64_t> cutx, cuty;
+        if (cfg.twostep && alone && stencil_ok && !hq_set(o.brick_no_ntsame)) {
+            const int64_t W = sx1 - sx0 + 1, H = sy1 - sy0 + 1;
+            int64_t kx = (W - 2) / HQ_B2_TX, ky = (H - 2) / HQ_B2_TY;
+            if (ky >= 1 && H - ky * HQ_B2_TY < 8) ky--;
+            int64_t n2 = 0;
+#pragma omp parallel for schedule(static) reduction(+ : n2)
+            for (int64_t i = 0; i < (int64_t)S.size(); i++) n2 += S[(size_t)i] == 2;
+            if (kx >= 2 && ky >= 2 && H - ky * HQ_B2_TY <= 2 * TY && n2 == W * H * (L.D[2] - 1)) {
+                const int64_t lx0 = (W - kx * HQ_B2_TX) / 2, ly0 = (H - ky * HQ_B2_TY) / 2;
+                cutx.push_back(sx0);
+                for (int64_t i = 0; i <= kx; i++) cutx.push_back(sx0 + lx0 + i * HQ_B2_TX);
+                cutx.push_back(sx1 + 1);
+                cuty.push_back(sy0);
+                for (int64_t j = 0; j <= ky; j++) cuty.push_back(sy0 + ly0 + j * HQ_B2_TY);
+                cuty.push_back(sy1 + 1);
+                L.S0 = S;
+            }
+        }
         std::vector<std::vector<column_t>> found;
         int32_t ntx_lvl = 1;
         const int rag = cfg.ragged && stencil_ok && !hq_set(o.brick_no_ntsame) ? 1 : 0;
@@ -295,7 +325,9 @@
                             if (in_run(S[(size_t)((Z * NY + Y) * NX + X)])) { sx0 = std::min(sx0, X); sx1 = std::max(sx1, X); sy0 = std::min(sy0, Y); sy1 = std::max(sy1, Y); }
                 if (sx1 < 0) { if (pass == 1) break; else continue; }
             }
-            const int32_t ntx = (int32_t)((sx1 - sx0) / PTX + 1), nty = (int32_t)((sy1 - sy0) / PTY + 1);
+            const bool cut = round == 0 && !cutx.empty();
+            const int32_t ntx = cut ? (int32_t)cutx.size() - 1 : (int32_t)((sx1 - sx0) / PTX + 1);
+            const int32_t nty = cut ? (int32_t)cuty.size() - 1 : (int32_t)((sy1 - sy0) / PTY + 1);
             if (round == 0) ntx_lvl = ntx;
             const size_t f0 = found.size();
             found.resize(f0 + (size_t)nty);
@@ -303,12 +335,12 @@
             const int32_t minfill = rh_round ? std::max(1, cfg.minfill * (HQ_BH_TX * HQ_BH_TY) / HQ_BK_THREADS) : cfg.minfill;
 #pragma omp parallel for schedule(dynamic, 1)
             for (int32_t tj = 0; tj < nty; tj++) {
-                const int64_t y0 = sy0 + (int64_t)tj * PTY;
-                const int32_t ny = (int32_t)std::min<int64_t>(PTY, sy1 - y0 + 1);
+                const int64_t y0 = cut ? cuty[(size_t)tj] : sy0 + (int64_t)tj * PTY;
+                const int32_t ny = cut ? (int32_t)(cuty[(size_t)tj + 1] - y0) : (int32_t)std::min<int64_t>(PTY, sy1 - y0 + 1);
                 std::vector<int32_t> cntz;
                 for (int32_t ti = 0; ti < ntx; ti++) {
-                    const int64_t x0 = sx0 + (int64_t)ti * PTX;
-                    const int32_t nx = (int32_t)std::min<int64_t>(PTX, sx1 - x0 + 1);
+                    const int64_t x0 = cut ? cutx[(size_t)ti] : sx0 + (int64_t)ti * PTX;
+                    const int32_t nx = cut ? (int32_t)(cutx[(size_t)ti + 1] - x0) : (int32_t)std::min<int64_t>(PTX, sx1 - x0 + 1);
                     if (rag_round || rh_round) {
                         cntz.assign((size_t)NZ, 0);
                         for (int iter = 0; iter < (rh_round ? 1 : 4); iter++) {
@@ -529,11 +561,36 @@
     }
     std::stable_sort(us.begin(), us.end(), [](const unit_t& a, const unit_t& b) { return a.key < b.key; });
     B->units.resize(us.size());
-    std::vector<int64_t> toff(us.size() + 1, 0);
+    std::vector<char> two(us.size(), 0);
+#pragma omp parallel for schedule(dynamic, 16)
+    for (int64_t u = 0; u < (int64_t)us.size(); u++) {
+        const column_t& c = cols[(size_t)us[(size_t)u].col];
+        const level_t& L = levels[(size_t)c.lvl];
+        const int32_t za = us[(size_t)u].za, np = us[(size_t)u].np;
+        if (L.S0.empty() || c.rag || c.het || c.nx > HQ_B2_TX || c.ny > HQ_B2_TY) continue;
+        if ((c.top && za == c.z0) || (c.bot && za + np == c.z0 + c.nz)) continue;
+        const int64_t NX = L.D[0] + 1, NY = L.D[1] + 1;
+        if (c.x0 < 2 || c.y0 < 2 || za < 2 || c.x0 + c.nx + 1 > L.D[0] || c.y0 + c.ny + 1 > L.D[1] || za + np + 1 > L.D[2]) continue;
+        const double* q0 = ntab + 7 * (int64_t)L.Ng[(size_t)(((int64_t)za * NY + c.y0) * NX + c.x0)];
+        const int32_t e0 = L.Eg[(size_t)((((int64_t)za - 1) * L.D[1] + (c.y0 - 1)) * L.D[0] + (c.x0 - 1))];
+        bool ok = e0 >= 0;
+        for (int64_t Z = (int64_t)za - 1; Z <= (int64_t)za + np && ok; Z++)
+            for (int64_t Y = (int64_t)c.y0 - 1; Y <= (int64_t)c.y0 + c.ny && ok; Y++)
+                for (int64_t X = (int64_t)c.x0 - 1; X <= (int64_t)c.x0 + c.nx; X++) {
+                    const size_t at = (size_t)((Z * NY + Y) * NX + X);
+                    if (L.S0[at] != 2) { ok = false; break; }
+                    const double* q = ntab + 7 * (int64_t)L.Ng[at];
+                    const int32_t e = L.Eg[(size_t)(((Z - 1) * L.D[1] + (Y - 1)) * L.D[0] + (X - 1))];
+                    if (q[0] != q0[0] || q[1] != q0[1] || q[4] != q0[4] || e < 0 || c1[e] != c1[e0] || c2[e] != c2[e0] || beta[e] != beta[e0]) { ok = false; break; }
+                }
+        two[(size_t)u] = ok;
+    }
+    std::vector<int64_t> toff(us.size() + 1, 0), toff2(us.size(), 0);
     for (size_t u = 0; u < us.size(); u++) {
         const column_t& c = cols[(size_t)us[u].col];
         const int64_t nr = 2 * (c.nx + 2) + 2 * c.ny;
-        toff[u + 1] = toff[u] + ((int64_t)(us[u].np + 2) * nr + (c.rag ? us[u].np + 2 : 2) * (int64_t)c.nx * c.ny + 3) / 4 * 4;
+        toff2[u] = toff[u] + ((int64_t)(us[u].np + 2) * nr + (c.rag ? us[u].np + 2 : 2) * (int64_t)c.nx * c.ny + 3) / 4 * 4;
+        toff[u + 1] = toff2[u] + (two[u] ? ((int64_t)(us[u].np + 4) * (nr + 2 * (c.nx + 4) + 2 * (c.ny + 2)) + 4 * (int64_t)c.nx * c.ny + 3) / 4 * 4 : 0);
     }
     B->tab.assign((size_t)toff[us.size()] + 64, 0);
     std::vector<int64_t> coff(us.size() + 1, 0);
@@ -601,7 +658,7 @@
             }
             U.base = c.base + R.pfx[(size_t)(za - c.z0)];
             U.tab = toff[(size_t)u];
-            U.nx = nx; U.ny = ny; U.np = np; U.flags = HQ_BK_NTSAME | HQ_BK_RAGGED;
+            U.nx = nx; U.ny = ny; U.np = np; U.flags = HQ_BK_NTSAME | HQ_BK_RAGGED; U.tab2 = 0;
             memset(U.ft, 0, sizeof U.ft); memset(U.fb, 0, sizeof U.fb);
             U.coef = 0;
             if (!c.het) {
@@ -628,7 +685,7 @@
             }
         U.base = c.base + (int64_t)(za - c.z0 + c.top) * nx * ny;
         U.tab = toff[(size_t)u];
-        U.nx = nx; U.ny = ny; U.np = np; U.flags = 0;
+        U.nx = nx; U.ny = ny; U.np = np; U.flags = 0; U.tab2 = 0;
         memset(U.ft, 0, sizeof U.ft); memset(U.fb, 0, sizeof U.fb);
         if (c.top && za == c.z0) {
             U.flags |= HQ_BK_TOPFACE;
@@ -656,6 +713,26 @@
         if (sm && !c.het && !hq_set(o.brick_no_ntsame)) { U.flags |= HQ_BK_NTSAME; same[(size_t)u] = 1; }
         U.m0 = q0[0]; U.m2 = q0[1]; U.m1 = q0[4];
         U.coef = 0;
+        if (two[(size_t)u] && same[(size_t)u] == 1) {
+            U.flags |= HQ_BK_TWOSTEP; same[(size_t)u] = 7;
+            U.tab2 = toff2[(size_t)u];
+            const int32_t nr2 = 2 * (nx + 4) + 2 * (ny + 2), rl = nr + nr2;
+            int32_t* t2 = B->tab.data() + toff2[(size_t)u];
+            for (int32_t k = 0; k < np + 4; k++) {
+                const int64_t Z = (int64_t)za - 2 + k;
+                int32_t* r = t2 + (int64_t)k * rl;
+                for (int32_t i = 0; i < nx + 2; i++) { r[i] = dev(c.x0 - 1 + i, c.y0 - 1, Z); r[nx + 2 + i] = dev(c.x0 - 1 + i, c.y0 + ny, Z); }
+                for (int32_t j = 0; j < ny; j++) { r[2 * (nx + 2) + j] = dev(c.x0 - 1, c.y0 + j, Z); r[2 * (nx + 2) + ny + j] = dev(c.x0 + nx, c.y0 + j, Z); }
+                r += nr;
+                for (int32_t i = 0; i < nx + 4; i++) { r[i] = dev(c.x0 - 2 + i, c.y0 - 2, Z); r[nx + 4 + i] = dev(c.x0 - 2 + i, c.y0 + ny + 1, Z); }
+                for (int32_t j = 0; j < ny + 2; j++) { r[2 * (nx + 4) + j] = dev(c.x0 - 2, c.y0 - 1 + j, Z); r[2 * (nx + 4) + ny + 2 + j] = dev(c.x0 + nx + 1, c.y0 - 1 + j, Z); }
+            }
+            int32_t* cap2 = t2 + (int64_t)(np + 4) * rl;
+            const int64_t Zc[4] = { (int64_t)za - 2, (int64_t)za - 1, (int64_t)za + np, (int64_t)za + np + 1 };
+            for (int q4 = 0; q4 < 4; q4++)
+                for (int32_t j = 0; j < ny; j++)
+                    for (int32_t i = 0; i < nx; i++) cap2[((int64_t)q4 * ny + j) * nx + i] = dev(c.x0 + i, c.y0 + j, Zc[q4]);
+        }
         }
         if (c.het) {
             U.flags |= HQ_BK_HET;
@@ -727,9 +804,11 @@
     lap("unit tables");
     if (fault) { g_patch_err = "brick plan: a neighbour of a simple node is missing"; return -1; }
     {
-        std::vector<hq_brick_unit> a, r, b, h, hp, rh, rhp;
+        std::vector<hq_brick_unit> a, a1, r, b, h, hp, rh, rhp;
         for (size_t u = 0; u < us.size(); u++)
-            (same[u] == 1 ? a : (same[u] == 4 ? r : (same[u] == 2 ? h : (same[u] == 3 ? hp : (same[u] == 5 ? rh : (same[u] == 6 ? rhp : b)))))).push_back(B->units[u]);
+            (same[u] == 7 ? a : same[u] == 1 ? a1 : (same[u] == 4 ? r : (same[u] == 2 ? h : (same[u] == 3 ? hp : (same[u] == 5 ? rh : (same[u] == 6 ? rhp : b)))))).push_back(B->units[u]);
+        B->ntwo = (int32_t)a.size();
+        a.insert(a.end(), a1.begin(), a1.end());
         B->nsame = (int32_t)(a.size() + r.size());
         B->nrag = (int32_t)r.size();
         B->nhet = (int32_t)(h.size() + hp.size());
@@ -744,6 +823,7 @@
         a.insert(a.end(), rhp.begin(), rhp.end());
         B->units.swap(a);
         if (B->npacked + B->nrpacked == 0) { std::vector<float>().swap(B->coef32); std::vector<double>().swap(B->nt2); }
+        if (verbose) fprintf(stderr, "  brick plan: %d units may take two steps per pass\n", B->ntwo);
         if (verbose) fprintf(stderr, "  brick plan: %d units: %d with one n_t row of which %d ragged, %d per-element coefficients of which %d packed, %d ragged per-element of which %d packed\n",
                              (int)B->units.size(), B->nsame, B->nrag, B->nhet, B->npacked, B->nrhet, B->nrpacked);
         if (verbose && B->nrag) {
@@ -771,11 +851,12 @@
 hq_k_brick(int32_t count, int32_t per_xcd, const hq_brick_unit* __restrict__ units, const int32_t* __restrict__ tab,
            const hq_real* __restrict__ u1g, const hq_real* __restrict__ u2g, hq_real* __restrict__ ung,
            const double* __restrict__ nt3, const int32_t* __restrict__ src_ptr, const int32_t* __restrict__ src_ent,
-           const double* __restrict__ F, double dt2, hq_stencil_coef sc)
+           const double* __restrict__ F, double dt2, hq_stencil_coef sc, const uint8_t* __restrict__ only = nullptr)
 {
     __shared__ __align__(16) double s_w[2 * 3 * HQ_BK_PLANE];
     const int slot = (int)(blockIdx.x & 7) * per_xcd + (int)(blockIdx.x >> 3);
     if (slot >= count) return;
+    if (only && !only[slot]) return;
     const hq_brick_unit U = units[slot];
     const int nx = U.nx, ny = U.ny, np = U.np, nxy = nx * ny, nr = 2 * (nx + 2) + 2 * ny;
     const int t = threadIdx.x, lx = t & (HQ_BK_TX - 1), ly = t >> 6;
@@ -959,6 +1040,225 @@
     }
 #undef HQ_BK_LOAD
 #undef HQ_BK_PUT
+}
+
+
+
+template <int PY>
+static __device__ __forceinline__ void hq_bk_plane_sums(const hq_lds_double* __restrict__ q, const double* P, const double* Q,
+                                                       double m[3], double g[3], double Uo[3])
+{
+    double C[3], XM[3], XP[3], YM[3], YP[3], MM[3], PM[3], MP[3], PP[3];
+#pragma unroll
+    for (int d = 0; d < 3; d++) {
+        C[d] = q[d]; XM[d] = q[d - 3]; XP[d] = q[d + 3]; YM[d] = q[d - 3 * PY]; YP[d] = q[d + 3 * PY];
+        MM[d] = q[d - 3 * PY - 3]; PM[d] = q[d - 3 * PY + 3];
+        MP[d] = q[d + 3 * PY - 3]; PP[d] = q[d + 3 * PY + 3];
+    }
+    double sx[3], sy[3], dg[3];
+#pragma unroll
+    for (int d = 0; d < 3; d++) { sx[d] = XM[d] + XP[d]; sy[d] = YM[d] + YP[d]; dg[d] = (MM[d] + PP[d]) + (PM[d] + MP[d]); }
+    const double A_x = (PP[0] + MM[0]) - (PM[0] + MP[0]), A_y = (PP[1] + MM[1]) - (PM[1] + MP[1]);
+    const double Bx0_z = XP[2] - XM[2], Bx0_x = XP[0] - XM[0], By0_z = YP[2] - YM[2], By0_y = YP[1] - YM[1];
+    const double Bx1_z = (PP[2] - MP[2]) + (PM[2] - MM[2]), Bx1_x = (PP[0] - MP[0]) + (PM[0] - MM[0]);
+    const double By1_z = (PP[2] - PM[2]) + (MP[2] - MM[2]), By1_y = (PP[1] - PM[1]) + (MP[1] - MM[1]);
+    const double sxy_z = sx[2] + sy[2];
+    m[0] = fma(P[0], C[0], fma(P[1], sx[0], fma(P[2], sy[0], fma(P[3], dg[0], Q[0] * A_y))));
+    m[1] = fma(P[0], C[1], fma(P[1], sy[1], fma(P[2], sx[1], fma(P[3], dg[1], Q[0] * A_x))));
+    m[2] = fma(P[0], C[2], fma(P[2], sxy_z, P[4] * dg[2]));
+    g[0] = fma(P[2], C[0], fma(P[3], sx[0], fma(P[4], sy[0], fma(P[5], dg[0], Q[1] * A_y))));
+    g[1] = fma(P[2], C[1], fma(P[3], sy[1], fma(P[4], sx[1], fma(P[5], dg[1], Q[1] * A_x))));
+    g[2] = fma(P[1], C[2], fma(P[3], sxy_z, P[5] * dg[2]));
+    Uo[0] = fma(Q[0], Bx0_z, Q[1] * Bx1_z);
+    Uo[1] = fma(Q[0], By0_z, Q[1] * By1_z);
+    Uo[2] = fma(Q[0], Bx0_x, fma(Q[1], Bx1_x, fma(Q[0], By0_y, Q[1] * By1_y)));
+}
+
+#define HQ_B2_P1Y (HQ_BK_TX + 2)
+#define HQ_B2_PLANE1 ((HQ_BK_TX + 2) * (HQ_BK_TY + 2))
+#define HQ_B2_P2Y HQ_BK_TX
+#define HQ_B2_PLANE2 (HQ_BK_TX * HQ_BK_TY)
+#define HQ_B2_LDS (8 * (2 * 3 * HQ_B2_PLANE1 + 2 * 9 * HQ_B2_PLANE2 + 2 * 3 * HQ_B2_PLANE2))
+
+__global__ void __launch_bounds__(HQ_B2_THREADS, 4)
+hq_k_brick2(int32_t count, int32_t per_xcd, const hq_brick_unit* __restrict__ units, const int32_t* __restrict__ tab,
+            const uint8_t* __restrict__ demoted, const hq_real* __restrict__ u1g, const hq_real* __restrict__ u2g,
+            hq_real* __restrict__ ung, hq_real* __restrict__ u4g, hq_stencil_coef sc)
+{
+    extern __shared__ __align__(16) double s_b2[];
+    double* const s_w1 = s_b2;
+    double* const s_w2 = s_b2 + 2 * 3 * HQ_B2_PLANE1;
+    double* const s_u = s_w2 + 2 * 9 * HQ_B2_PLANE2;
+    const int slot = (int)(blockIdx.x & 7) * per_xcd + (int)(blockIdx.x >> 3);
+    if (slot >= count) return;
+    if (demoted && demoted[slot]) return;
+    const hq_brick_unit U = units[slot];
+    const int nx = U.nx, ny = U.ny, np = U.np, nxy = nx * ny;
+    const int nr = 2 * (nx + 2) + 2 * ny, nr2 = 2 * (nx + 4) + 2 * (ny + 2), rl = nr + nr2;
+    const int32_t* __restrict__ t2 = tab + U.tab2;
+    const int32_t* __restrict__ cap2 = t2 + (int64_t)(np + 4) * rl;
+    double P[6], Q[2];
+#pragma unroll
+    for (int i = 0; i < 6; i++) P[i] = hq_uniform(U.c1 * sc.p1[i] + U.c2 * sc.p2[i]);
+#pragma unroll
+    for (int i = 0; i < 2; i++) Q[i] = hq_uniform(U.c1 * sc.q1[i] + U.c2 * sc.q2[i]);
+    const double beta = U.beta, m2 = U.m2, m1 = U.m1, m0i = hq_uniform(1.0 / U.m0);
+    const int t = threadIdx.x;
+    const bool s1 = t < HQ_BK_THREADS;
+    const int tt = s1 ? t : t - HQ_BK_THREADS;
+    const int lx = tt & (HQ_BK_TX - 1), ly = s1 ? tt >> 6 : 1 + (tt >> 6);
+    const bool inner = lx >= 1 && lx <= nx && ly >= 1 && ly <= ny;
+    const int sidx = inner ? (ly - 1) * nx + (lx - 1) : 0;
+    const int row1 = (ly + 1) * HQ_B2_P1Y + lx + 1, row2 = ly * HQ_B2_P2Y + lx;
+    if (s1) {
+        const bool inreg = lx < nx + 2 && ly < ny + 2, border = inreg && !inner;
+        const int bofs = !border ? 0 : (ly == 0 ? lx : (ly == ny + 1 ? nx + 2 + lx : (lx == 0 ? 2 * (nx + 2) + ly - 1 : 2 * (nx + 2) + ny + ly - 1)));
+        const bool ring = t < nr2;
+        int rrow;
+        {
+            const int rx = nx + 2, ry = ny + 2;
+            int px, py;
+            if (t < rx + 2) { px = t - 1; py = -1; }
+            else if (t < 2 * (rx + 2)) { px = t - (rx + 2) - 1; py = ry; }
+            else if (t < 2 * (rx + 2) + ry) { px = -1; py = t - 2 * (rx + 2); }
+            else { px = rx; py = t - 2 * (rx + 2) - ry; }
+            rrow = (py + 1) * HQ_B2_P1Y + px + 1;
+        }
+        const int oofs = nr + (ring ? t : 0);
+        hq_real x1[3] = { 0, 0, 0 }, x2[3] = { 0, 0, 0 }, y1[3] = { 0, 0, 0 }, y2[3] = { 0, 0, 0 };
+        double fA[3] = { 0.0, 0.0, 0.0 }, fB[3] = { 0.0, 0.0, 0.0 };
+        int32_t bid = inner ? cap2[sidx] : t2[bofs], oid = t2[oofs];
+#define HQ_B2_LOAD(k_)                                                                                \
+        {                                                                                             \
+            const int kk_ = (k_);                                                                     \
+            if (inreg) {                                                                              \
+                const int64_t a_ = inner && kk_ >= 2 && kk_ < np + 2 ? U.base + (int64_t)(kk_ - 2) * nxy + sidx : (int64_t)bid; \
+                _Pragma("unroll") for (int d = 0; d < 3; d++) { x1[d] = u1g[3 * a_ + d]; x2[d] = u2g[3 * a_ + d]; } \
+            }                                                                                         \
+            if (ring) {                                                                               \
+                const int64_t b_ = (int64_t)oid;                                                      \
+                _Pragma("unroll") for (int d = 0; d < 3; d++) { y1[d] = u1g[3 * b_ + d]; y2[d] = u2g[3 * b_ + d]; } \
+            }                                                                                         \
+            if (kk_ < np + 3) {                                              \
+                const int kn_ = kk_ + 1;                                                              \
+                bid = inner ? cap2[(kn_ < 2 ? kn_ : (kn_ >= np + 2 ? kn_ - np : 0)) * nxy + sidx] : t2[(int64_t)kn_ * rl + bofs]; \
+                oid = t2[(int64_t)kn_ * rl + oofs];                                                   \
+            }                                                                                         \
+        }
+#define HQ_B2_PUT(k_, acc_)                                                                           \
+        {                                                                                             \
+            hq_lds_double* img_ = (hq_lds_double*)s_w1 + 3 * HQ_B2_PLANE1 * ((k_) & 1);                \
+            _Pragma("unroll") for (int d = 0; d < 3; d++) {                                           \
+                const double a1_ = x1[d], a2_ = x2[d];                                                \
+                img_[3 * row1 + d] = a1_ + beta * (a1_ - a2_);                                        \
+                acc_[d] += m2 * a1_ - m1 * a2_;                                                       \
+                ((hq_lds_double*)s_u)[3 * (HQ_B2_PLANE2 * ((k_) & 1) + row2) + d] = a1_;               \
+            }                                                                                         \
+            if (ring) { _Pragma("unroll") for (int d = 0; d < 3; d++) { const double b1_ = y1[d], b2_ = y2[d]; img_[3 * rrow + d] = b1_ + beta * (b1_ - b2_); } } \
+        }
+        HQ_B2_LOAD(0)
+        { double dummy[3] = { 0.0, 0.0, 0.0 }; HQ_B2_PUT(0, dummy) }
+        for (int k = 0; k <= np + 4; k++) {
+            if (k <= np + 2) HQ_B2_LOAD(k + 1)
+            __syncthreads();
+            if (k <= np + 3) {
+                double m[3], g[3], Uo[3];
+                hq_bk_plane_sums<HQ_B2_P1Y>((const hq_lds_double*)s_w1 + 3 * (HQ_B2_PLANE1 * (k & 1) + row1), P, Q, m, g, Uo);
+                __builtin_amdgcn_sched_barrier(0);
+                double un1[3];
+#pragma unroll
+                for (int d = 0; d < 3; d++) {
+                    const double f = fA[d] + (g[d] + Uo[d]);
+                    const hq_real r = (hq_real)(f * m0i);
+                    un1[d] = (double)r;
+                }
+                if (inner && k >= 3 && k < np + 3) {
+                    hq_real* out = ung + 3 * (U.base + (int64_t)(k - 3) * nxy + sidx);
+#pragma unroll
+                    for (int d = 0; d < 3; d++) out[d] = (hq_real)un1[d];
+                }
+                hq_lds_double* img2 = (hq_lds_double*)s_w2 + 9 * HQ_B2_PLANE2 * ((k + 1) & 1);
+#pragma unroll
+                for (int d = 0; d < 3; d++) {
+                    const double a1_ = un1[d], a2_ = ((const hq_lds_double*)s_u)[3 * (HQ_B2_PLANE2 * ((k + 1) & 1) + row2) + d];
+                    img2[3 * row2 + d] = a1_ + beta * (a1_ - a2_);
+                    img2[3 * HQ_B2_PLANE2 + 3 * row2 + d] = a1_;
+                    img2[6 * HQ_B2_PLANE2 + 3 * row2 + d] = a2_;
+                }
+#pragma unroll
+                for (int d = 0; d < 3; d++) { fA[d] = fB[d] + m[d]; fB[d] = g[d] - Uo[d]; }
+                if (k <= np + 2) HQ_B2_PUT(k + 1, fB)
+            }
+        }
+#undef HQ_B2_LOAD
+#undef HQ_B2_PUT
+    } else {
+        double gA[3] = { 0.0, 0.0, 0.0 }, gB[3] = { 0.0, 0.0, 0.0 };
+        for (int k = 0; k <= np + 4; k++) {
+            __syncthreads();
+            const int r = k - 2;
+            if (inner && r >= 1) {
+                const hq_lds_double* img2 = (const hq_lds_double*)s_w2 + 9 * HQ_B2_PLANE2 * (r & 1);
+                double m[3], g[3], Uo[3];
+#pragma unroll
+                for (int d = 0; d < 3; d++) {
+                    const double a1_ = img2[3 * HQ_B2_PLANE2 + 3 * row2 + d], a2_ = img2[6 * HQ_B2_PLANE2 + 3 * row2 + d];
+                    gB[d] += m2 * a1_ - m1 * a2_;
+                }
+                hq_bk_plane_sums<HQ_B2_P2Y>(img2 + 3 * row2, P, Q, m, g, Uo);
+                if (r >= 3 && r < np + 3) {
+                    hq_real* out = u4g + 3 * (U.base + (int64_t)(r - 3) * nxy + sidx);
+#pragma unroll
+                    for (int d = 0; d < 3; d++) { const double f = gA[d] + (g[d] + Uo[d]); out[d] = (hq_real)(f * m0i); }
+                }
+#pragma unroll
+                for (int d = 0; d < 3; d++) { gA[d] = gB[d] + m[d]; gB[d] = g[d] - Uo[d]; }
+            }
+        }
+    }
+}
+
+static __host__ __device__ inline bool hq_b2_is_loaded(const int32_t* __restrict__ sorted, int32_t n, int32_t id)
+{
+    int32_t lo = 0, hi = n;
+    while (lo < hi) { const int32_t mid = (lo + hi) >> 1; if (sorted[mid] < id) lo = mid + 1; else hi = mid; }
+    return lo < n && sorted[lo] == id;
+}
+
+__global__ void hq_k_brick2_demote(int32_t ntwo, const hq_brick_unit* __restrict__ units, const int32_t* __restrict__ tab,
+                                   int32_t nloaded, const int32_t* __restrict__ sorted, uint8_t* __restrict__ demoted)
+{
+    const int u = blockIdx.x;
+    if (u >= ntwo) return;
+    const hq_brick_unit U = units[u];
+    const int nxy = U.nx * U.ny;
+    const int64_t total = (int64_t)(U.np + 4) * (2 * (U.nx + 2) + 2 * U.ny + 2 * (U.nx + 4) + 2 * (U.ny + 2)) + 4 * (int64_t)nxy;
+    const int32_t* __restrict__ t2 = tab + U.tab2;
+    bool hit = false;
+    for (int64_t i = threadIdx.x; i < total; i += blockDim.x) hit = hit || hq_b2_is_loaded(sorted, nloaded, t2[i]);
+    if (threadIdx.x == 0) {
+        int32_t lo = 0, hi = nloaded;
+        while (lo < hi) { const int32_t mid = (lo + hi) >> 1; if ((int64_t)sorted[mid] < U.base) lo = mid + 1; else hi = mid; }
+        hit = hit || (lo < nloaded && (int64_t)sorted[lo] < U.base + (int64_t)nxy * U.np);
+    }
+    if (hit) demoted[u] = 1;
+}
+
+static void hq_brick2_demote_host(const hq_brick_host& B, const std::vector<int32_t>& sorted, std::vector<uint8_t>* flags)
+{
+    flags->assign((size_t)B.ntwo, 0);
+    const int32_t n = (int32_t)sorted.size();
+    for (int32_t u = 0; u < B.ntwo; u++) {
+        const hq_brick_unit& U = B.units[(size_t)u];
+        const int64_t nxy = (int64_t)U.nx * U.ny;
+        const int64_t total = (int64_t)(U.np + 4) * (2 * (U.nx + 2) + 2 * U.ny + 2 * (U.nx + 4) + 2 * (U.ny + 2)) + 4 * nxy;
+        const int32_t* t2 = B.tab.data() + U.tab2;
+        bool hit = false;
+        for (int64_t i = 0; i < total && !hit; i++) hit = hq_b2_is_loaded(sorted.data(), n, t2[i]);
+        auto it = std::lower_bound(sorted.begin(), sorted.end(), (int32_t)U.base);
+        hit = hit || (it != sorted.end() && (int64_t)*it < U.base + nxy * U.np);
+        (*flags)[(size_t)u] = hit;
+    }
 }
 
 
@@ -1152,7 +1452,7 @@
 
 static void hq_brick_free(hq_brick_plan* P)
 {
-    void* ptrs[] = { P->d_units, P->d_tab, P->d_coef, P->d_coef32, P->d_nt2, P->d_src_ptr, P->d_src_ent };
+    void* ptrs[] = { P->d_units, P->d_tab, P->d_coef, P->d_coef32, P->d_nt2, P->d_src_ptr, P->d_src_ent, P->d_demoted };
     for (void* p : ptrs) if (p) hipFree(p);
     *P = hq_brick_plan();
 }
@@ -1167,7 +1467,18 @@
     P->npacked = B.npacked;
     P->nrhet = B.nrhet;
     P->nrpacked = B.nrpacked;
+    P->ntwo = B.ntwo;
     if (P->nunits == 0) return 0;
+    if (P->ntwo > 0) {
+        static bool attr2_set = false;
+        if (!attr2_set) {
+            if (hipFuncSetAttribute((const void*)hq_k_brick2, hipFuncAttributeMaxDynamicSharedMemorySize, HQ_B2_LDS) != hipSuccess) { g_patch_err = "hq_k_brick2: LDS attribute"; return -3; }
+            attr2_set = true;
+        }
+        if (hipMalloc((void**)&P->d_demoted, (size_t)P->ntwo) != hipSuccess) { g_patch_err = "hipMalloc failed"; return -2; }
+        if (hipMemset(P->d_demoted, 0, (size_t)P->ntwo) != hipSuccess) { g_patch_err = "memset failed"; return -3; }
+        *bytes += P->ntwo;
+    }
     if (P->nhet + P->nrhet > 0) {
         if (P->nhet > P->npacked || P->nrhet > P->nrpacked) {
             if (hipMalloc((void**)&P->d_coef, 8 * B.coef.size()) != hipSuccess) { g_patch_err = "hipMalloc failed"; return -2; }
@@ -1217,6 +1528,25 @@
 {
     if (P->d_src_ptr) { hipFree(P->d_src_ptr); P->d_src_ptr = nullptr; }
     if (P->d_src_ent) { hipFree(P->d_src_ent); P->d_src_ent = nullptr; }
+    P->ndemoted = 0;
+    if (P->ntwo > 0) {
+        if (hipMemset(P->d_demoted, 0, (size_t)P->ntwo) != hipSuccess) return -3;
+        if (nloaded > 0) {
+            std::vector<int32_t> sorted(loaded, loaded + nloaded);
+            std::sort(sorted.begin(), sorted.end());
+            int32_t* d_sorted = nullptr;
+            if (hipMalloc((void**)&d_sorted, 4 * sorted.size()) != hipSuccess) return -2;
+            std::vector<uint8_t> flags((size_t)P->ntwo, 0);
+            bool ok = hipMemcpy(d_sorted, sorted.data(), 4 * sorted.size(), hipMemcpyHostToDevice) == hipSuccess;
+            if (ok) {
+                hq_k_brick2_demote<<<P->ntwo, 256, 0, nullptr>>>(P->ntwo, P->d_units, P->d_tab, nloaded, d_sorted, P->d_demoted);
+                ok = hipMemcpy(flags.data(), P->d_demoted, (size_t)P->ntwo, hipMemcpyDeviceToHost) == hipSuccess;
+            }
+            hipFree(d_sorted);
+            if (!ok) return -3;
+            for (uint8_t f : flags) P->ndemoted += f != 0;
+        }
+    }
     if (nloaded <= 0 || P->nunits == 0) return 0;
     std::vector<std::array<int32_t, 3>> rec;
     for (int32_t i = 0; i < nloaded; i++) {
@@ -1245,14 +1575,26 @@
 }
 
 static void hq_brick_launch(const hq_brick_plan* P, const hq_real* u1, const hq_real* u2, hq_real* un, const double* nt3,
-                            const double* F, double dt2, hipStream_t stream, bool light = false)
+                            const double* F, double dt2, hipStream_t stream, bool light = false, int pair = 0, hq_real* u4 = nullptr)
 {
+    if (pair == 1 && P->ntwo > 0) {
+        const int per_xcd = (P->ntwo + 7) / 8;
+        hq_k_brick2<<<per_xcd * 8, HQ_B2_THREADS, HQ_B2_LDS, stream>>>(P->ntwo, per_xcd, P->d_units, P->d_tab, P->d_demoted, u1, u2, un, u4, hq_stencil().c);
+    }
+    if (pair && P->ndemoted > 0) {
+        const int per_xcd = (P->ntwo + 7) / 8;
+        const int32_t* sp = P->d_src_ptr;
+        hq_k_brick<false, false><<<per_xcd * 8, HQ_BK_THREADS, 0, stream>>>(P->ntwo, per_xcd, P->d_units, P->d_tab, u1, u2, un, nt3, sp, P->d_src_ent,
+                                                                            (sp ? F : nullptr), dt2, hq_stencil().c, P->d_demoted);
+    }
     const int32_t cnt[7] = { P->nsame - P->nrag, P->nunits - P->nsame - P->nhet - P->nrhet, P->nhet - P->npacked, P->npacked, P->nrag,
                              P->nrhet - P->nrpacked, P->nrpacked };
     int32_t first = 0;
+    const int32_t skip = pair ? P->ntwo : 0;
     for (int k4 = 0; k4 < 7; k4++) {
         const int k = k4 == 0 ? 0 : (k4 == 1 ? 4 : (k4 < 5 ? k4 - 1 : k4));
-        const int32_t count = cnt[k];
+        int32_t count = cnt[k];
+        if (k == 0 && skip) { first += skip; count -= skip; }
         if (count <= 0) continue;
         const int per_xcd = (count + 7) / 8;
         const int32_t* sp = P->d_src_ptr ? P->d_src_ptr + first : nullptr;
diff --git a/hercules_amd/csrc/hq_engine.hip b/hercules_amd/csrc/hq_engine.hip
--- a/hercules_amd/csrc/hq_engine.hip
+++ b/hercules_amd/csrc/hq_engine.hip
@@ -138,8 +138,11 @@
     double* d_beta = nullptr;
     double* d_nt = nullptr;
     double* d_nt_rows = nullptr;
-    hq_real* d_u[3] = { nullptr, nullptr, nullptr };
+    hq_real* d_u[4] = { nullptr, nullptr, nullptr, nullptr };
     int now = 0, prev = 1, spare = 2;
+    int extra = 3;
+    int pair = 0;
+    int64_t steps_paired = 0;
     double* d_force = nullptr;
     int32_t nloaded = 0, src_step0 = 0, src_nsteps = 0;
     int32_t* d_loaded = nullptr;
@@ -1224,7 +1227,8 @@
             auto launch_bricks = [&]() {
                 if (c->bricks.nunits > 0)
                     hq_brick_launch(&c->bricks, c->d_u[c->now], c->d_u[c->prev], c->d_u[c->spare], c->plan.d_nt3, F, c->dt2,
-                                    bs ? c->bstream : c->stream, hq_given(c->opts.brick_by_component) ? c->opts.brick_by_component != 0 : c->overlap);
+                                    bs ? c->bstream : c->stream, hq_given(c->opts.brick_by_component) ? c->opts.brick_by_component != 0 : c->overlap,
+                                    c->pair, c->pair == 1 ? c->d_u[c->extra] : nullptr);
                 if (bs) hipEventRecord(c->ev_bricks, c->bstream);
             };
             hq_mark(c);
@@ -1382,6 +1386,41 @@
     return HQ_OK;
 }
 
+static bool hq_can_pair(const hq_ctx* c, int32_t remaining)
+{
+    if (remaining < 2 || c->variant != HQ_VARIANT_PATCH || c->bricks.ntwo <= 0 || !c->d_u[3]) return false;
+    if (hq_has_transport(c) || c->nranks != 1) return false;
+    const int64_t mid = (int64_t)c->step + 1;
+    for (const auto& r : c->recs) if (mid % r.rate == 0) return false;
+    for (const auto& sn : c->snaps) if (hq_snapshot_due(sn, mid)) return false;
+    if (c->nloaded > 0 && c->src_nsteps > 0 && (mid == c->src_step0 || mid == (int64_t)c->src_step0 + c->src_nsteps)) return false;
+    if (hq_clock_on(c) && (hq_set(c->opts.phase_timing) || (mid & 3) == 0)) return false;
+    return true;
+}
+
+static int hq_step_pair(hq_ctx* c)
+{
+    c->pair = 1;
+    int rc = hq_step(c);
+    if (rc == HQ_OK) {
+        std::swap(c->spare, c->extra);
+        c->pair = 2;
+        rc = hq_step(c);
+    }
+    c->pair = 0;
+    if (rc == HQ_OK) c->steps_paired++;
+    return rc;
+}
+
+static int hq_steps(hq_ctx* c, int32_t nsteps)
+{
+    for (int32_t s = 0; s < nsteps;) {
+        if (hq_can_pair(c, nsteps - s)) { HQ_TRY(hq_step_pair(c)); s += 2; }
+        else { HQ_TRY(hq_step(c)); s++; }
+    }
+    return HQ_OK;
+}
+
 
 static int hq_build_distribution(hq_ctx* c, const std::vector<int32_t>& sd)
 {
@@ -1728,6 +1767,10 @@
                             prep.dn, prep.seed0.data(), &pb, BH.nb);
         lap("patch plan");
         if (rc == 0 && BH.nb > 0) rc = hq_brick_upload(&c->bricks, BH, &pb);
+        if (rc == 0 && c->bricks.ntwo > 0) {
+            if (hq_dev_alloc(c, &c->d_u[3], n3) != HQ_OK) rc = -2;
+            else if (hipMemset(c->d_u[3], 0, sizeof(hq_real) * n3) != hipSuccess) rc = -3;
+        }
         c->bricks.mat = { 0.0, 0.0, d->deltaT, d->mat_bbase, d->mat_threshold_damping, d->mat_threshold_vpvs };
         lap("brick upload");
         if (rc != 0)
@@ -1770,7 +1813,7 @@
         delete I;
         c->ipc = nullptr;
     }
-    void* ptrs[] = { c->d_gather_ids, c->d_gather_out, c->d_lnid, c->d_c1, c->d_c2, c->d_beta, c->d_nt_rows, c->d_u[0], c->d_u[1], c->d_u[2],
+    void* ptrs[] = { c->d_gather_ids, c->d_gather_out, c->d_lnid, c->d_c1, c->d_c2, c->d_beta, c->d_nt_rows, c->d_u[0], c->d_u[1], c->d_u[2], c->d_u[3],
                      c->d_force, c->d_loaded, c->d_F, c->d_dn_id, c->d_dn_ptr, c->d_dn_anchor,
                      c->an.d_cmap, c->an.d_smap, c->an.d_c_out, c->an.d_c_in, c->an.d_s_out, c->an.d_s_in,
                      c->dn.d_cmap, c->dn.d_smap, c->dn.d_c_out, c->dn.d_c_in, c->dn.d_s_out, c->dn.d_s_in,
@@ -2336,7 +2379,7 @@
         return hq_fail(HQ_ERR_STATE, "linked contexts are stepped with hq_group_run%s", "");
     HQ_TRY(hq_output_check_room(c, nsteps));
     HQ_HIP(hipSetDevice(c->device));
-    for (int32_t s = 0; s < nsteps; s++) HQ_TRY(hq_step(c));
+    HQ_TRY(hq_steps(c, nsteps));
     HQ_HIP(hipGetLastError());
     return HQ_OK;
 }
@@ -2413,7 +2456,7 @@
     HQ_HIP(hipEventRecord(c->ev_span[0], c->stream));
     c->timing = true;
     int rc = HQ_OK;
-    for (int32_t s = 0; s < nsteps && rc == HQ_OK; s++) rc = hq_step(c);
+    rc = hq_steps(c, nsteps);
     c->timing = false;
     if (c->overlap) hipStreamWaitEvent(c->stream, c->ev_shared, 0);
     if (c->bstream) hipStreamWaitEvent(c->stream, c->ev_bricks, 0);
@@ -2436,6 +2479,13 @@
     if (he != hipSuccess) return hq_fail(HQ_ERR_DEVICE, "timed run failed: %s", hipGetErrorString(he));
     if (total_ms) *total_ms = tot;
     if (kernel_ms_avg) *kernel_ms_avg = ker;
+    return HQ_OK;
+}
+
+extern "C" int hq_get_pair_info(hq_ctx* c, int64_t out[4])
+{
+    if (!c || !out) return hq_fail(HQ_ERR_ARG, "null argument%s", "");
+    out[0] = c->bricks.ntwo; out[1] = c->bricks.ndemoted; out[2] = c->steps_paired; out[3] = 0;
     return HQ_OK;
 }
 
@@ -2756,6 +2806,7 @@
     HQ_TRY(hq_field_to_device(c, tm1, c->d_u[c->now]));
     HQ_TRY(hq_field_to_device(c, tm2, c->d_u[c->prev]));
     if (c->d_u[2]) {
+        if (c->d_u[3]) HQ_HIP(hipMemsetAsync(c->d_u[c->extra], 0, bytes, c->stream));
         HQ_HIP(hipMemsetAsync(c->d_u[c->spare], 0, bytes, c->stream));
         HQ_HIP(hipStreamSynchronize(c->stream));
     }
diff --git a/hercules_amd/csrc/hq_opts.h b/hercules_amd/csrc/hq_opts.h
--- a/hercules_amd/csrc/hq_opts.h
+++ b/hercules_amd/csrc/hq_opts.h
@@ -26,6 +26,7 @@
     HQ_OPT_D("HQ_LOOPBACK_DELAY_US", loopback_delay_us), HQ_OPT_I("HQ_PATCH_VERBOSE", verbose), HQ_OPT_I("HQ_QUIET", quiet),
     HQ_OPT_I("HQ_BRICK_RAGGED", brick_ragged), HQ_OPT_I("HQ_BRICK_RAGGED_MINFILL", brick_ragged_minfill),
     HQ_OPT_I("HQ_PHASE_TIMING", phase_timing), HQ_OPT_I("HQ_BRICK_RAGGED_HET", brick_ragged_het),
+    HQ_OPT_I("HQ_BRICK_TWOSTEP", brick_twostep),
 };
 #undef HQ_OPT_I
 #undef HQ_OPT_D
@@ -39,6 +40,7 @@
     }
     o->allow_env = -1;
     o->reserved0 = -1;
+    o->reserved1 = -1;
 }
 
 static void hq_options_adopt(hq_options* dst, const hq_options* src)
diff --git a/hercules_amd/csrc/hq_plan_check.h b/hercules_amd/csrc/hq_plan_check.h
--- a/hercules_amd/csrc/hq_plan_check.h
+++ b/hercules_amd/csrc/hq_plan_check.h
@@ -412,4 +412,131 @@
     return rc;
 }
 
+extern "C" int hq_brick_twostep_check(const hq_desc* d, int32_t nloaded, const int32_t* loaded, int64_t report[8])
+{
+    hq_options opts;
+    hq_options_resolve(&opts, nullptr);
+    if (!report) return hq_fail(HQ_ERR_ARG, "null argument%s", "");
+    for (int k = 0; k < 8; k++) report[k] = 0;
+    if (!d || !d->node_xyz || !d->eTable || !d->nTable || nloaded < 0 || (nloaded && !loaded))
+        return hq_fail(HQ_ERR_ARG, "inconsistent mesh description (node_xyz is needed)%s", "");
+    hq_prep prep;
+    HQ_TRY(hq_prepare(d, opts, HQ_PREP_BRICKS, &prep));
+    const int64_t E = d->lenum, N = d->nharbored;
+    const hq_brick_host& B = prep.bricks;
+    report[5] = (int64_t)B.units.size();
+    if (B.nb == 0 || B.ntwo == 0) return HQ_OK;
+    const std::vector<int32_t>& perm = prep.perm;
+    const std::vector<double>&c1 = prep.c1, &c2 = prep.c2, &beta = prep.beta;
+    int64_t bad = 0, nreg = 0, nnb = 0, nown = 0;
+    std::vector<int32_t> inv((size_t)N, -1);
+    for (int64_t n = 0; n < N; n++) inv[(size_t)perm[(size_t)n]] = (int32_t)n;
+    std::vector<int64_t> aptr((size_t)N + 1, 0);
+    for (int64_t i = 0; i < E * 8; i++) aptr[(size_t)d->lnid[i] + 1]++;
+    for (int64_t n = 0; n < N; n++) aptr[(size_t)n + 1] += aptr[(size_t)n];
+    std::vector<int64_t> adj((size_t)(E * 8));
+    {
+        std::vector<int64_t> fill(aptr.begin(), aptr.end() - 1);
+        for (int64_t i = 0; i < E * 8; i++) adj[(size_t)fill[(size_t)d->lnid[i]]++] = i;
+    }
+    auto at2 = [&](const hq_brick_unit& U, int x, int y, int k) -> int64_t {
+        const int nx = U.nx, ny = U.ny, np = U.np, nr = 2 * (nx + 2) + 2 * ny, rl = nr + 2 * (nx + 4) + 2 * (ny + 2);
+        const int32_t* t2 = B.tab.data() + U.tab2;
+        const int32_t* row = t2 + (int64_t)k * rl;
+        if (x >= 0 && x < nx && y >= 0 && y < ny) {
+            if (k >= 2 && k < np + 2) return U.base + ((int64_t)(k - 2) * ny + y) * nx + x;
+            return t2[(int64_t)(np + 4) * rl + ((int64_t)(k < 2 ? k : k - np) * ny + y) * nx + x];
+        }
+        if (x >= -1 && x <= nx && y >= -1 && y <= ny) {
+            if (y == -1) return row[x + 1];
+            if (y == ny) return row[nx + 2 + x + 1];
+            if (x == -1) return row[2 * (nx + 2) + y];
+            return row[2 * (nx + 2) + ny + y];
+        }
+        row += nr;
+        if (y == -2) return row[x + 2];
+        if (y == ny + 1) return row[nx + 4 + x + 2];
+        if (x == -2) return row[2 * (nx + 4) + y + 1];
+        return row[2 * (nx + 4) + ny + 2 + y + 1];
+    };
+    for (size_t u = 0; u < B.units.size(); u++)
+        if (((B.units[u].flags & HQ_BK_TWOSTEP) != 0) != ((int64_t)u < B.ntwo)) bad++;
+#pragma omp parallel for schedule(dynamic, 4) reduction(+ : bad, nreg, nnb, nown)
+    for (int64_t u = 0; u < (int64_t)B.ntwo; u++) {
+        const hq_brick_unit& U = B.units[(size_t)u];
+        const int nx = U.nx, ny = U.ny, np = U.np;
+        if (!(U.flags & HQ_BK_NTSAME) || (U.flags & (HQ_BK_HET | HQ_BK_RAGGED | HQ_BK_TOPFACE | HQ_BK_BOTFACE)) || nx < 1 || nx > HQ_B2_TX ||
+            ny < 1 || ny > HQ_B2_TY || np < 1 || U.tab2 < 0) { bad++; continue; }
+        nown += (int64_t)nx * ny * np;
+        for (int k = 1; k <= np + 2; k++)
+            for (int y = -1; y <= ny; y++)
+                for (int x = -1; x <= nx; x++) {
+                    const int64_t q = at2(U, x, y, k);
+                    if (q < 0 || q >= N) { bad++; continue; }
+                    const int32_t n = inv[(size_t)q];
+                    nreg++;
+                    if (prep.excl[(size_t)n]) bad++;
+                    const double* t7 = prep.ntab + 7 * q;
+                    if (!((t7[1] == t7[2]) && (t7[1] == t7[3]) && (t7[4] == t7[5]) && (t7[4] == t7[6]))) bad++;
+                    if (t7[0] != U.m0 || t7[1] != U.m2 || t7[4] != U.m1) bad++;
+                    if (aptr[(size_t)n + 1] - aptr[(size_t)n] != 8) { bad++; continue; }
+                    int64_t el[8];
+                    for (int o = 0; o < 8; o++) el[o] = -1;
+                    bool ok = true;
+                    for (int64_t a = aptr[(size_t)n]; a < aptr[(size_t)n + 1]; a++) {
+                        const int64_t e = adj[(size_t)a] >> 3;
+                        const int o = (int)(adj[(size_t)a] & 7);
+                        if (el[o] != -1) ok = false;
+                        el[o] = e;
+                        if (c1[(size_t)e] != U.c1 || c2[(size_t)e] != U.c2 || beta[(size_t)e] != U.beta) ok = false;
+                    }
+                    if (!ok) { bad++; continue; }
+                    for (int dz = -1; dz <= 1; dz++)
+                        for (int dy = -1; dy <= 1; dy++)
+                            for (int dx = -1; dx <= 1; dx++) {
+                                if (!dx && !dy && !dz) continue;
+                                const int o = (dx < 0 ? 1 : 0) | (dy < 0 ? 2 : 0) | (dz < 0 ? 4 : 0);
+                                const int m = (dx > 0 ? 1 : 0) | (dy > 0 ? 2 : 0) | (dz > 0 ? 4 : 0);
+                                if (at2(U, x + dx, y + dy, k + dz) != (int64_t)perm[(size_t)d->lnid[8 * el[o] + m]]) bad++;
+                                nnb++;
+                            }
+                }
+    }
+    std::vector<int32_t> sorted;
+    for (int32_t i = 0; i < nloaded; i++) {
+        if (loaded[i] < 0 || loaded[i] >= N) return hq_fail(HQ_ERR_ARG, "loaded node id out of range%s", "");
+        sorted.push_back(perm[(size_t)loaded[i]]);
+    }
+    std::sort(sorted.begin(), sorted.end());
+    std::vector<uint8_t> flags, want((size_t)B.ntwo, 0);
+    hq_brick2_demote_host(B, sorted, &flags);
+    if (nloaded > 0) {
+        std::vector<int32_t> unit_of((size_t)B.nb, -1);
+        for (int32_t u = 0; u < B.ntwo; u++) {
+            const hq_brick_unit& U = B.units[(size_t)u];
+            for (int64_t q = U.base; q < U.base + (int64_t)U.nx * U.ny * U.np; q++) unit_of[(size_t)q] = u;
+        }
+        for (int32_t i = 0; i < nloaded; i++) {
+            std::vector<int32_t> ball(1, loaded[i]);
+            for (int hop = 0; hop < 2; hop++) {
+                std::vector<int32_t> next = ball;
+                for (int32_t n : ball)
+                    for (int64_t a = aptr[(size_t)n]; a < aptr[(size_t)n + 1]; a++)
+                        for (int c8 = 0; c8 < 8; c8++) next.push_back(d->lnid[8 * (adj[(size_t)a] >> 3) + c8]);
+                std::sort(next.begin(), next.end());
+                next.erase(std::unique(next.begin(), next.end()), next.end());
+                ball.swap(next);
+            }
+            for (int32_t n : ball) {
+                const int32_t q = perm[(size_t)n];
+                if (q < B.nb && unit_of[(size_t)q] >= 0) want[(size_t)unit_of[(size_t)q]] = 1;
+            }
+        }
+    }
+    for (int32_t u = 0; u < B.ntwo; u++) { if (flags[(size_t)u] != want[(size_t)u]) bad++; report[4] += flags[(size_t)u]; }
+    report[0] = B.ntwo; report[1] = nown; report[2] = nreg; report[3] = nnb; report[7] = bad;
+    if (bad) return hq_fail(HQ_ERR_STATE, "two-step brick plan self-check failed%s", "");
+    return HQ_OK;
+}
+
 #endif
diff --git a/hercules_amd/csrc/hq_prepare.h b/hercules_amd/csrc/hq_prepare.h
--- a/hercules_amd/csrc/hq_prepare.h
+++ b/hercules_amd/csrc/hq_prepare.h
@@ -104,8 +104,10 @@
     if ((what & HQ_PREP_BRICKS) && d->node_xyz && !hq_set(o.no_bricks)) {
         hq_mat_src ms;
         ms.edata = d->edata; ms.dt = d->deltaT; ms.bbase = d->mat_bbase; ms.thr_damp = d->mat_threshold_damping; ms.thr_vpvs = d->mat_threshold_vpvs;
+        bool alone = d->nranks <= 1;
+        hq_for_each_sched_node(d, [&](int, int, int32_t) { alone = false; });
         if (hq_brick_plan_host(o, E, N, d->lnid, d->node_xyz, out->c1.data(), out->c2.data(), out->beta.data(), out->ntab,
-                               out->excl.data(), &BH, &ms) != 0)
+                               out->excl.data(), &BH, &ms, alone) != 0)
             return hq_fail(HQ_ERR_ARG, "brick plan: %s", hq_patch_error());
         lap(&out->brick_plan_s);
     }
diff --git a/include/hq_solver.h b/include/hq_solver.h
--- a/include/hq_solver.h
+++ b/include/hq_solver.h
@@ -157,6 +157,8 @@
     int32_t brick_ragged_het;
     int32_t reserved0;
     int32_t phase_timing;
+    int32_t brick_twostep;
+    int32_t reserved1;
 } hq_options;
 
 HQ_API void hq_options_init(hq_options* opts, uint64_t size);
@@ -246,6 +248,8 @@
 
 HQ_API int hq_brick_plan_check(const hq_desc* desc, int64_t report[8]);
 HQ_API int hq_brick_plan_check_n(const hq_desc* desc, int64_t* report, int32_t n);
+HQ_API int hq_get_pair_info(hq_ctx* ctx, int64_t out[4]);
+HQ_API int hq_brick_twostep_check(const hq_desc* desc, int32_t nloaded, const int32_t* loaded, int64_t report[8]);
 
 HQ_API int hq_stencil_coefficients(double out[16]);
 
```

Result: slower. 47.64 billion (-22.8%).
